# theshubh007/neural_rx

Measured on AMD Instinct MI355X. Metric: 5G NR slots/sec + p50 per-slot latency, nrx_rt config, higher is better.
Workload: dtype f16; 1 GPU; nrx_rt, 2 users, 4 PRB, 4 rx_ant, 16-QAM, batch=128 slots per GPU; global_batch=128, num_it=2, parallelism=dp1 (slot shards), streams=2

## Files before the change

### neural_rx_amd/build.py

```python
from __future__ import annotations

import hashlib
import os
import subprocess
import sys

HERE = os.path.dirname(os.path.abspath(__file__))
CSRC = os.path.join(HERE, "csrc")
LIB = os.path.join(HERE, "lib", "libnrx.so")
KERNEL_TUS = ["nrx_k_p16.hip", "nrx_k_p16m.hip", "nrx_k_p16s.hip", "nrx_k_p64.hip", "nrx_k_fwd0.hip",
              "nrx_k_fwd1.hip", "nrx_k_fwd2.hip", "nrx_k_rr.hip", "nrx_k_col.hip", "nrx_dispatch.hip"]
SOURCES = [os.path.join(CSRC, f) for f in KERNEL_TUS] + [
    os.path.join(CSRC, "nrx_aerial.hip"), os.path.join(CSRC, "nrx_synth.hip"), os.path.join(CSRC, "nrx_lmmse.hip"),
    os.path.join(CSRC, "nrx_kbest.hip"), os.path.join(CSRC, "nrx_chest.hip"),
    os.path.join(CSRC, "nrx_softmetrics.hip"), os.path.join(CSRC, "nrx_ldpc.hip"),
    os.path.join(CSRC, "nrx_cfo.hip"), os.path.join(CSRC, "nrx_ls.hip"), os.path.join(CSRC, "nrx_cir.hip"),
    os.path.join(CSRC, "nrx_ofdm.hip"), os.path.join(CSRC, "nrx_timechan.hip"), os.path.join(CSRC, "nrx_train.hip"),
    os.path.join(CSRC, "nrx_model.cpp"), os.path.join(CSRC, "nrx_api.cpp")]
HEADERS = [os.path.join(CSRC, "nrx_internal.h"), os.path.join(CSRC, "nrx_model.h"), os.path.join(CSRC, "nrx_rng.h"),
           os.path.join(HERE, "..", "include", "nrx.h")]
KERNEL_INCS = [os.path.join(CSRC, "nrx_device.inc"), os.path.join(CSRC, "nrx_launch.inc"),
               os.path.join(CSRC, "nrx_rr.inc"), os.path.join(CSRC, "nrx_col.inc"), os.path.join(CSRC, "nrx_geom.h")]
DEPS = SOURCES + HEADERS + KERNEL_INCS + [os.path.abspath(__file__)]
ARCH = os.environ.get("NRX_OFFLOAD_ARCH", "gfx950")


def hipcc() -> str:
    for c in (os.environ.get("HIPCC"), "/opt/rocm/bin/hipcc", "hipcc"):
        if c and (os.path.sep not in c or os.path.exists(c)):
            return c
    raise RuntimeError("hipcc not found")


def needs_build() -> bool:
    if not os.path.exists(LIB):
        return True
    t = os.path.getmtime(LIB)
    if any(os.path.getmtime(d) > t for d in DEPS if os.path.exists(d)):
        return True
    return any(_stale(os.path.join(OBJ_DIR, os.path.basename(s) + ".o"), s) for s in SOURCES)


OBJ_DIR = os.path.join(HERE, "lib", "obj")


def _includes(src: str) -> list:
    if os.path.basename(src) in KERNEL_TUS:
        return HEADERS + KERNEL_INCS
    return HEADERS


def _sig(src: str) -> str:
    return " ".join(repr(os.path.getmtime(d)) for d in [src] + _includes(src) if os.path.exists(d))


def _stale(obj: str, src: str) -> bool:
    sig = obj + ".sig"
    if not os.path.exists(obj) or not os.path.exists(sig):
        return True
    return open(sig).read() != _sig(src)


def strip_comments(text: str) -> str:
    out, i, n = [], 0, len(text)
    while i < n:
        c = text[i]
        if c == "/" and i + 1 < n and text[i + 1] == "/":
            j = text.find("\n", i)
            i = n if j < 0 else j
            out.append(" ")
        elif c == "/" and i + 1 < n and text[i + 1] == "*":
            j = text.find("*/", i + 2)
            i = n if j < 0 else j + 2
            out.append(" ")
        elif c in "\"'":
            j = i + 1
            while j < n and text[j] != c:
                j += 2 if text[j] == "\\" else 1
            out.append(text[i:j + 1])
            i = j + 1
        else:
            out.append(c)
            i += 1
    return " ".join("".join(out).split())


def hash_sources(texts: dict) -> str:
    h = hashlib.sha256()
    for name in sorted(texts):
        h.update(name.encode() + b"\0" + strip_comments(texts[name]).encode() + b"\0")
    return h.hexdigest()[:16]


def source_hash() -> str:
    texts = {}
    for p in sorted(set(SOURCES + HEADERS + KERNEL_INCS)):
        with open(p, encoding="utf-8") as f:
            texts[os.path.basename(p)] = f.read()
    return hash_sources(texts)


def _build_id_object(verbose: bool, obj_dir: str = OBJ_DIR, tag: str = "") -> str:
    src = os.path.join(obj_dir, "nrx_build_id.cpp")
    obj = src + ".o"
    with open(src, "w") as f:
        f.write('extern "C" const char* nrx_build_id(void) { return "%s%s"; }\n' % (source_hash(), tag))
    cmd = [hipcc(), "-O2", "-fPIC", "-c", src, "-o", obj]
    if verbose:
        print(" ".join(cmd), flush=True)
    subprocess.run(cmd, check=True)
    return obj


def build(force: bool = False, verbose: bool = True, lib: str = LIB, obj_dir: str = OBJ_DIR,
          extra_flags=()) -> str:
    if lib == LIB and not force and not needs_build():
        return LIB
    os.makedirs(obj_dir, exist_ok=True)
    tmp = lib + f".tmp{os.getpid()}"
    flags = [f"--offload-arch={ARCH}", "-O3", "-std=c++17", "-fPIC", "-Wall", "-Wno-unused-function",
             *extra_flags]
    objs, procs = [], []
    for src in SOURCES:
        obj = os.path.join(obj_dir, os.path.basename(src) + ".o")
        objs.append(obj)
        if not force and not _stale(obj, src):
            continue
        part = obj + f".{os.getpid()}.part"
        cmd = [hipcc(), *flags, "-c", src, "-o", part]
        if verbose:
            print(" ".join(cmd), flush=True)
        procs.append((subprocess.Popen(cmd), part, obj, _sig(src)))
    bad = 0
    for p, part, obj, sig in procs:
        rc = p.wait()
        if rc:
            bad = rc
            if os.path.exists(part):
                os.remove(part)
        else:
            os.replace(part, obj)
            with open(obj + ".sig", "w") as f:
                f.write(sig)
    if bad:
        raise subprocess.CalledProcessError(bad, "hipcc -c")
    objs.append(_build_id_object(verbose, obj_dir, "+" + "".join(extra_flags) if extra_flags else ""))
    cmd = [hipcc(), f"--offload-arch={ARCH}", "-shared", *objs, "-o", tmp]
    if verbose:
        print(" ".join(cmd), flush=True)
    subprocess.run(cmd, check=True)
    os.replace(tmp, lib)
    return lib


if __name__ == "__main__":
    build(force="--force" in sys.argv)
```

### neural_rx_amd/csrc/nrx_api.cpp

```cpp
#include <hip/hip_runtime.h>

#include <cmath>
#include <cstdio>
#include <cstdlib>
#include <cstring>
#include <string>
#include <type_traits>
#include <vector>

#include "../../include/nrx.h"
#include "nrx_internal.h"
#include "nrx_model.h"

namespace nrx {
hipError_t launch_forward_f16(const FwdArgs<_Float16, float, _Float16>& args, const ModelW<_Float16, float>& W,
                              const FwdPlan& pl, const FusedCtl& fc, hipStream_t st, Prof* prof);
void device_counts(int* cus, int* xccs);
size_t fused_sync_bytes();
hipError_t fused_sync_status(void* sync, int* st, bool reset, hipEvent_t last);
hipError_t run_tier_p64(const FwdArgs<double, double, float>& args, const ModelW<double, double>& W,
                        const FwdPlan& pl, hipStream_t st, Prof* prof);
hipError_t setup_kernels();
int strip_width(int precision);

static thread_local std::string g_err;

int fail(int code, const std::string& msg) {
  g_err = msg;
  return code;
}

int hip_fail(hipError_t e, const char* what) {
  return fail(NRX_ERR_HIP, std::string(what) + ": " + hipGetErrorString(e));
}
}

using namespace nrx;

namespace {

int check_range(const char* name, long v, long lo, long hi, int code = NRX_ERR_SHAPE) {
  if (v >= lo && v <= hi) return NRX_OK;
  return fail(code, std::string(name) + " must be " + std::to_string(lo) + ".." + std::to_string(hi));
}

template <class IO>
int check_grid(const IO* io, int tx_supported = kMaxUsers, int min_subcarriers = 1) {
  if (io->num_symbols != kT) return fail(NRX_ERR_SHAPE, "num_symbols must be 14");
  if (int rc = check_range("batch", io->batch, 1, 65535)) return rc;
  if (int rc = check_range("num_subcarriers", io->num_subcarriers, min_subcarriers, 12 * 275)) return rc;
  if (io->num_tx > tx_supported && tx_supported < kMaxUsers)
    return fail(NRX_ERR_UNSUPPORTED, "the kernels are built for num_tx <= " + std::to_string(tx_supported));
  return check_range("num_tx", io->num_tx, 1, kMaxUsers);
}
template <class IO>
int check_grid_ant(const IO* io, int tx_supported = kMaxUsers, int min_subcarriers = 1) {
  if (int rc = check_grid(io, tx_supported, min_subcarriers)) return rc;
  return check_range("num_rx_ant", io->num_rx_ant, 1, 16);
}

int check_mcs_bits(const int32_t* bits, int num_mcs, bool qam, int num_mcs_code = NRX_ERR_SHAPE) {
  if (int rc = check_range("num_mcs", num_mcs, 1, 8, num_mcs_code)) return rc;
  for (int m = 0; m < num_mcs; ++m)
    if (qam ? bits[m] != 2 && bits[m] != 4 && bits[m] != 6 : bits[m] < 1 || bits[m] > 8)
      return fail(NRX_ERR_INVALID_ARG, qam ? "mcs_bits must be 2, 4 or 6" : "mcs_bits must be 1..8");
  return NRX_OK;
}
int check_bits_stride(int bits_stride, const int32_t* bits, int num_mcs) {
  for (int m = 0; m < num_mcs; ++m)
    if (bits_stride < bits[m]) return fail(NRX_ERR_SHAPE, "bits_stride < max(mcs_bits)");
  return NRX_OK;
}

int check_dmrs_symbols(const int32_t* sym, int n, int* mask = nullptr) {
  if (int rc = check_range("num_dmrs_symbols", n, 1, 4)) return rc;
  int bits = 0;
  for (int k = 0; k < n; ++k) {
    if (sym[k] < 0 || sym[k] >= kT || (k && sym[k] <= sym[k - 1]))
      return fail(NRX_ERR_INVALID_ARG, "dmrs_symbols must be ascending symbol indices below 14");
    bits |= 1 << sym[k];
  }
  if (mask) *mask = bits;
  return NRX_OK;
}
int check_cdm_group(const int32_t* group, int num_tx) {
  for (int u = 0; u < num_tx; ++u)
    if (group[u] != 0 && group[u] != 1) return fail(NRX_ERR_INVALID_ARG, "cdm_group must be 0/1");
  return NRX_OK;
}
int check_dmrs_ports(int num_tx, const int32_t* group, const int32_t* focc, const int32_t* tocc, int despread_f,
                     int despread_t, int num_subcarriers, const int32_t* sym, int num_dmrs_symbols) {
  if (int rc = check_range("despread_f", despread_f, 0, 1, NRX_ERR_INVALID_ARG)) return rc;
  if (int rc = check_range("despread_t", despread_t, 0, 1, NRX_ERR_INVALID_ARG)) return rc;
  unsigned seen = 0;
  for (int u = 0; u < num_tx; ++u) {
    if ((focc[u] != 0 && focc[u] != 1) || (tocc[u] != 0 && tocc[u] != 1))
      return fail(NRX_ERR_INVALID_ARG, "focc and tocc must be 0/1");
    const unsigned bit = 1u << (group[u] + 2 * focc[u] + 4 * tocc[u]);
    if (seen & bit) return fail(NRX_ERR_INVALID_ARG, "two ports share one (cdm_group, focc, tocc)");
    seen |= bit;
    if (focc[u] && !despread_f) return fail(NRX_ERR_INVALID_ARG, "a port with focc = 1 needs despread_f");
    if (tocc[u] && !despread_t) return fail(NRX_ERR_INVALID_ARG, "a port with tocc = 1 needs despread_t");
  }
  if (despread_f && num_subcarriers % 4)
    return fail(NRX_ERR_SHAPE, "despread_f needs num_subcarriers % 4 == 0 (pairs of comb positions)");
  if (despread_t) {
    bool ok = num_dmrs_symbols % 2 == 0;
    for (int k = 0; ok && k < num_dmrs_symbols; k += 2) ok = sym[k + 1] == sym[k] + 1;
    if (!ok) return fail(NRX_ERR_INVALID_ARG, "despread_t needs dmrs_symbols in pairs (t, t + 1)");
  }
  return NRX_OK;
}
int check_aerial_list(const void* re, const void* im, int num_subcarriers) {
  if ((re == nullptr) != (im == nullptr)) return fail(NRX_ERR_INVALID_ARG, "Aerial outputs come in (real, imag) pairs");
  if (re && num_subcarriers % 12) return fail(NRX_ERR_SHAPE, "Aerial pilot list needs num_subcarriers % 12 == 0");
  return NRX_OK;
}
int check_symbol_mask(const char* name, int v) {
  if (v >= 0 && v < (1 << kT)) return NRX_OK;
  return fail(NRX_ERR_INVALID_ARG, std::string(name) + " must be a mask of the 14 symbols");
}
int check_pos(const char* name, double v) {
  if (v > 0.0 && std::isfinite(v)) return NRX_OK;
  return fail(NRX_ERR_INVALID_ARG, std::string(name) + " must be finite and > 0");
}
int check_nonneg(const char* name, double v) {
  if (v >= 0.0 && std::isfinite(v)) return NRX_OK;
  return fail(NRX_ERR_INVALID_ARG, std::string(name) + " must be finite and >= 0");
}

int check_tap_span(long l_min, long l_max) {
  if (int rc = check_range("l_min", l_min, -255, 0)) return rc;
  if (int rc = check_range("l_max", l_max, 0, 255)) return rc;
  if (l_max - l_min + 1 > 256) return fail(NRX_ERR_SHAPE, "the tap span l_max - l_min + 1 must be <= 256");
  return NRX_OK;
}

int too_small(size_t need) {
  return fail(NRX_ERR_WORKSPACE, "workspace too small: need " + std::to_string(need) + " bytes");
}
int check_workspace(const void* ws, size_t bytes, size_t need, size_t align) {
  if (!ws) return fail(NRX_ERR_INVALID_ARG, "null workspace pointer");
  if ((uintptr_t)ws & (align - 1))
    return fail(NRX_ERR_INVALID_ARG, "workspace must be " + std::to_string(align) + "-byte aligned");
  return bytes < need ? too_small(need) : NRX_OK;
}
int store_size(size_t* bytes, size_t need) {
  if (!bytes) return fail(NRX_ERR_INVALID_ARG, "bytes is NULL");
  *bytes = need;
  return NRX_OK;
}
int launched(hipError_t e, const char* what) { return e == hipSuccess ? NRX_OK : hip_fail(e, what); }

}

struct EventProf : Prof {
  struct Rec { int kid; hipEvent_t a, b; };
  std::vector<Rec> recs;
  std::vector<hipEvent_t> pool;
  hipEvent_t get() {
    if (!pool.empty()) {
      hipEvent_t e = pool.back();
      pool.pop_back();
      return e;
    }
    hipEvent_t e = nullptr;
    (void)hipEventCreate(&e);
    return e;
  }
  void begin(int kid, void* st) override {
    Rec r{kid, get(), nullptr};
    (void)hipEventRecord(r.a, (hipStream_t)st);
    recs.push_back(r);
  }
  void end(int, void* st) override {
    hipEvent_t e = get();
    (void)hipEventRecord(e, (hipStream_t)st);
    recs.back().b = e;
  }
  int64_t launches[K_COUNT] = {0};
  double total_ms[K_COUNT] = {0};
  hipError_t collect() {
    for (auto& r : recs) {
      hipError_t e = hipEventSynchronize(r.b);
      if (e != hipSuccess) return e;
      float ms = 0.f;
      e = hipEventElapsedTime(&ms, r.a, r.b);
      if (e != hipSuccess) return e;
      launches[r.kid] += 1;
      total_ms[r.kid] += ms;
      pool.push_back(r.a);
      pool.push_back(r.b);
    }
    recs.clear();
    return hipSuccess;
  }
  void reset() {
    for (int k = 0; k < K_COUNT; ++k) {
      launches[k] = 0;
      total_ms[k] = 0;
    }
  }
  ~EventProf() override {
    for (auto& r : recs) {
      (void)hipEventDestroy(r.a);
      if (r.b) (void)hipEventDestroy(r.b);
    }
    for (auto e : pool) (void)hipEventDestroy(e);
  }
};

struct nrx_handle {
  nrx_desc desc;
  int device;
  DeviceModel<_Float16, float> m16;
  DeviceModel<double, double> m64;
  EventProf* prof = nullptr;
  void* fused_sync = nullptr;
  int fused_enabled = 1;
  int spin_limit = kFusedSpinLimit;
  int dbg_err = 0;
  int update_rr = kSchedDefault;
  hipEvent_t last_ev = nullptr;
  hipStream_t last_stream = nullptr;
  bool have_last = false;
  FusedCtl fused_ctl() const { return FusedCtl{fused_sync, spin_limit, dbg_err}; }
  int small_tiers = 1;
  Sched sched() const { return Sched{update_rr, fused_enabled, small_tiers}; }
};

struct FwdWs {
  double* norm;
  void *s_out, *s_in, *a_out, *a, *pe16;
  size_t total;
};
static FwdWs fwd_layout(const nrx_shape* s, int precision, void* ws) {
  const bool f16 = precision == NRX_PREC_F16;
  const size_t plane = (size_t)s->num_tx * s->num_subcarriers * kT * kDS * (f16 ? 2 : 4);
  Carver c(ws);
  FwdWs w{};
  w.norm = c.take<double>(s->batch);
  w.s_out = c.take<char>(s->batch * plane);
  w.s_in = c.take<char>(s->batch * plane);
  w.a_out = c.take<char>(s->batch * plane);
  w.a = c.take<char>(s->batch * plane);
  if (f16) w.pe16 = c.take<char>(plane);
  w.total = c.bytes();
  return w;
}
static size_t ws_bytes_of(const nrx_shape* s, int precision) { return fwd_layout(s, precision, nullptr).total; }

static int check_shape(const nrx_shape* s) {
  if (!s) return fail(NRX_ERR_INVALID_ARG, "shape is NULL");
  return check_grid(s);
}

template <class WT, class BT, class S>
static void fill_args(FwdArgs<WT, BT, S>& a, const nrx_desc* d, const nrx_io* io, void* ws, int init_cinp) {
  const nrx_shape* s = &io->shape;
  a.B = s->batch;
  a.llr_B = s->batch;
  a.U = s->num_tx;
  a.F = s->num_subcarriers;
  a.A = d->num_rx_ant;
  a.M = d->num_mcs;
  a.H = num_heads(d);
  a.init_cinp = init_cinp;
  a.num_init = num_heads(d);
  a.masking = d->var_mcs_masking;
  a.use_h = d->use_h_hat;
  a.bits_max = bits_max(d);
  for (int i = 0; i < kMaxHeads; ++i)
    a.head_bits[i] = i < a.H ? head_bits(d, i) : 0;
  a.y = io->y;
  a.pe = io->pe;
  a.h_hat = io->h_hat;
  a.active = io->active;
  a.mcs_mask = io->mcs_mask;
  a.llr = io->llr;
  a.h_ref = io->h_ref;
  const FwdWs w = fwd_layout(s, io->precision, ws);
  a.norm = w.norm;
  a.s_in = (S*)w.s_in;
  a.s_out = (S*)w.s_out;
  a.a = (S*)w.a;
  a.a_out = (S*)w.a_out;
  a.pe16 = (S*)w.pe16;
  a.ws_base = (const char*)ws;
  a.ws_bytes = w.total < 0xFFFFFFFFull ? (unsigned)w.total : 0xFFFFFFFFu;
}

static int forward_slots(nrx_handle* h, const nrx_io* io, int llr_B, void* workspace, hipStream_t st);
static int chunk_slots(const nrx_shape* s, int precision);

template <class F>
static int each_chunk(const nrx_shape* s, int precision, F f) {
  const int B = s->batch, bc = chunk_slots(s, precision);
  for (int b0 = 0; b0 < B; b0 += bc)
    if (int rc = f(b0, b0 + bc < B ? bc : B - b0)) return rc;
  return NRX_OK;
}

static FwdPlan plan_f16(FwdArgs<_Float16, float, _Float16>& a, const nrx_desc* d, const nrx_io* io, int n, void* ws,
                        int init_cinp, const Sched& sc, int cus, int xccs) {
  nrx_io c = *io;
  c.shape.batch = n;
  fill_args(a, d, &c, ws, init_cinp);
  return plan_forward(a, io->num_it, sc, cus, xccs);
}

static int busy(const nrx_handle* h, hipStream_t st) {
  if (h->have_last && h->last_stream != st && hipEventQuery(h->last_ev) == hipErrorNotReady)
    return fail(NRX_ERR_BUSY, "a one-launch forward of this handle is still running on another stream");
  return NRX_OK;
// ... 840 lines not shown
}

int nrx_chest_nmse(const nrx_nmse_io* io, void* workspace, size_t workspace_bytes, void* stream) {
  if (int rc = check_nmse(io)) return rc;
  if (int rc = check_workspace(workspace, workspace_bytes, nmse_workspace_bytes(*io), 8)) return rc;
  return launched(launch_chest_nmse(*io, workspace, (hipStream_t)stream), "channel nmse launch");
}

struct nrx_ldpc {
  LdpcDev d;
  int device;
  void* tables;
};

constexpr int kLdpcMaxN = 68 * 384;

int nrx_ldpc_create(const nrx_ldpc_code* code, int32_t device, nrx_ldpc** out) {
  if (!code || !code->shifts || !out) return fail(NRX_ERR_INVALID_ARG, "null argument");
  *out = nullptr;
  const int mb = code->mb, nb = code->nb, z = code->z;
  if (mb < 1 || mb > 46) return fail(NRX_ERR_SHAPE, "mb must be 1..46");
  if (nb < 2 || nb > 68) return fail(NRX_ERR_SHAPE, "nb must be 2..68");
  if (nb <= mb) return fail(NRX_ERR_SHAPE, "nb must be > mb");
  if (z < 2 || z > 384) return fail(NRX_ERR_SHAPE, "z must be 2..384");
  if (code->kb < 1 || code->kb >= nb) return fail(NRX_ERR_SHAPE, "kb must be 1..nb-1");
  if (device < -1) return fail(NRX_ERR_INVALID_ARG, "device must be >= 0, or -1 for a handle without device tables");
  std::vector<int> row_ptr(mb + 1, 0), edges, colw(nb, 0);
  for (int i = 0; i < mb; ++i) {
    for (int j = 0; j < nb; ++j) {
      const int s = code->shifts[i * nb + j];
      if (s < -1 || s >= z) return fail(NRX_ERR_INVALID_ARG, "shifts must be -1..z-1");
      if (s < 0) continue;
      edges.push_back(j * z);
      edges.push_back(s);
      colw[j] += 1;
    }
    row_ptr[i + 1] = (int)edges.size() / 2;
    const int w = row_ptr[i + 1] - row_ptr[i];
    if (w < 2 || w > 32) return fail(NRX_ERR_INVALID_ARG, "row weight must be 2..32");
  }
  for (int j = 0; j < nb; ++j)
    if (!colw[j]) return fail(NRX_ERR_INVALID_ARG, "column weight must be >= 1");
  nrx_ldpc* h = new nrx_ldpc();
  h->d.mb = mb, h->d.nb = nb, h->d.z = z, h->d.kb = code->kb, h->d.num_edges = row_ptr[mb];
  h->d.plan = ldpc_plan(nb, z, h->d.num_edges);
  h->d.row_ptr = nullptr, h->d.edges = nullptr;
  h->device = device;
  h->tables = nullptr;
  if (device >= 0) {
    hipError_t e = hipSetDevice(device);
    if (e == hipSuccess) e = ldpc_setup();
    const size_t rp = (size_t)(mb + 1) * 4, rpa = (rp + 15) / 16 * 16, eb = edges.size() * 4;
    if (e == hipSuccess) e = hipMalloc(&h->tables, rpa + eb);
    if (e == hipSuccess) e = hipMemcpy(h->tables, row_ptr.data(), rp, hipMemcpyHostToDevice);
    if (e == hipSuccess) e = hipMemcpy((char*)h->tables + rpa, edges.data(), eb, hipMemcpyHostToDevice);
    if (e != hipSuccess) {
      if (h->tables) (void)hipFree(h->tables);
      delete h;
      return hip_fail(e, "ldpc tables");
    }
    h->d.row_ptr = (const int*)h->tables;
    h->d.edges = (const int*)((char*)h->tables + rpa);
  }
  *out = h;
  return NRX_OK;
}

void nrx_ldpc_destroy(nrx_ldpc* h) {
  if (!h) return;
  if (h->tables) (void)hipFree(h->tables);
  delete h;
}

static int check_ldpc_io(const nrx_ldpc_io* io) {
  if (!io) return fail(NRX_ERR_INVALID_ARG, "io is NULL");
  if (!io->llr_in || !io->hard || !io->iters || !io->parity_ok) return fail(NRX_ERR_INVALID_ARG, "null tensor pointer");
  if (int rc = check_range("num_iter", io->num_iter, 1, 100, NRX_ERR_INVALID_ARG)) return rc;
  if (io->cn_type != 0 && io->cn_type != 1) return fail(NRX_ERR_INVALID_ARG, "cn_type must be 0 (boxplus) or 1 (min-sum)");
  if (io->early_stop != 0 && io->early_stop != 1) return fail(NRX_ERR_INVALID_ARG, "early_stop must be 0 or 1");
  if (io->cn_type == 1 && !(io->ms_scale > 0.0f && io->ms_scale <= 1.0f))
    return fail(NRX_ERR_INVALID_ARG, "ms_scale must be in (0, 1]");
  if (int rc = check_pos("llr_clip", io->llr_clip)) return rc;
  return check_range("num_cw", io->num_cw, 1, 1 << 20);
}

static size_t ldpc_workspace_bytes(const nrx_ldpc* h, const nrx_ldpc_io* io) {
  const size_t msgs = h->d.plan.msg_lds ? 0 : (size_t)io->num_cw * h->d.num_edges * h->d.z * 4;
  return msgs > 256 ? msgs : 256;
}

int nrx_ldpc_workspace_size(const nrx_ldpc* h, const nrx_ldpc_io* io, size_t* bytes) {
  if (int rc = check_ldpc_io(io)) return rc;
  if (!h) return fail(NRX_ERR_INVALID_ARG, "null handle");
  return store_size(bytes, ldpc_workspace_bytes(h, io));
}

int nrx_ldpc_decode(nrx_ldpc* h, const nrx_ldpc_io* io, void* workspace, size_t workspace_bytes, void* stream) {
  if (int rc = check_ldpc_io(io)) return rc;
  if (!h) return fail(NRX_ERR_INVALID_ARG, "null handle");
  if (int rc = check_workspace(workspace, workspace_bytes, ldpc_workspace_bytes(h, io), 16)) return rc;
  if (h->device < 0) return fail(NRX_ERR_INVALID_ARG, "no device: the handle was created with device = -1");
  return launched(launch_ldpc_decode(h->d, *io, workspace, (hipStream_t)stream), "ldpc decode launch");
}

int nrx_ldpc_gather(const nrx_ldpc_gather_io* io, void* stream) {
  if (!io) return fail(NRX_ERR_INVALID_ARG, "io is NULL");
  if (!io->llr || !io->bits || !io->active || !io->llr_in || !io->skip)
    return fail(NRX_ERR_INVALID_ARG, "null tensor pointer");
  if (int rc = check_llr_grid(io)) return rc;
  if (int rc = check_range("num_cw_per_user", io->num_cw_per_user, 1, 64)) return rc;
  if (int rc = check_range("n", io->n, 4, kLdpcMaxN)) return rc;
  if ((int64_t)io->batch * io->num_tx * io->num_cw_per_user > (1 << 20))
    return fail(NRX_ERR_SHAPE, "batch * num_tx * num_cw_per_user must be <= 2^20");
  if (int rc = check_range("n_tx", io->n_tx, 1, 1 << 20)) return rc;
  if (!io->tx_col && io->n_tx > io->n) return fail(NRX_ERR_SHAPE, "n_tx > n needs a tx_col");
  return launched(launch_ldpc_gather(*io, (hipStream_t)stream), "ldpc gather launch");
}

int nrx_ldpc_count(const nrx_ldpc_count_io* io, void* stream) {
  if (!io) return fail(NRX_ERR_INVALID_ARG, "io is NULL");
  if (!io->hard || !io->skip || !io->counts) return fail(NRX_ERR_INVALID_ARG, "null tensor pointer");
  if (int rc = check_range("batch", io->batch, 1, 65535)) return rc;
  if (int rc = check_range("num_tx", io->num_tx, 1, kMaxUsers)) return rc;
  if (int rc = check_range("num_cw_per_user", io->num_cw_per_user, 1, 64)) return rc;
  if (int rc = check_range("n", io->n, 4, kLdpcMaxN)) return rc;
  if (io->num_info < 1 || io->num_info > io->n) return fail(NRX_ERR_SHAPE, "num_info must be 1..n");
  return launched(launch_ldpc_count(*io, (hipStream_t)stream), "ldpc count launch");
}

static int check_aligned(const char* name, const void* p, size_t align) {
  if (!((uintptr_t)p & (align - 1))) return NRX_OK;
  return fail(NRX_ERR_INVALID_ARG, std::string(name) + " must be " + std::to_string(align) + "-byte aligned");
}

static int check_train(const nrx_desc* d, const nrx_train_io* io) {
  if (int rc = check_desc(d)) return rc;
  if (!io) return fail(NRX_ERR_INVALID_ARG, "io is NULL");
  if (int rc = check_shape(&io->shape)) return rc;
  if ((int64_t)io->shape.batch * io->shape.num_tx * io->shape.num_subcarriers * kT > (1 << 24))
    return fail(NRX_ERR_SHAPE, "training takes at most 2^24 positions (batch x num_tx x num_subcarriers x 14)");
  if (io->num_it < 1 || io->num_it > d->num_it) return fail(NRX_ERR_INVALID_ARG, "Invalid number of iterations");
  if (int rc = check_symbol_mask("dmrs_symbol_mask", io->dmrs_symbol_mask)) return rc;
  if (io->dmrs_symbol_mask == (1 << kT) - 1)
    return fail(NRX_ERR_INVALID_ARG, "dmrs_symbol_mask must leave a data symbol");
  if (int rc = check_range("multiloss", io->multiloss, 0, 1, NRX_ERR_INVALID_ARG)) return rc;
  if (int rc = check_nonneg("w_chest", io->w_chest)) return rc;
  if (int rc = check_bits_stride(io->bits_stride, d->bits, d->num_mcs)) return rc;
  if (!io->y || !io->pe || !io->active || !io->bits || !io->weights || !io->grad || !io->loss)
    return fail(NRX_ERR_INVALID_ARG, "null tensor pointer");
  if (d->use_h_hat && !io->h_hat) return fail(NRX_ERR_INVALID_ARG, "h_hat is required by this model");
  if (io->w_chest > 0.0 && !io->h) return fail(NRX_ERR_INVALID_ARG, "h is required when w_chest > 0");
  const void* f32s[] = {io->y, io->pe, io->h_hat, io->active, io->mcs_mask, io->h, io->weights, io->grad, io->llr,
                        io->h_ref};
  for (const void* p : f32s)
    if (int rc = check_aligned("float tensors", p, 4)) return rc;
  return check_aligned("loss", io->loss, 8);
}

int nrx_train_workspace_size(const nrx_desc* desc, const nrx_train_io* io, size_t* bytes) {
  if (int rc = check_train(desc, io)) return rc;
  return store_size(bytes, train_workspace_bytes(*desc, *io));
}

int nrx_train_grad(const nrx_desc* desc, const nrx_train_io* io, void* workspace, size_t workspace_bytes,
                   void* stream) {
  return nrx_train_grad_acc(desc, io, nullptr, workspace, workspace_bytes, stream);
}

int nrx_train_grad_acc(const nrx_desc* desc, const nrx_train_io* io, const nrx_train_acc* acc, void* workspace,
                       size_t workspace_bytes, void* stream) {
  if (int rc = check_train(desc, io)) return rc;
  if (acc) {
    if (int rc = check_range("accumulate", acc->accumulate, 0, 1, NRX_ERR_INVALID_ARG)) return rc;
    if (acc->batch_total < io->shape.batch || acc->batch_total > 65535)
      return fail(NRX_ERR_SHAPE, "batch_total must be shape.batch..65535");
  }
  if (int rc = check_workspace(workspace, workspace_bytes, train_workspace_bytes(*desc, *io), 256)) return rc;
  return launched(launch_train_grad(*desc, *io, acc && acc->accumulate, acc ? acc->batch_total : io->shape.batch,
                                    workspace, (hipStream_t)stream),
                  "training launch");
}

int nrx_adam_step(const nrx_adam_io* io, void* stream) {
  if (!io) return fail(NRX_ERR_INVALID_ARG, "io is NULL");
  if (!io->w || !io->g || !io->m || !io->v) return fail(NRX_ERR_INVALID_ARG, "null tensor pointer");
  const void* f32s[] = {io->w, io->g, io->m, io->v};
  for (const void* p : f32s)
    if (int rc = check_aligned("float tensors", p, 4)) return rc;
  if (io->n < 0) return fail(NRX_ERR_INVALID_ARG, "n must be >= 0");
  if (io->step < 1) return fail(NRX_ERR_INVALID_ARG, "step must be >= 1");
  if (int rc = check_nonneg("lr", io->lr)) return rc;
  if (int rc = check_nonneg("eps", io->eps)) return rc;
  if (!(io->beta1 >= 0.0 && io->beta1 < 1.0) || !(io->beta2 >= 0.0 && io->beta2 < 1.0))
    return fail(NRX_ERR_INVALID_ARG, "beta1 and beta2 must be in [0, 1)");
  const double c1 = 1.0 - std::pow(io->beta1, (double)io->step), c2 = 1.0 - std::pow(io->beta2, (double)io->step);
  return launched(launch_adam(*io, c1, c2, (hipStream_t)stream), "adam launch");
}

int nrx_profile_enable(nrx_handle* h, int32_t enable) {
  if (!h) return fail(NRX_ERR_INVALID_ARG, "null handle");
  if (enable) {
    if (!h->prof) h->prof = new EventProf();
    hipError_t e = h->prof->collect();
    h->prof->reset();
    if (e != hipSuccess) return hip_fail(e, "profile reset");
  } else {
    delete h->prof;
    h->prof = nullptr;
  }
  return NRX_OK;
}

int nrx_fused_status(nrx_handle* h, int32_t* status, int32_t reset) {
  if (!h || !status) return fail(NRX_ERR_INVALID_ARG, "null argument");
  int st[3] = {0, 0, 0};
  hipError_t e = fused_sync_status(h->fused_sync, st, reset != 0, h->have_last ? h->last_ev : nullptr);
  if (e != hipSuccess) return hip_fail(e, "fused status");
  for (int i = 0; i < 3; ++i) status[i] = st[i];
  if (st[0])
    return fail(NRX_ERR_FUSED, "one-launch forward error bits " + std::to_string(st[0]) +
                                   " (1: dependency wait timed out, 2: items left undone): outputs invalid");
  return NRX_OK;
}

int nrx_fused_config(nrx_handle* h, int32_t enable, int32_t spin_limit, int32_t inject_err) {
  if (!h) return fail(NRX_ERR_INVALID_ARG, "null argument");
  if (enable > 2) return fail(NRX_ERR_INVALID_ARG, "enable must be 0 (off), 1 (default) or 2 (force)");
  if (enable >= 0) h->fused_enabled = enable;
  if (spin_limit >= 0) h->spin_limit = spin_limit > 0 ? spin_limit : kFusedSpinLimit;
  if (inject_err >= 0) h->dbg_err = inject_err;
  return NRX_OK;
}

int nrx_update_schedule(nrx_handle* h, int32_t update_rr) {
  if (!h) return fail(NRX_ERR_INVALID_ARG, "null argument");
  if (update_rr > kSchedMax) return fail(NRX_ERR_INVALID_ARG, "update_rr is a stage mask 0..127");
  if (update_rr >= 0) h->update_rr = update_rr;
  return NRX_OK;
}

int nrx_debug_small_tiers(nrx_handle* h, int32_t enable) {
  if (!h) return fail(NRX_ERR_INVALID_ARG, "null argument");
  if (enable >= 0) h->small_tiers = enable != 0;
  return NRX_OK;
}

static int debug_forward_plan(const nrx_desc* desc, const nrx_shape* shape, int32_t precision, int32_t num_it,
                              int32_t sched_mask, int32_t fused_mode, int32_t cus, int32_t xccs, int32_t io_flags,
                              int32_t* out, int32_t cap) {
  if (int rc = check_desc(desc)) return rc;
  if (int rc = check_shape(shape)) return rc;
  if (precision != NRX_PREC_F16 && precision != NRX_PREC_F32X) return fail(NRX_ERR_INVALID_ARG, "unknown precision");
  if (num_it < 1 || num_it > desc->num_it) return fail(NRX_ERR_INVALID_ARG, "Invalid number of iterations");
  if (sched_mask < 0 || sched_mask > kSchedMax || fused_mode < 0 || fused_mode > 2 || cus < 0 || (!out && cap > 0))
    return fail(NRX_ERR_INVALID_ARG, "bad schedule, device counts or output");
  if (cus == 0) device_counts(&cus, &xccs);
  nrx_io io{*shape, num_it, precision};
  void* ws = reinterpret_cast<void*>(uintptr_t(256));
  if (io_flags & 1) io.h_ref = reinterpret_cast<float*>(ws);
  if (io_flags & 2) io.mcs_mask = reinterpret_cast<const float*>(ws);
  int n_out = 0;
  auto put = [&](int b0, int n, int s, const void* plan, int x, int y) {
    int rec[16] = {b0, n, s};
    memcpy(rec + 3, plan, 11 * sizeof(int));
    rec[14] = x, rec[15] = y;
    for (int k = 0; k < 16; ++k, ++n_out)
      if (n_out < cap) out[n_out] = rec[k];
  };
  static_assert(offsetof(FwdPlan, st) == 11 * sizeof(int) && offsetof(StagePlan, variant) == 11 * sizeof(int) &&
                    sizeof(StagePlan) == 12 * sizeof(int),
                "record layout");
  (void)each_chunk(shape, precision, [&](int b0, int n) {
    FwdPlan pl;
    if (precision == NRX_PREC_F16) {
      FwdArgs<_Float16, float, _Float16> a{};
      pl = plan_f16(a, desc, &io, n, ws, init_padded_cin(desc, 32), Sched{sched_mask, fused_mode}, cus, xccs);
    } else {
      FwdArgs<double, double, float> a{};
      nrx_io c = io;
      c.shape.batch = n;
      fill_args(a, desc, &c, ws, init_padded_cin(desc, 16));
      pl = plan_forward(a, num_it);
    }
    put(b0, n, -1, &pl, pl.one_launch(), pl.combine_launches());
    for (int s = 0; s < pl.num_init + pl.num_it; ++s) put(b0, n, s, &pl.st[s], pl.st[s].variant, 0);
    return 0;
  });
  return n_out;
}

int nrx_debug_forward_plan(const nrx_desc* desc, const nrx_shape* shape, int32_t precision, int32_t num_it,
                           int32_t sched_mask, int32_t fused_mode, int32_t cus, int32_t xccs, int32_t* out,
                           int32_t cap) {
  return debug_forward_plan(desc, shape, precision, num_it, sched_mask, fused_mode, cus, xccs, 0, out, cap);
}

int nrx_debug_forward_plan_io(const nrx_desc* desc, const nrx_shape* shape, int32_t precision, int32_t num_it,
                              int32_t sched_mask, int32_t fused_mode, int32_t cus, int32_t xccs, int32_t io_flags,
                              int32_t* out, int32_t cap) {
  if (io_flags < 0 || io_flags > 3) return fail(NRX_ERR_INVALID_ARG, "io_flags: 1 h_ref, 2 mcs_mask");
  return debug_forward_plan(desc, shape, precision, num_it, sched_mask, fused_mode, cus, xccs, io_flags, out, cap);
}

int nrx_profile_read(nrx_handle* h, int32_t kernel, int64_t* launches, double* total_ms) {
  if (!h || !launches || !total_ms) return fail(NRX_ERR_INVALID_ARG, "null argument");
  if (kernel < 0 || kernel >= K_COUNT) return fail(NRX_ERR_INVALID_ARG, "bad kernel id");
  if (!h->prof) return fail(NRX_ERR_INVALID_ARG, "profiling is not enabled");
  hipError_t e = h->prof->collect();
  if (e != hipSuccess) return hip_fail(e, "profile collect");
  *launches = h->prof->launches[kernel];
  *total_ms = h->prof->total_ms[kernel];
  return NRX_OK;
}

int nrx_compute_pe(int32_t num_tx, int32_t F, int32_t T, const int32_t* dmrs_symbols, int32_t nsym,
                   const int32_t* cdm_group, float* pe) {
  if (num_tx < 1 || F < 1 || T < 1 || !dmrs_symbols || nsym < 1 || !cdm_group || !pe)
    return fail(NRX_ERR_INVALID_ARG, "bad argument");
  std::vector<double> dt(T), df(F);
  for (int u = 0; u < num_tx; ++u) {
    if (cdm_group[u] != 0 && cdm_group[u] != 1) return fail(NRX_ERR_INVALID_ARG, "cdm_group must be 0/1");
    bool any_f = false;
    for (int t = 0; t < T; ++t) {
      int best = 1 << 30;
      for (int k = 0; k < nsym; ++k) best = std::min(best, std::abs(dmrs_symbols[k] - t));
      dt[t] = best;
    }
    for (int f = 0; f < F; ++f) {
      int best = 1 << 30;
      for (int p = cdm_group[u]; p < F; p += 2) {
        best = std::min(best, std::abs(p - f));
        any_f = true;
      }
      df[f] = best;
    }
    if (!any_f) return fail(NRX_ERR_INVALID_ARG, "user has no pilots");
    auto norm = [](std::vector<double>& v) {
      double m = 0;
      for (double x : v) m += x;
      m /= v.size();
      double s2 = 0;
      for (double& x : v) {
        x -= m;
        s2 += x * x;
      }
      const double sd = std::sqrt(s2 / v.size());
      if (sd > 0)
        for (double& x : v) x /= sd;
    };
    norm(dt);
    norm(df);
    for (int f = 0; f < F; ++f)
      for (int t = 0; t < T; ++t) {
        pe[(((size_t)u * F + f) * T + t) * 2 + 0] = (float)dt[t];
        pe[(((size_t)u * F + f) * T + t) * 2 + 1] = (float)df[f];
      }
  }
  return NRX_OK;
}

double nrx_flops_per_re_user(const nrx_desc* d, int32_t num_it) {
  return check_desc(d) ? 0.0 : flops_per_re_user(d, num_it);
}

}
```

### neural_rx_amd/csrc/nrx_col.inc

```

#ifndef NRX_COL_PR3
#define NRX_COL_PR3 2
#endif
__device__ __forceinline__ int col_fstart(int strip, int strips) { return strips == 1 ? 0 : strip * kColFO - 2; }
__device__ __forceinline__ int col_pos_lo(int strips) { return strips == 1 ? 0 : 2; }
__device__ __forceinline__ int col_pos_hi(int strips) { return strips == 1 ? kColPos : kColPos - 2; }

template <int N, class F, int... I>
__device__ __forceinline__ void col_sfor_(F&& f, std::integer_sequence<int, I...>) {
  (f(std::integral_constant<int, I>{}), ...);
}
template <int N, class F>
__device__ __forceinline__ void col_sfor(F&& f) {
  col_sfor_<N>(f, std::make_integer_sequence<int, N>{});
}

template <int CINP, int COUTP>
struct WCol {
  WLds<P16, CINP, COUTP> w;
  unsigned boff;
  __device__ WCol(const char* base, const char* bias_row, int g) : w{base} {
    boff = rr_lds_addr(bias_row) + 16u * (unsigned)g;
    asm("" : "+v"(boff));
  }
  __device__ half8 afrag(int n, int kc, int lane, int g) const { return w.afrag(n, kc, lane, g); }
  __device__ void dw_taps(int kc, int g, half8 (&t)[9]) const { w.dw_taps(kc, g, t); }
  __device__ floatx4 bias_acc(int n, int) const { return *(rr_lds_cfloatx4*)((rr_lds_cchar*)(size_t)boff + 64 * n); }
};

template <int NKC, int RO, int A, int B, int COUTP, bool REGH, int NIN, class WS>
__device__ __forceinline__ void col_pass(const half8 (&in)[NIN][NKC], const RrNb& nb, const WS& ws, int lane, int g,
                                         floatx4 (&acc)[B - A][COUTP / 16]) {
  constexpr int NR = B - A;
  constexpr int NT = COUTP / 16;
  constexpr bool TOP = !REGH && A == 0, BOT = !REGH && B == RO;
  static_assert(NR >= 1 && A >= 0 && B <= RO && NIN == (REGH ? RO + 2 : RO), "rows");
  half8 w[9], xt{}, xb{};
  auto load = [&](int kc) {
    if constexpr (TOP) xt = rr_ld(nb.top, kc);
    if constexpr (BOT) xb = rr_ld(nb.bot, kc);
    ws.dw_taps(kc, g, w);
  };
  load(0);
#pragma unroll
  for (int kc = 0; kc < NKC; ++kc) {
    half8 a_cur = ws.afrag(0, kc, lane, g);
    half8 d[NR];
#pragma unroll
    for (int r = 0; r < NR; ++r) {
      const int i = A + r;
      if constexpr (REGH) {
        d[r] = P16::dw_row(in[i][kc], in[i + 1][kc], in[i + 2][kc], w);
      } else {
        const half8 x0 = i - 1 < 0 ? xt : in[i - 1 < 0 ? 0 : i - 1][kc];
        const half8 x2 = i + 1 >= RO ? xb : in[i + 1 >= RO ? RO - 1 : i + 1][kc];
        d[r] = P16::dw_row(x0, in[i][kc], x2, w);
      }
    }
    dw_fence<NR>(d);
    if (kc + 1 < NKC) load(kc + 1);
#pragma unroll
    for (int n = 0; n < NT; ++n) {
      half8 a_nxt = a_cur;
      if (n + 1 < NT) a_nxt = ws.afrag(n + 1, kc, lane, g);
      if (kc == 0) {
        const floatx4 bn = ws.bias_acc(n, g);
#pragma unroll
        for (int r = 0; r < NR; ++r) acc[r][n] = P16::mma_v(a_cur, d[r], bn);
      } else {
#pragma unroll
        for (int r = 0; r < NR; ++r) acc[r][n] = P16::mma_v(a_cur, d[r], acc[r][n]);
      }
      a_cur = a_nxt;
    }
  }
}

struct ColNoPost {
  __device__ void operator()() const {}
};
template <int NKC, int RO, int PR, bool REGH, int NIN, class WS, class Post = ColNoPost>
__device__ __forceinline__ void col_layer(const half8 (&in)[NIN][NKC], const RrNb& nb, const WS& ws, int lane, int g,
                                          half8 (&out)[RO][4], int f_own0, int F, Post post0 = Post{}) {
  static_assert(RO % PR == 0, "passes");
  col_sfor<RO / PR>([&](auto J) __attribute__((always_inline)) {
    constexpr int A = decltype(J)::value * PR;
    floatx4 acc[PR][8];
    col_pass<NKC, RO, A, A + PR, kHID, REGH>(in, nb, ws, lane, g, acc);
    rr_to_own<RO, A, A + PR>(acc, out, f_own0, F);
    if constexpr (A == 0) post0();
  });
}

#ifndef NRX_COL_ZD
#define NRX_COL_ZD 2
#endif
#if defined(NRX_STAMPS) && defined(NRX_PRO_STAMPS)
#define COL_PRO_TS(m) rr_ts(1, m)
#else
#define COL_PRO_TS(m)
#endif
template <int PR>
struct ColZ {
  static constexpr int D = NRX_COL_ZD;
  unsigned soff[kColRO + 2];
  half8 xb[D][PR + 2];
};
template <int PR>
__device__ __forceinline__ void col_gz_load_step(ColZ<PR>& z, const GZ& gz, int s) {
  const int j = s / 4, kc = s % 4;
#pragma unroll
  for (int i = 0; i < PR + 2; ++i) z.xb[s % ColZ<PR>::D][i] = gz.load(kc, z.soff[j * PR + i]);
}
template <int PR>
__device__ __forceinline__ void col_gz_first(ColZ<PR>& z, const GZ& gz, int p0) {
#pragma unroll
  for (int i = 0; i < kColRO + 2; ++i) z.soff[i] = gz.row_soff(p0 - 1 + i);
#pragma unroll
  for (int s = 0; s < ColZ<PR>::D; ++s) col_gz_load_step<PR>(z, gz, s);
}
template <int PR, class WS, class Post = ColNoPost>
__device__ __forceinline__ void col_conv1_gz(ColZ<PR>& z, const GZ& gz, const WS& ws, int lane, int g,
                                             half8 (&out)[kColRO][4], int f_own0, int F, Post post0 = Post{}) {
  constexpr int RO = kColRO, NP = RO / PR, NS = NP * 4, D = ColZ<PR>::D;
  half8 w[9];
  ws.dw_taps(0, g, w);
  col_sfor<NP>([&](auto J) __attribute__((always_inline)) {
    constexpr int j = decltype(J)::value;
    floatx4 acc[PR][8];
#pragma unroll
    for (int kc = 0; kc < 4; ++kc) {
      const int s = j * 4 + kc;
      half8 a_cur = ws.afrag(0, kc, lane, g);
      half8 d[PR];
#pragma unroll
      for (int r = 0; r < PR; ++r) d[r] = P16::dw_row(z.xb[s % D][r], z.xb[s % D][r + 1], z.xb[s % D][r + 2], w);
      dw_fence<PR>(d);
      if constexpr (!std::is_same_v<Post, ColNoPost>) {
        if (s == 0) COL_PRO_TS(3);
      }
      if (s + D < NS) col_gz_load_step<PR>(z, gz, s + D);
      if (s + 1 < NS) ws.dw_taps((kc + 1) % 4, g, w);
#pragma unroll
      for (int n = 0; n < 8; ++n) {
        half8 a_nxt = a_cur;
        if (n + 1 < 8) a_nxt = ws.afrag(n + 1, kc, lane, g);
        if (kc == 0) {
          const floatx4 bn = ws.bias_acc(n, g);
#pragma unroll
          for (int r = 0; r < PR; ++r) acc[r][n] = P16::mma_v(a_cur, d[r], bn);
        } else {
#pragma unroll
          for (int r = 0; r < PR; ++r) acc[r][n] = P16::mma_v(a_cur, d[r], acc[r][n]);
        }
        a_cur = a_nxt;
      }
    }
    rr_to_own<RO, j * PR, (j + 1) * PR>(acc, out, f_own0, F);
    if constexpr (j == 0 && !std::is_same_v<Post, ColNoPost>) {
      COL_PRO_TS(4);
      post0();
      COL_PRO_TS(5);
    }
  });
}

template <int PR, class Epi>
__device__ __forceinline__ void col_conv3(const half8 (&own)[kColRO][4], const RrNb& nb, Epi& epi, int lane, int t,
                                          int g, int p0) {
  col_sfor<kColRO / PR>([&](auto J) __attribute__((always_inline)) {
    constexpr int A = decltype(J)::value * PR;
    typename Epi::template PrefT<PR> pf;
    epi.template prefetch<PR>(pf, p0 + A, t, g);
    floatx4 acc[PR][4];
    col_pass<4, kColRO, A, A + PR, kDSP, false>(own, nb, epi.ws, lane, g, acc);
    epi.template settle<PR>(pf);
    epi.template run<PR>(acc, pf, p0 + A, t, g, 0, PR);
  });
}

#ifndef NRX_COL_RB
#define NRX_COL_RB 3
#endif
template <int PR, class Epi>
__device__ __forceinline__ void col_conv3_ro(const half8 (&own)[kColRO][4], const RrNb& nb, Epi& epi, int lane, int t,
                                             int g, int p0) {
  constexpr int RB = NRX_COL_RB;
  static_assert(kColRO % RB == 0, "readout row batches");
  CFrag<P16, kDSP / 16> sb[kColRO];
  bool ok[kColRO];
  col_sfor<kColRO / PR>([&](auto J) __attribute__((always_inline)) {
    constexpr int A = decltype(J)::value * PR;
    typename Epi::template PrefT<PR> pf;
    epi.template prefetch<PR>(pf, p0 + A, t, g);
    floatx4 acc[PR][4];
    col_pass<4, kColRO, A, A + PR, kDSP, false>(own, nb, epi.ws, lane, g, acc);
    epi.template settle<PR>(pf);
    CFrag<P16, kDSP / 16> sbp[PR];
    bool okp[PR];
    epi.template state_frags<PR>(acc, pf, p0 + A, t, g, sbp, okp);
#pragma unroll
    for (int r = 0; r < PR; ++r) {
      sb[A + r] = sbp[r];
      ok[A + r] = okp[r];
    }
  });
  col_sfor<kColRO / RB>([&](auto J) __attribute__((always_inline)) {
    constexpr int A = decltype(J)::value * RB;
    CFrag<P16, kDSP / 16> sbr[RB];
    bool okr[RB];
#pragma unroll
    for (int r = 0; r < RB; ++r) {
      sbr[r] = sb[A + r];
      okr[r] = ok[A + r];
    }
    epi.template readout_rows<RB>(sbr, okr, p0 + A, t, g);
  });
}

__device__ __forceinline__ void col_ts(int k, int m) { rr_ts(k, m); }

template <int CINP1, int TAILM>
struct ColStage {
  SepStage<CINP1, kHID> s1;
  SepStage<kHID, kHID> s2;
  SepStage<kHID, kDSP> s3;
  DenseStage<kDSP, kAGG> d1;
  DenseStage<kAGG, kDSP> d2;
  __device__ __forceinline__ void load_w1(const BlockParams<P16>& prm) { s1.load(prm.w[0]); }
  __device__ __forceinline__ void load_rest(const BlockParams<P16>& prm) {
    s2.load(prm.w[1]);
    s3.load(prm.w[2]);
    if constexpr (TAILM == TAIL_AGG) {
      d1.load(prm.agg[0]);
      d2.load(prm.agg[1]);
    }
  }
  __device__ __forceinline__ void load(const BlockParams<P16>& prm) {
    load_w1(prm);
    load_rest(prm);
  }
  __device__ __forceinline__ void store_w1(char* smem) const {
    s1.store(smem + kRrW1);
    for (int i = nrx_tid(); i < 768 / 4; i += 512) reinterpret_cast<float*>(smem + kRrNeg)[i] = -__builtin_inff();
    for (int i = nrx_tid(); i < kRrExChunk * 4 / 16; i += 512)
      reinterpret_cast<intx4*>(smem + kRrZero)[i] = intx4{0, 0, 0, 0};
  }
  __device__ __forceinline__ void store_rest(char* smem) const {
    s2.store(smem + kRrW2);
    s3.store(smem + kRrW3);
    if constexpr (TAILM == TAIL_AGG) {
      d1.store(smem + kRrW3 + 16 * 1024, reinterpret_cast<float*>(smem + kRrW3 + kWTailBias));
      d2.store(smem + kRrW3 + 24 * 1024, reinterpret_cast<float*>(smem + kRrW3 + kWTailBias + kAGG * 4));
    }
  }
  __device__ __forceinline__ void store(char* smem) const {
    store_w1(smem);
    store_rest(smem);
  }
};

template <int CHP, int TAILM, bool FIRST = false, class LT = ColGeneric>
__device__ __forceinline__ void col_upd_item(const BlockParams<P16>& prm, char* smem, int wave, int b, int u, int strip,
                                             int k, ColStage<kUPD_CINP, TAILM>* stage = nullptr) {
  constexpr int PR = 2;
  col_ts(k, 0);
  const int lane = nrx_tid() & 63, t = lane & 15, g = lane >> 4;
  const int p0 = kColRO * wave;
  const int strips = prm.strips;
  const int f_start = col_fstart(strip, strips);
  const int F = prm.a.F;
  const int f_own0 = f_start + p0;
  const RrNb nb = rr_nb(smem, wave, t, g);
  half8 own[kColRO][4];
  const GZ gz = gz_make(prm, b, u, f_start, t, g);
  ColZ<PR> z;
  col_gz_first<PR>(z, gz, p0);
  if constexpr (FIRST) {
    COL_PRO_TS(0);
    stage->load_rest(prm);
    COL_PRO_TS(1);
    stage->store_w1(smem);
    COL_PRO_TS(2);
    __syncthreads();
  }
  col_ts(k, 5);
  {
    const WRr<kHID> w1(smem + kRrW1, t < kT ? smem + kRrW1 + kWBias : smem + kRrNeg + kRrNegOff, g);
    if constexpr (FIRST) col_conv1_gz<PR>(z, gz, w1, lane, g, own, f_own0, F, [&]() { stage->store_rest(smem); });
    else col_conv1_gz<PR>(z, gz, w1, lane, g, own, f_own0, F);
  }
  col_ts(k, 1);
  __syncthreads();
  rr_write_exch<kColRO>(smem, wave, t, g, own);
  __syncthreads();
  col_ts(k, 2);
  {
    const WRr<kHID> w2(smem + kRrW2, t < kT ? smem + kRrW2 + kWBias : smem + kRrNeg + kRrNegOff, g);
    half8 nxt[kColRO][4];
    col_layer<4, kColRO, PR, false>(own, nb, w2, lane, g, nxt, f_own0, F);
#pragma unroll
    for (int r = 0; r < kColRO; ++r)
#pragma unroll
      for (int kc = 0; kc < 4; ++kc) own[r][kc] = nxt[r][kc];
  }
  col_ts(k, 3);
  using WS3 = WLds<P16, kHID, kDSP>;
  const WS3 w3{smem + kRrW3};
  char* WB = TAILM == TAIL_READOUT_WB ? smem + kRrW1 : smem + kRrW3;
  if constexpr (TAILM == TAIL_READOUT_WB) {
    RrHeads<CHP> hd;
    hd.load(prm);
    __syncthreads();
    rr_write_exch<kColRO>(smem, wave, t, g, own);
    hd.store(WB, prm);
  } else {
    __syncthreads();
    rr_write_exch<kColRO>(smem, wave, t, g, own);
  }
  __syncthreads();
  col_ts(k, 4);
  EpiConv3<P16, WS3, CHP, TAILM, LT> epi{&prm, nullptr, WB, w3, b, u, f_start, col_pos_hi(strips), 0, 1.f, false,
                                     (float)prm.a.active[(size_t)b * prm.a.U + u], -1, 0, 0};
  epi.pos_lo = col_pos_lo(strips);
  if constexpr (TAILM == TAIL_READOUT_WB) col_conv3_ro<NRX_COL_PR3>(own, nb, epi, lane, t, g, p0);
  else col_conv3<NRX_COL_PR3>(own, nb, epi, lane, t, g, p0);
  col_ts(k, 6);
}

template <int CHP, int TAILM, bool MULTI, class LT = ColGeneric>
__device__ __forceinline__ void col_update_stage(const BlockParams<P16>& prm, int items) {
  extern __shared__ __attribute__((aligned(16))) char smem[];
  rr_ts(0, 7);
  rr_ts_edge(0);
  const int wave = __builtin_amdgcn_readfirstlane(nrx_tid() >> 6);
  int k = 0;
  {
    ColStage<kUPD_CINP, TAILM> stage;
    stage.load_w1(prm);
    int b, u, strip;
    work_item(blockIdx.x, prm.a.B, prm.a.U, prm.strips, prm.order_rev, b, u, strip);
    col_upd_item<CHP, TAILM, true, LT>(prm, smem, wave, b, u, strip, k, &stage);
  }
  if constexpr (MULTI) {
    for (int i = blockIdx.x; i < items; i += gridDim.x, ++k) {
      int b, u, strip;
      if (k > 0) {
        work_item(i, prm.a.B, prm.a.U, prm.strips, prm.order_rev, b, u, strip);
        col_upd_item<CHP, TAILM>(prm, smem, wave, b, u, strip, k);
      }
      if constexpr (TAILM == TAIL_READOUT_WB) {
        if (i + (int)gridDim.x < items) {
          SepStage<kUPD_CINP, kHID> s1;
          SepStage<kHID, kHID> s2;
          s1.load(prm.w[0]);
          s2.load(prm.w[1]);
          __syncthreads();
          s1.store(smem + kRrW1);
          s2.store(smem + kRrW2);
          __syncthreads();
        }
      }
    }
  }
  rr_ts_edge(1);
}

template <int CHP, int TAILM, class LT = ColGeneric>
__global__ __launch_bounds__(512) void k_update_col(BlockParams<P16> prm, int items) {
  col_update_stage<CHP, TAILM, false, LT>(prm, items);
}
template <int CHP, int TAILM>
__global__ __launch_bounds__(512) void k_update_col_multi(BlockParams<P16> prm, int items) {
  col_update_stage<CHP, TAILM, true>(prm, items);
}

struct ColInitRow {
  floatx4 v0, v1;
  float2 pe;
};
__device__ __forceinline__ ColInitRow col_init_load(const FwdArgs<_Float16, float, _Float16>& a, int b, int u, int f,
                                                    int t, int g) {
  const bool ok = f >= 0 && f < a.F && t < kT;
  const size_t re = ((size_t)b * a.F + (ok ? f : 0)) * kT + (ok ? t : 0);
  const float* src = a.y + re * 8;
  if (g == 1 && a.use_h) src = a.h_hat + ((size_t)b * a.U * a.F * kT + (size_t)u * a.F * kT + (re - (size_t)b * a.F * kT)) * 8;
  ColInitRow r;
  r.v0 = reinterpret_cast<const floatx4*>(src)[0];
  r.v1 = reinterpret_cast<const floatx4*>(src)[1];
  r.pe = *reinterpret_cast<const float2*>(a.pe + (((size_t)u * a.F + (ok ? f : 0)) * kT + (ok ? t : 0)) * 2);
  return r;
}
__device__ __forceinline__ half8 col_init_z(const ColInitRow& r, float ns, bool ok, int g, bool use_h) {
  const float v[8] = {r.v0[0], r.v0[1], r.v0[2], r.v0[3], r.v1[0], r.v1[1], r.v1[2], r.v1[3]};
  half8 o;
#pragma unroll
  for (int e = 0; e < 8; ++e) {
    float x = f32_rounded(v[e] * ns);
    if (g == 2) x = e == 0 ? r.pe.x : (e == 1 ? r.pe.y : 0.f);
    if (!ok || g == 3 || (g == 1 && !use_h)) x = 0.f;
    o[e] = (_Float16)x;
  }
  return o;
}

struct ColInitLane {
  const char* src;
  const char* pe;
};
__device__ __forceinline__ ColInitLane col_init_lane(const FwdArgs<_Float16, float, _Float16>& a, int b, int u, int g) {
  const size_t plane = (size_t)a.F * kT * 8;
  const float* y = a.y + (size_t)b * plane;
  const float* h = a.h_hat + ((size_t)b * a.U + u) * plane;
  return ColInitLane{reinterpret_cast<const char*>(g == 1 ? h : y),
                     reinterpret_cast<const char*>(a.pe + (size_t)u * a.F * kT * 2)};
}
__device__ __forceinline__ ColInitRow col_init_load_lean(const ColInitLane& ln, int F, int f, int t) {
  const bool ok = f >= 0 && f < F && t < kT;
  const unsigned re = (unsigned)((ok ? f : 0) * kT + (ok ? t : 0));
  ColInitRow r;
  r.v0 = *reinterpret_cast<const floatx4*>(ln.src + re * 32u);
  r.v1 = *reinterpret_cast<const floatx4*>(ln.src + re * 32u + 16u);
  r.pe = *reinterpret_cast<const float2*>(ln.pe + re * 8u);
  return r;
}
__device__ __forceinline__ half8 col_init_z_lean(const ColInitRow& r, float sc, bool ok, int g) {
  float v[8] = {r.v0[0], r.v0[1], r.v0[2], r.v0[3], r.v1[0], r.v1[1], r.v1[2], r.v1[3]};
  if (g == 2) v[0] = r.pe.x, v[1] = r.pe.y;
  half8 o;
#pragma unroll
  for (int e = 0; e < 8; ++e) o[e] = (_Float16)f32_rounded(v[e] * sc);
  typedef unsigned u32x4 __attribute__((ext_vector_type(4)));
  u32x4 w = __builtin_bit_cast(u32x4, o);
  const bool k0 = ok && g < 3, k1 = ok && g < 2;
  w[0] = k0 ? w[0] : 0u;
#pragma unroll
  for (int i = 1; i < 4; ++i) w[i] = k1 ? w[i] : 0u;
  return __builtin_bit_cast(half8, w);
}

template <int TAILM, bool FIRST = false, class LT = ColGeneric>
__device__ __forceinline__ void col_init_item(const BlockParams<P16>& prm, char* smem, int wave, int b, int u,
                                              int strip, int k, ColStage<32, TAILM>* stage = nullptr) {
  constexpr int PR = 2;
  constexpr bool LEAN = LT::kLean;
  col_ts(k, 0);
  const auto& a = prm.a;
  const int lane = nrx_tid() & 63, t = lane & 15, g = lane >> 4;
  const int p0 = kColRO * wave;
  const int strips = LEAN ? 1 : prm.strips;
  const int f_start = col_fstart(strip, strips);
  const int F = a.F, A2 = LEAN ? 8 : 2 * a.A;
  const bool norm_pre = LEAN ? false : prm.norm_pre != 0;
  const int f_own0 = f_start + p0;
  const RrNb nb = rr_nb(smem, wave, t, g);
  const float* yslot = a.y + (size_t)b * F * kT * A2;
  const int nqs = F * kT * A2 / 4;
  NormPre npre;
  if (!norm_pre) npre = slot_norm_issue(yslot, nqs);
  ColInitRow zr[kColRO + 2];
  if constexpr (LEAN) {
    const ColInitLane ln = col_init_lane(a, b, u, g);
#pragma unroll
    for (int i = 0; i < kColRO + 2; ++i) zr[i] = col_init_load_lean(ln, F, f_own0 - 1 + i, t);
  } else {
#pragma unroll
    for (int i = 0; i < kColRO + 2; ++i) zr[i] = col_init_load(a, b, u, f_own0 - 1 + i, t, g);
  }
  if constexpr (FIRST) stage->load_rest(prm);
  const int m = LEAN ? 0 : prm.m;
  const float wm = a.masking ? 1.f : (a.mcs_mask ? a.mcs_mask[((size_t)b * a.U + u) * a.M + m] : (m == 0 ? 1.f : 0.f));
  if constexpr (FIRST) {
    stage->store_w1(smem);
    if (norm_pre) __syncthreads();
  }
  const float ns = norm_pre ? (float)a.norm[b]
                                : (float)slot_norm(npre, yslot, nqs, reinterpret_cast<double*>(smem + kColRed));
  col_ts(k, 5);
  half8 zin[kColRO + 2][1];
  const float zsc = g == 2 ? 1.f : ns;
#pragma unroll
  for (int i = 0; i < kColRO + 2; ++i) {
    const int f = f_own0 - 1 + i;
    if constexpr (LEAN) zin[i][0] = col_init_z_lean(zr[i], zsc, f >= 0 && f < F && t < kT, g);
    else zin[i][0] = col_init_z(zr[i], ns, f >= 0 && f < F && t < kT, g, a.use_h != 0);
  }
  dpp_in_fence(zin);
  if (a.pe16 && g == 2 && t < kT) {
#pragma unroll
    for (int i = 1; i <= kColRO; ++i) {
      const int p = p0 + i - 1, f = f_start + p;
      if (p >= col_pos_lo(strips) && p < col_pos_hi(strips) && f >= 0 && f < F) {
        const half8 h = zin[i][0];
        *reinterpret_cast<half8*>(a.pe16 + (((size_t)u * F + f) * kT + t) * kDS) = h;
      }
    }
  }
  half8 own[kColRO][4];
  {
    const WCol<32, kHID> w1(smem + kRrW1, t < kT ? smem + kRrW1 + kWBias : smem + kRrNeg + kRrNegOff, g);
    half8 o1[kColRO][4];
    if constexpr (FIRST) col_layer<1, kColRO, PR, true>(zin, nb, w1, lane, g, o1, f_own0, F, [&]() { stage->store_rest(smem); });
    else col_layer<1, kColRO, PR, true>(zin, nb, w1, lane, g, o1, f_own0, F);
#pragma unroll
    for (int r = 0; r < kColRO; ++r)
#pragma unroll
      for (int kc = 0; kc < 4; ++kc) own[r][kc] = o1[r][kc];
  }
  col_ts(k, 1);
  __syncthreads();
  rr_write_exch<kColRO>(smem, wave, t, g, own);
  __syncthreads();
  col_ts(k, 2);
  {
    const WRr<kHID> w2(smem + kRrW2, t < kT ? smem + kRrW2 + kWBias : smem + kRrNeg + kRrNegOff, g);
    half8 nxt[kColRO][4];
    col_layer<4, kColRO, PR, false>(own, nb, w2, lane, g, nxt, f_own0, F);
#pragma unroll
    for (int r = 0; r < kColRO; ++r)
#pragma unroll
      for (int kc = 0; kc < 4; ++kc) own[r][kc] = nxt[r][kc];
  }
  col_ts(k, 3);
  __syncthreads();
  rr_write_exch<kColRO>(smem, wave, t, g, own);
  __syncthreads();
  col_ts(k, 4);
  using WS3 = WLds<P16, kHID, kDSP>;
  const WS3 w3{smem + kRrW3};
  EpiConv3<P16, WS3, 16, TAILM, LT> epi{&prm, nullptr, smem + kRrW3, w3, b, u, f_start, col_pos_hi(strips), 1, wm, m == 0,
                                    (float)a.active[(size_t)b * a.U + u], -1, 0, 0};
  epi.pos_lo = col_pos_lo(strips);
  col_conv3<NRX_COL_PR3>(own, nb, epi, lane, t, g, p0);
  col_ts(k, 6);
}

template <int TAILM, bool MULTI, class LT = ColGeneric>
__device__ __forceinline__ void col_init_stage(const BlockParams<P16>& prm, int items) {
  extern __shared__ __attribute__((aligned(16))) char smem[];
  rr_ts(0, 7);
  rr_ts_edge(0);
  const int wave = __builtin_amdgcn_readfirstlane(nrx_tid() >> 6);
  {
    ColStage<32, TAILM> stage;
    stage.load_w1(prm);
    int b, u, strip;
    work_item(blockIdx.x, prm.a.B, prm.a.U, LT::kLean ? 1 : prm.strips, prm.order_rev, b, u, strip);
    col_init_item<TAILM, true, LT>(prm, smem, wave, b, u, strip, 0, &stage);
  }
  if constexpr (MULTI) {
    int k = 1;
    for (int i = blockIdx.x + gridDim.x; i < items; i += gridDim.x, ++k) {
      int b, u, strip;
      work_item(i, prm.a.B, prm.a.U, prm.strips, prm.order_rev, b, u, strip);
      col_init_item<TAILM>(prm, smem, wave, b, u, strip, k);
    }
  }
  rr_ts_edge(1);
}

template <int TAILM, class LT = ColGeneric>
__global__ __launch_bounds__(512) void k_init_col(BlockParams<P16> prm, int items) {
  col_init_stage<TAILM, false, LT>(prm, items);
}
template <int TAILM>
__global__ __launch_bounds__(512) void k_init_col_multi(BlockParams<P16> prm, int items) {
  col_init_stage<TAILM, true>(prm, items);
}

struct ColFwdParams {
  BlockParams<P16> st[kColMaxStages];
  FusedSync* sync;
  int nst;
  int nq;
  int spin_limit;
  int dbg_err;
};

template <int CHP, int KIND>
__device__ __forceinline__ void fwd_col_item(const BlockParams<P16>& prm, char* smem, int wave, int b, int u,
                                             int strip, int k) {
  if constexpr (KIND == 0) {
    ColStage<32, TAIL_AGG> st;
    st.load_w1(prm);
    col_init_item<TAIL_AGG, true>(prm, smem, wave, b, u, strip, k, &st);
  } else if constexpr (KIND == 1) {
    ColStage<kUPD_CINP, TAIL_AGG> st;
    st.load_w1(prm);
    col_upd_item<CHP, TAIL_AGG, true>(prm, smem, wave, b, u, strip, k, &st);
  } else {
    ColStage<kUPD_CINP, TAIL_READOUT_WB> st;
    st.load_w1(prm);
    col_upd_item<CHP, TAIL_READOUT_WB, true>(prm, smem, wave, b, u, strip, k, &st);
  }
}

__device__ __forceinline__ int fwd_col_done(int* cnt, int* head, int* sh) {
  asm volatile("s_waitcnt vmcnt(0)" ::: "memory");
  __syncthreads();
  if (nrx_tid() == 0) {
    __hip_atomic_fetch_add(cnt, 1, __ATOMIC_RELAXED, __HIP_MEMORY_SCOPE_AGENT);
    sh[0] = atomicAdd(head, 1);
  }
  __syncthreads();
  return sh[0];
}

#ifdef NRX_STAMPS
#define NRX_FC_WAIT_STAMP(k)                                                  \
  if (nrx_tid() == 0 && g_nrx_stamp_on && (k) < 4 && blockIdx.x < 4096) \
    g_nrx_rr_stamps[blockIdx.x][16 * (k) + 15] = __builtin_amdgcn_s_memtime();
#else
#define NRX_FC_WAIT_STAMP(k)
#endif

template <int CHP>
__global__ __launch_bounds__(512) void k_fwd_col(ColFwdParams fp_arg) {
  typedef const __attribute__((address_space(4))) ColFwdParams KFP;
  const ColFwdParams& fp = *(const ColFwdParams*)(KFP*)__builtin_amdgcn_kernarg_segment_ptr();
  extern __shared__ __attribute__((aligned(16))) char smem[];
  __shared__ int sh[2];
  rr_ts(0, 7);
  rr_ts_edge(0);
  FusedSync* sy = fp_arg.sync;
  int* done = reinterpret_cast<int*>(sy + 1);
  const int nst = fp_arg.nst, nqs = fp_arg.nq, spin_limit = fp_arg.spin_limit;
  const int B = fp.st[0].a.B, U = fp.st[0].a.U, strips = fp.st[0].strips;
  const int ips = U * strips;
  const int q = xcc_id() % nqs;
  const int nbq = (B - q + nqs - 1) / nqs;
  const int per_stage = nbq * ips;
  const int total = nst * per_stage;
  int* head = &sy->head[q];
  const int wave = __builtin_amdgcn_readfirstlane(nrx_tid() >> 6);
  if (nrx_tid() == 0) {
    sh[0] = atomicAdd(head, 1);
    if (fp_arg.dbg_err && blockIdx.x == 0)
      __hip_atomic_fetch_or(&sy->err, fp_arg.dbg_err, __ATOMIC_RELAXED, __HIP_MEMORY_SCOPE_AGENT);
  }
  __syncthreads();
  int j = sh[0], k = 0;
  auto decode = [&](int jj, int s, int& b, int& u, int& strip) {
    const int r = jj - s * per_stage;
    b = q + nqs * (r / ips);
    const int ru = r % ips;
    u = ru / strips;
    strip = ru % strips;
  };
  if (nst == 3 && j < per_stage) {
    int b, u, strip;
    decode(j, 0, b, u, strip);
    fwd_col_item<CHP, 0>(fp.st[0], smem, wave, b, u, strip, k++);
    j = fwd_col_done(done + b, head, sh);
    if (j >= per_stage && j < 2 * per_stage) {
      decode(j, 1, b, u, strip);
      fused_wait(done + b, ips, sy, spin_limit);
      NRX_FC_WAIT_STAMP(k);
      fwd_col_item<CHP, 1>(fp.st[1], smem, wave, b, u, strip, k++);
      j = fwd_col_done(done + B + b, head, sh);
      if (j >= 2 * per_stage && j < total) {
        decode(j, 2, b, u, strip);
        fused_wait(done + B + b, ips, sy, spin_limit);
        NRX_FC_WAIT_STAMP(k);
        fwd_col_item<CHP, 2>(fp.st[2], smem, wave, b, u, strip, k++);
        j = fwd_col_done(done + 2 * B + b, head, sh);
      }
    }
  }
  while (j < total) {
    const int s = j / per_stage;
    int b, u, strip;
    decode(j, s, b, u, strip);
    if (s >= 1) fused_wait(done + (s - 1) * B + b, ips, sy, spin_limit);
    NRX_FC_WAIT_STAMP(k);
    if (s == 0) fwd_col_item<CHP, 0>(fp.st[0], smem, wave, b, u, strip, k);
    else if (s < nst - 1) fwd_col_item<CHP, 1>(fp.st[s], smem, wave, b, u, strip, k);
    else fwd_col_item<CHP, 2>(fp.st[s], smem, wave, b, u, strip, k);
    j = fwd_col_done(done + s * B + b, head, sh);
    ++k;
  }
  rr_ts_edge(1);
  if (nrx_tid() == 0) {
    asm volatile("s_waitcnt vmcnt(0)" ::: "memory");
    sh[1] = atomicAdd(&sy->exits, 1) == (int)(gridDim.x * gridDim.y) - 1;
  }
  __syncthreads();
  if (sh[1]) {
    for (int i = nrx_tid(); i < nst * B; i += 512)
      if (__hip_atomic_load(done + i, __ATOMIC_RELAXED, __HIP_MEMORY_SCOPE_AGENT) != ips)
        __hip_atomic_fetch_or(&sy->err, 2, __ATOMIC_RELAXED, __HIP_MEMORY_SCOPE_AGENT);
    __syncthreads();
    for (int i = nrx_tid(); i < nst * B; i += 512) done[i] = 0;
    if (nrx_tid() < 8) sy->head[nrx_tid()] = 0;
    if (nrx_tid() == 0) sy->exits = 0;
  }
}
```

### neural_rx_amd/csrc/nrx_device.inc

```
#include <hip/hip_runtime.h>
#include <stdint.h>
#include <stdlib.h>

#include <type_traits>
#include <utility>

#include "nrx_internal.h"
#include "nrx_geom.h"

#ifndef NRX_ABLATE
#define NRX_ABLATE 0
#endif

namespace nrx {

#ifdef NRX_STAMPS
static __device__ unsigned long long g_nrx_stamps[4096][64];
static __constant__ int g_nrx_stamp_on;
static __device__ unsigned long long g_nrx_rr_stamps[4096][64];
static __device__ int g_fstamp_item[4096];
__device__ __forceinline__ void fstamp(int m) {
  if (threadIdx.x == 0 && g_nrx_stamp_on == 100) {
    const int wg = blockIdx.x, it = g_fstamp_item[wg];
    if (wg < 4096 && it < 8) g_nrx_rr_stamps[wg][8 * it + m] = __builtin_amdgcn_s_memtime();
// ... 508 lines not shown
    if (in_off == 0) stamp_w(56);
    __syncthreads();
  }
}

template <class P, int CINP, int COUTP, bool GZIN = false, class WS, class Epi, class Post>
__device__ __forceinline__ void conv_layer(const char* X, int nslots, int in_off, int pos_lo,
                                           int pos_hi, const WS& ws, Epi&& epi, Post&& post_math,
                                           const GZ* gz = nullptr, bool skip = false) {
  const int wave = __builtin_amdgcn_readfirstlane(nrx_tid() >> 6);
  if constexpr (P::WLDS) {
    static_assert(P::R == 4, "f16 row split assumes passes of 4 / 3 rows");
    const int nrows = pos_hi - pos_lo;
    int n4 = nrows - 24;
    n4 = n4 < 0 ? 0 : n4;
    const int p0 = pos_lo + 4 * (wave < n4 ? wave : n4) + 3 * (wave > n4 ? wave - n4 : 0);
    const bool act = p0 < pos_hi;
    if (wave < n4) layer_pass<P, CINP, COUTP, 4, GZIN>(X, nslots, in_off, p0, act, true, ws, epi, post_math, gz, skip);
    else layer_pass<P, CINP, COUTP, 3, GZIN>(X, nslots, in_off, p0, act, true, ws, epi, post_math, gz, skip);
  } else {
    for (int base = pos_lo; base < pos_hi; base += 8 * P::R) {
      const int p0 = base + wave * P::R;
      layer_pass<P, CINP, COUTP, P::R, false>(X, nslots, in_off, p0, p0 < pos_hi, base == pos_lo, ws, epi, post_math,
                                              nullptr, skip);
    }
  }
}

struct NoPref {};

template <class P, int COUTP, class WS, int ER = 2>
struct EpiInPlace {
  template <int R>
  using PrefT = NoPref;
  static constexpr bool kNoBarrier = false;
  static constexpr bool kNextHook = false;
  static constexpr bool kNextHookRO = false;
  static constexpr int kEarlyRow = ER;
  char* X;
  int in_off, pos_hi, f_start, F;
  WS ws;
  __device__ void pre() const {}
  template <int R>
  __device__ void prefetch(NoPref&, int, int, int) const {}
  template <int R>
  __device__ void run(const typename P::Acc (&acc)[R][COUTP / 16], const NoPref&, int p0, int t,
                      int g, int r_lo, int r_hi) const {
    using Real = typename P::Real;
    using S = typename P::S;
    constexpr int NQ = COUTP * (int)sizeof(S) / 16;
    if constexpr (sizeof(S) == 2) {
      typedef __attribute__((address_space(3))) half8 lds_half8;
      constexpr int NKC = COUTP / 32;
      unsigned lo[NKC];
#pragma unroll
      for (int kc = 0; kc < NKC; ++kc) {
        lo[kc] = (unsigned)(size_t)(__attribute__((address_space(3))) char*)X +
                 (unsigned)((p0 - in_off - 1) * slot_pitch<P>() + (t * NQ + ((4 * kc + g) ^ swz<NQ>(t))) * 16);
        asm("" : "+v"(lo[kc]));
      }
#pragma unroll
      for (int r = 0; r < R; ++r) {
        if (r < r_lo || r >= r_hi) continue;
        const int p = p0 + r;
        if (p >= pos_hi) continue;
        const int f = f_start + p;
        const bool z = f < 0 || f >= F;
        if (t < kT) {
          if (!z) {
#pragma unroll
            for (int kc = 0; kc < NKC; ++kc) {
              const auto& a0 = acc[r][2 * kc];
              const auto& a1 = acc[r][2 * kc + 1];
              half8 h = half8{(S)a0[0], (S)a0[1], (S)a0[2], (S)a0[3], (S)a1[0], (S)a1[1], (S)a1[2], (S)a1[3]};
              h = __builtin_elementwise_max(h, half8{});
              *(lds_half8*)(size_t)(lo[kc] + r * slot_pitch<P>()) = h;
            }
          } else {
#pragma unroll
            for (int kc = 0; kc < NKC; ++kc) *(lds_half8*)(size_t)(lo[kc] + r * slot_pitch<P>()) = half8{};
          }
        }
      }
    } else {
#pragma unroll
      for (int r = 0; r < R; ++r) {
        if (r < r_lo || r >= r_hi) continue;
        const int p = p0 + r;
        if (p >= pos_hi) continue;
        const int f = f_start + p;
        const bool z = f < 0 || f >= F;
        const int slot = p - in_off - 1;
#pragma unroll
        for (int n = 0; n < COUTP / 16; ++n) {
#pragma unroll
          for (int j = 0; j < 4; ++j) {
            const int co = 16 * n + P::co(g, j);
            Real v = (Real)acc[r][n][j];
            v = v > (Real)0 ? v : (Real)0;
            if (z || t >= kT) v = (Real)0;
            *reinterpret_cast<S*>(X + xoff<P, NQ>(slot, t, co / P::EPC) + (co % P::EPC) * (int)sizeof(S)) = (S)v;
          }
        }
      }
    }
  }
};

template <class P, int CINP, int COUTP, class Src>
__device__ __forceinline__ void dense_tile(Src src, int lane, int g,
                                           const DenseW<typename P::WT, typename P::BT>& w,
                                           typename P::Acc (&acc)[COUTP / 16]) {
  constexpr int NKC = CINP / P::KC;
#pragma unroll
  for (int n = 0; n < COUTP / 16; ++n) acc[n] = P::zero();
  const typename P::WT* wrow = w.w + (lane & 15) * CINP + g * P::CPL;
#pragma unroll
  for (int kc = 0; kc < NKC; ++kc) {
    const typename P::DV b = src(kc * 4 + g);
#pragma unroll
    for (int n = 0; n < COUTP / 16; ++n)
      acc[n] = P::mma(wrow + n * 16 * CINP + kc * P::KC, b, acc[n]);
  }
}

template <class P, int COUTP>
__device__ __forceinline__ void epi_lds(char* out, int row, int t, int g,
                                        const typename P::Acc (&acc)[COUTP / 16],
                                        const typename P::BT* bias, bool relu, bool zero) {
  using Real = typename P::Real;
  const bool z = zero || t >= kT;
#pragma unroll
  for (int n = 0; n < COUTP / 16; ++n) {
#pragma unroll
    for (int j = 0; j < 4; ++j) {
      const int co = 16 * n + P::co(g, j);
      Real v = (Real)acc[n][j] + (Real)bias[co];
      if (relu) v = v > (Real)0 ? v : (Real)0;
      if (z) v = (Real)0;
      lds_store<P>(out, lds_elem_off<P, COUTP>(row, t, co), v);
    }
  }
}

__device__ __forceinline__ void wave_lds_sync() {
  __builtin_amdgcn_fence(__ATOMIC_RELEASE, "wavefront");
  __builtin_amdgcn_wave_barrier();
  __builtin_amdgcn_fence(__ATOMIC_ACQUIRE, "wavefront");
}


template <class P>
struct BlockParams {
  FwdArgs<typename P::WT, typename P::BT, typename P::S> a;
  SepW<typename P::WT, typename P::BT> w[3];
  DenseW<typename P::WT, typename P::BT> agg[2];
  DenseW<typename P::WT, typename P::BT> llr[kMaxHeads][2];
  DenseW<typename P::WT, typename P::BT> chest[2];
  int tail;
  int m;
  int strips;
  int order_rev;
  int inline_combine;
  int norm_pre;
  int pair;
  int gz;
};

static_assert(strip_lds_bytes<P16>(true) == 160 * 1024, "P16 strip image + WB = LDS");
static_assert(P16::FO <= 8 * P16::R && P16M::FO <= 8 * P16M::R && P16S::FO <= 8 * P16S::R,
              "the conv3 of a strip must run in one round");

__device__ __forceinline__ int sre(int f, int t) { return (f * kT + t) * kDS; }
__device__ __forceinline__ size_t srow(int b, int u, int f, int t, int U, int F) {
  return ((((size_t)b * U + u) * F + f) * kT + t) * kDS;
}

template <class P, int CINP, int COUTP, bool GZIN = false, class Epi, class Post>
__device__ __forceinline__ void run_layer(char* X, char* WB, const SepW<typename P::WT, typename P::BT>& w,
                                          int in_off, int pos_lo, int pos_hi, Epi&& epi_of, Post&& post,
                                          const GZ* gz = nullptr, bool skip = false) {
  constexpr int R0 = strip_slots<P>();
  if constexpr (P::WLDS) {
    WLds<P, CINP, COUTP> ws{WB};
    conv_layer<P, CINP, COUTP, GZIN>(X, R0, in_off, pos_lo, pos_hi, ws, epi_of(ws), post, gz, skip);
  } else {
    WGlb<P, CINP, COUTP> ws{w};
    conv_layer<P, CINP, COUTP>(X, R0, in_off, pos_lo, pos_hi, ws, epi_of(ws), post, nullptr, skip);
  }
}

static_assert(P16::FO + 4 <= 8 * P16::R && P16M::FO + 4 <= 8 * P16M::R && P16S::FO + 4 <= 8 * P16S::R,
              "P16 layers must run in one round (weights are swapped after it)");

template <class P, int CINP>
struct DLds {
  const char* base;
  const float* bias_p;
  static constexpr int NQ = CINP * 2 / 16;
  __device__ typename P::DV afrag(int n, int kc, int lane, int g) const {
    typedef const __attribute__((address_space(3))) char lds_char;
    typedef const __attribute__((address_space(3))) half8 lds_half8;
    unsigned a = (unsigned)(size_t)(lds_char*)base + (unsigned)lds_off<NQ>(0, lane & 15, kc * 4 + g);
    asm("" : "+v"(a));
    return *reinterpret_cast<lds_half8*>((lds_char*)(size_t)a + n * (kTP * NQ * 16));
  }
  __device__ typename P::Acc bias_acc(int n, int g) const { return P::bias_acc(bias_p, n, g); }
};
template <class P, int CINP>
struct DGlb {
  DenseW<typename P::WT, typename P::BT> w;
  __device__ typename P::DV afrag(int n, int kc, int lane, int g) const {
    return P::ld_w(w.w + (16 * n + (lane & 15)) * CINP + kc * P::KC + g * P::CPL);
  }
  __device__ typename P::Acc bias_acc(int n, int g) const { return P::bias_acc(w.b, n, g); }
};

template <int CINP, int COUTP>
__device__ __forceinline__ void stage_dense(char* dst, float* bias_dst, const DenseW<_Float16, float>& w) {
  constexpr int NQ = CINP * 2 / 16;
  constexpr int NW = COUTP * NQ;
  for (int idx = nrx_tid(); idx < NW; idx += 512) {
    const int co = idx / NQ, q = idx % NQ;
    *reinterpret_cast<intx4*>(dst + lds_off<NQ>(co >> 4, co & 15, q)) =
        *reinterpret_cast<const intx4*>(w.w + co * CINP + q * 8);
  }
  for (int idx = nrx_tid(); idx < COUTP; idx += 512) bias_dst[idx] = w.b[idx];
}

template <class P, int NT>
struct CFrag {
  static constexpr int NKC = NT * 16 / P::KC;
  typename P::DV b[NKC];
  __device__ CFrag() {}
  __device__ CFrag(const typename P::Real (&v)[NT][4]) {
    if constexpr (P::KC == 32) {
#pragma unroll
      for (int kc = 0; kc < NKC; ++kc)
        b[kc] = typename P::DV{(_Float16)v[2 * kc][0], (_Float16)v[2 * kc][1], (_Float16)v[2 * kc][2],
                               (_Float16)v[2 * kc][3], (_Float16)v[2 * kc + 1][0], (_Float16)v[2 * kc + 1][1],
                               (_Float16)v[2 * kc + 1][2], (_Float16)v[2 * kc + 1][3]};
    } else {
#pragma unroll
      for (int kc = 0; kc < NKC; ++kc)
        b[kc] = typename P::DV{(double)v[kc][0], (double)v[kc][1], (double)v[kc][2], (double)v[kc][3]};
    }
  }
  static constexpr bool kPackedRelu = P::KC == 32;
  __device__ void relu() {
    if constexpr (kPackedRelu) {
#pragma unroll
      for (int kc = 0; kc < NKC; ++kc) b[kc] = __builtin_elementwise_max(b[kc], typename P::DV{});
    }
  }
};

template <class P, int NT, int COUTP, int NR, class WS>
__device__ __forceinline__ void dense_rows(const CFrag<P, NT> (&in)[NR], const WS& ws, int lane, int g,
                                           typename P::Real (&out)[NR][COUTP / 16][4], bool relu) {
  using Real = typename P::Real;
  constexpr int NKC = CFrag<P, NT>::NKC;
#pragma unroll
  for (int n = 0; n < COUTP / 16; ++n) {
    typename P::Acc acc[NR];
    const typename P::Acc bn = ws.bias_acc(n, g);
#pragma unroll
    for (int kc = 0; kc < NKC; ++kc) {
      const typename P::DV a = ws.afrag(n, kc, lane, g);
#pragma unroll
      for (int r = 0; r < NR; ++r) acc[r] = P::mma_v(a, in[r].b[kc], kc == 0 ? bn : acc[r]);
    }
#pragma unroll
    for (int r = 0; r < NR; ++r)
#pragma unroll
      for (int j = 0; j < 4; ++j) {
        const Real v = (Real)acc[r][j];
        out[r][n][j] = relu ? (v > (Real)0 ? v : (Real)0) : v;
      }
  }
}

__device__ __forceinline__ int head_w1(int h) { return h * (kHeadSlot + 1024); }
__device__ __forceinline__ int head_w2(int h) { return head_w1(h) + 16 * 1024; }
__device__ __forceinline__ int head_b1(int h) { return head_w1(h) + kHeadSlot; }
__device__ __forceinline__ int head_b2(int h) { return head_b1(h) + 512; }

#ifndef NRX_RO_STRAIGHT
#define NRX_RO_STRAIGHT 1
#endif

template <class P, class WS, int CHP, int TAILM, class LT = ColGeneric>
struct EpiConv3 {
  using S = typename P::S;
  using Real = typename P::Real;
  static constexpr int NTS = kDSP / 16;
  template <int R>
  struct PrefT {
    std::conditional_t<sizeof(S) == 2, half4, Real[4]> prev[R][NTS];
  };
  static constexpr bool kNoBarrier = !readout_tail(TAILM);
  static constexpr bool kNextHook = TAILM == TAIL_AGG && P::WLDS;
  static constexpr bool kNextHookRO = TAILM == TAIL_READOUT_WB && P::WLDS;
  static constexpr int kEarlyRow = 8;
  const BlockParams<P>* prm;
  char* X;
  char* WB;
  WS ws;
  int b, u, f_start, pos_hi, mode;
  Real wm;
  bool first;
  Real act_h;
  int nb, nu, nfs;
  int pos_lo = 0;
  const BlockParams<P>* nprm = nullptr;
  const int* ndone = nullptr;
  int* nflag = nullptr;

  __device__ bool next_ready() const { return nb >= 0 && (!ndone || *nflag); }

  template <int R>
  __device__ void settle(PrefT<R>& pf) {
    if constexpr (sizeof(S) == 2) {
#pragma unroll
      for (int r = 0; r < R; ++r)
#pragma unroll
        for (int n = 0; n < NTS; ++n) asm volatile("" : "+v"(pf.prev[r][n]));
    }
    asm volatile("" : "+v"(act_h));
  }
  __device__ void next_hook();

  __device__ bool row_ok(int p, int t) const {
    if constexpr (LT::kLean) return p < prm->a.F && t < kT;
    return p >= pos_lo && p < pos_hi && f_start + p < prm->a.F && t < kT;
  }

  template <int R>
  __device__ void prefetch(PrefT<R>& pf, int p0, int t, int g) const {
    const auto& a = prm->a;
    if constexpr (LT::kLean) {
      static_assert(sizeof(S) == 2, "lean variants are f16");
      if (mode != 0) {
#pragma unroll
        for (int r = 0; r < R; ++r)
#pragma unroll
          for (int n = 0; n < NTS; ++n) pf.prev[r][n] = half4{0, 0, 0, 0};
        return;
      }
      const char* plane = reinterpret_cast<const char*>(a.s_in + srow(b, u, 0, 0, a.U, a.F));
      __builtin_amdgcn_sched_barrier(0);
#pragma unroll
      for (int r = 0; r < R; ++r) {
        const bool ok = row_ok(p0 + r, t);
        const unsigned ro = (unsigned)sre(ok ? p0 + r : 0, ok ? t : 0) * 2u + 8u * (unsigned)g;
#pragma unroll
        for (int n = 0; n < NTS; ++n) {
          unsigned o = ro + 32u * n;
          if (n == NTS - 1) o = ro + (g >= 2 ? 32u * n - 8u * (unsigned)(g - 1) : 32u * n);
          pf.prev[r][n] = *reinterpret_cast<const half4*>(plane + o);
        }
      }
      __builtin_amdgcn_sched_barrier(0);
      return;
    }
    const bool need = mode == 0 || !first;
#pragma unroll
    for (int r = 0; r < R; ++r) {
      const bool ok = need && row_ok(p0 + r, t);
      const S* src = (mode == 0 ? a.s_in : a.s_out) + srow(b, u, 0, 0, a.U, a.F) +
                     sre(ok ? f_start + p0 + r : 0, ok ? t : 0);
#pragma unroll
      for (int n = 0; n < NTS; ++n) {
        if constexpr (sizeof(S) == 2) {
          const int c0 = 16 * n + 4 * g;
          half4 h4 = half4{0, 0, 0, 0};
          if (ok && c0 < kDS) h4 = *reinterpret_cast<const half4*>(src + c0);
          pf.prev[r][n] = h4;
        } else {
#pragma unroll
          for (int j = 0; j < 4; ++j) {
            const int co = 16 * n + P::co(g, j);
            pf.prev[r][n][j] = (ok && co < kDS) ? (Real)src[co] : (Real)0;
          }
        }
      }
    }
  }

  __device__ void pre() const {
    if constexpr (P::WLDS) {
      if constexpr (TAILM == TAIL_READOUT_WB) {
        __syncthreads();
      } else if constexpr (TAILM == TAIL_READOUT) {
        const auto& a = prm->a;
        for (int h = 1; h < a.H; ++h) {
          stage_dense<kDSP, kHID>(X + head_w1(h), reinterpret_cast<float*>(X + head_b1(h)), prm->llr[h][0]);
          stage_dense<kHID, 16>(X + head_w2(h), reinterpret_cast<float*>(X + head_b2(h)), prm->llr[h][1]);
        }
        __syncthreads();
      }
    }
  }

  __device__ static void store_row16(S* dst, const Real (&v)[NTS][4], bool ok, int g) {
    unsigned w[NTS][2];
#pragma unroll
    for (int n = 0; n < NTS; ++n) {
      const half2 lo = half2{(S)v[n][0], (S)v[n][1]}, hi = half2{(S)v[n][2], (S)v[n][3]};
      w[n][0] = __builtin_bit_cast(unsigned, lo);
      w[n][1] = __builtin_bit_cast(unsigned, hi);
    }
#pragma unroll
    for (int n = 0; n < NTS; n += 2)
#pragma unroll
      for (int d = 0; d < 2; ++d) {
        const auto x = __builtin_amdgcn_permlane16_swap(w[n][d], w[n + 1][d], false, false);
        w[n][d] = x[0];
        w[n + 1][d] = x[1];
      }
    if (!ok) return;
    const int ck = 2 * (g & 1) + (g >> 1);
#pragma unroll
    for (int n = 0; n < NTS; n += 2) {
      const int chunk = 2 * n + ck;
      if (chunk * 8 < kDS)
        *reinterpret_cast<intx4*>(dst + chunk * 8) = intx4{(int)w[n][0], (int)w[n][1], (int)w[n + 1][0], (int)w[n + 1][1]};
    }
  }

  template <int NT16>
  __device__ __forceinline__ void store_f32(float* dst, const Real (&o)[NT16][4], int g, int nvalid) const {
#pragma unroll
    for (int n = 0; n < NT16; ++n) {
      if constexpr (sizeof(S) == 2) {
        const int c0 = 16 * n + 4 * g;
        if (c0 + 3 < nvalid && (nvalid & 3) == 0) {
          *reinterpret_cast<floatx4*>(dst + c0) = floatx4{(float)o[n][0], (float)o[n][1], (float)o[n][2], (float)o[n][3]};
          continue;
        }
      }
#pragma unroll
      for (int j = 0; j < 4; ++j) {
        const int co = 16 * n + P::co(g, j);
        if (co < nvalid) dst[co] = (float)o[n][j];
      }
    }
  }

  __device__ void head_lds(int hh, bool ch, const char*& w1, const float*& b1, const char*& w2,
                           const float*& b2) const {
    if constexpr (TAILM == TAIL_READOUT_WB) {
      w1 = WB + (ch ? kHW1C : 0);
      b1 = reinterpret_cast<const float*>(WB + kHB1 + (ch ? kHID * 4 : 0));
      b2 = reinterpret_cast<const float*>(WB + kHB2 + (ch ? 16 * 4 : 0));
      w2 = WB + kHW2 + (ch ? (LT::kLean ? 4 : prm->a.bits_max) * 256 : 0);
    } else {
      w1 = X + head_w1(hh);
      b1 = reinterpret_cast<const float*>(X + head_b1(hh));
      w2 = X + head_w2(hh);
      b2 = reinterpret_cast<const float*>(X + head_b2(hh));
    }
  }

  template <int NO, int RB, class W1, class W2>
  __device__ __forceinline__ void head_rows(const CFrag<P, NTS> (&sb)[RB], const W1& w1, const W2& w2, int lane,
                                            int g, Real (&o)[RB][NO][4]) const {
    Real hdn[RB][kHID / 16][4];
    using HF = CFrag<P, kHID / 16>;
    dense_rows<P, NTS, kHID, RB>(sb, w1, lane, g, hdn, !HF::kPackedRelu);
    HF hb[RB];
#pragma unroll
    for (int r = 0; r < RB; ++r) {
      hb[r] = HF(hdn[r]);
      hb[r].relu();
    }
    dense_rows<P, kHID / 16, NO * 16, RB>(hb, w2, lane, g, o, false);
  }

  template <int R>
  __device__ void run(const typename P::Acc (&acc)[R][NTS], const PrefT<R>& pf, int p0, int t, int g,
                      int r_lo, int r_hi) const {
    if (r_lo >= r_hi) return;
    stamp(6);
    const auto& a = prm->a;
    const int F = a.F, U = a.U;
    const int lane = nrx_tid() & 63;
    typename P::Acc accw[R][NTS];
#pragma unroll
    for (int r = 0; r < R; ++r)
#pragma unroll
      for (int n = 0; n < NTS; ++n) accw[r][n] = acc[r][n];
    if constexpr (LT::kLean) {
      if (mode == 1 && wm != (Real)1) {
#pragma unroll
        for (int r = 0; r < R; ++r)
#pragma unroll
          for (int n = 0; n < NTS; ++n)
#pragma unroll
            for (int j = 0; j < 4; ++j) accw[r][n][j] *= wm;
      }
    }
    Real sv[R][NTS][4];
#pragma unroll
    for (int r = 0; r < R; ++r)
#pragma unroll
      for (int n = 0; n < NTS; ++n)
#pragma unroll
        for (int j = 0; j < 4; ++j) {
          const int co = 16 * n + P::co(g, j);
          Real v = (Real)accw[r][n][j];
          if (!LT::kLean && mode == 1) v *= wm;
          v += (Real)pf.prev[r][n][j];
          if (co >= kDS) v = 0;
          sv[r][n][j] = (Real)(S)v;
        }
    size_t off[R];
    bool ok[R];
#pragma unroll
    for (int r = 0; r < R; ++r) {
      ok[r] = row_ok(p0 + r, t) && !(NRX_ABLATE & 16);
      off[r] = srow(b, u, 0, 0, U, F) + (size_t)(unsigned)sre(ok[r] ? f_start + p0 + r : 0, ok[r] ? t : 0);
    }
    if constexpr (!readout_tail(TAILM)) {
#pragma unroll
      for (int r = 0; r < R; ++r) {
        S* dst = a.s_out + off[r];
        if constexpr (sizeof(S) == 2) {
          store_row16(dst, sv[r], ok[r] && !((NRX_ABLATE & 32) && a.B > 0), g);
        } else {
          if (!ok[r]) continue;
#pragma unroll
          for (int n = 0; n < NTS; ++n)
#pragma unroll
            for (int j = 0; j < 4; ++j) {
              const int co = 16 * n + P::co(g, j);
              if (co < kDS) dst[co] = (S)sv[r][n][j];
            }
        }
      }
    }
    if constexpr (TAILM == TAIL_NONE) return;
    CFrag<P, NTS> sb[R];
#pragma unroll
    for (int r = 0; r < R; ++r) sb[r] = CFrag<P, NTS>(sv[r]);
    if constexpr (TAILM == TAIL_AGG) {
      Real hdn[R][kAGG / 16][4], sp[R][NTS][4];
      const Real act = act_h;
      CFrag<P, kAGG / 16> hb[R];
      if constexpr ((NRX_ABLATE & 128) != 0 && P::WLDS) {
#pragma unroll
        for (int r = 0; r < R; ++r)
#pragma unroll
          for (int n = 0; n < NTS; ++n)
#pragma unroll
            for (int j = 0; j < 4; ++j) sp[r][n][j] = sv[r][n][j];
      } else if constexpr (P::WLDS) {
        DLds<P, kDSP> w1{WB + 16 * 1024, reinterpret_cast<const float*>(WB + kWTailBias)};
        DLds<P, kAGG> w2{WB + 24 * 1024, reinterpret_cast<const float*>(WB + kWTailBias + kAGG * 4)};
        dense_rows<P, NTS, kAGG, R>(sb, w1, lane, g, hdn, !CFrag<P, kAGG / 16>::kPackedRelu);
#pragma unroll
        for (int r = 0; r < R; ++r) {
          hb[r] = CFrag<P, kAGG / 16>(hdn[r]);
          hb[r].relu();
        }
        dense_rows<P, kAGG / 16, kDSP, R>(hb, w2, lane, g, sp, false);
      } else {
        dense_rows<P, NTS, kAGG, R>(sb, DGlb<P, kDSP>{prm->agg[0]}, lane, g, hdn, !CFrag<P, kAGG / 16>::kPackedRelu);
#pragma unroll
        for (int r = 0; r < R; ++r) {
          hb[r] = CFrag<P, kAGG / 16>(hdn[r]);
          hb[r].relu();
        }
        dense_rows<P, kAGG / 16, kDSP, R>(hb, DGlb<P, kAGG>{prm->agg[1]}, lane, g, sp, false);
      }
#pragma unroll
      for (int r = 0; r < R; ++r) {
        S* dst = a.a_out + off[r];
        if constexpr (sizeof(S) == 2) {
          Real spa[NTS][4];
#pragma unroll
          for (int n = 0; n < NTS; ++n)
#pragma unroll
            for (int j = 0; j < 4; ++j) spa[n][j] = sp[r][n][j] * act;
          store_row16(dst, spa, ok[r] && !((NRX_ABLATE & 64) && a.B > 0), g);
        } else {
          if (!ok[r]) continue;
#pragma unroll
          for (int n = 0; n < NTS; ++n)
#pragma unroll
            for (int j = 0; j < 4; ++j) {
              const int co = 16 * n + P::co(g, j);
              if (co < kDS) dst[co] = (S)(sp[r][n][j] * act);
            }
        }
      }
    } else {
      constexpr int RB = R % 2 == 0 ? 2 : (R == 3 ? 3 : 1);
#pragma unroll
      for (int r0 = 0; r0 < R; r0 += RB) {
        CFrag<P, NTS> sbr[RB];
        bool okr[RB];
#pragma unroll
        for (int r = 0; r < RB; ++r) {
          sbr[r] = sb[r0 + r];
          okr[r] = ok[r0 + r];
        }
        readout_rows<RB>(sbr, okr, p0 + r0, t, g);
      }
    }
  }

  template <int RB>
  __device__ void readout_rows(const CFrag<P, NTS> (&sbr)[RB], const bool (&okr)[RB], int p0r, int t, int g) const {
    const auto& a = prm->a;
    const int F = a.F, U = a.U;
    const int lane = nrx_tid() & 63;
    auto one_head = [&](int hh, bool ch) __attribute__((always_inline)) {
      if (!ch) {
        Real o[RB][1][4];
        if constexpr (P::WLDS) {
          const char *w1, *w2;
          const float *b1, *b2;
          head_lds(hh, false, w1, b1, w2, b2);
          head_rows<1, RB>(sbr, DLds<P, kDSP>{w1, b1}, DLds<P, kHID>{w2, b2}, lane, g, o);
        } else {
          head_rows<1, RB>(sbr, DGlb<P, kDSP>{prm->llr[hh][0]}, DGlb<P, kHID>{prm->llr[hh][1]}, lane, g, o);
        }
        if constexpr (LT::kLean) {
          char* plane = reinterpret_cast<char*>(a.llr + ((size_t)b * U + u) * F * kT * LT::kBits);
          const int nb = a.head_bits[0];
#pragma unroll
          for (int r = 0; r < RB; ++r) {
            if (okr[r] && g == 0)
              *reinterpret_cast<floatx4*>(plane + (unsigned)((p0r + r) * kT + t) * (unsigned)(LT::kBits * 4)) =
                  floatx4{nb > 0 ? (float)o[r][0][0] : 0.f, nb > 1 ? (float)o[r][0][1] : 0.f,
                          nb > 2 ? (float)o[r][0][2] : 0.f, nb > 3 ? (float)o[r][0][3] : 0.f};
          }
          return;
        }
#pragma unroll
        for (int r = 0; r < RB; ++r) {
          if (!okr[r]) continue;
          const int f = f_start + p0r + r;
          float* dst = a.llr + ((((size_t)hh * a.llr_B + b) * U + u) * F + f) * kT * a.bits_max + t * a.bits_max;
          if constexpr (sizeof(S) == 2) {
            if (a.bits_max == 4) {
              const int nb = a.head_bits[hh];
              if (g == 0)
                *reinterpret_cast<floatx4*>(dst) =
                    floatx4{nb > 0 ? (float)o[r][0][0] : 0.f, nb > 1 ? (float)o[r][0][1] : 0.f,
                            nb > 2 ? (float)o[r][0][2] : 0.f, nb > 3 ? (float)o[r][0][3] : 0.f};
              continue;
            }
          }
#pragma unroll
          for (int j = 0; j < 4; ++j) {
            const int co = P::co(g, j);
            if (co < a.bits_max) dst[co] = co < a.head_bits[hh] ? (float)o[r][0][j] : 0.f;
          }
        }
      } else {
        Real o[RB][CHP / 16][4];
        if constexpr (P::WLDS) {
          const char *w1, *w2;
          const float *b1, *b2;
          head_lds(hh, true, w1, b1, w2, b2);
          head_rows<CHP / 16, RB>(sbr, DLds<P, kDSP>{w1, b1}, DLds<P, kHID>{w2, b2}, lane, g, o);
        } else {
          head_rows<CHP / 16, RB>(sbr, DGlb<P, kDSP>{prm->chest[0]}, DGlb<P, kHID>{prm->chest[1]}, lane, g, o);
        }
        if constexpr (LT::kLean) {
          static_assert(CHP == 16 && LT::kA2 == 8, "lean ChEst store");
          char* plane = reinterpret_cast<char*>(a.h_ref + ((size_t)b * U + u) * F * kT * LT::kA2);
#pragma unroll
          for (int r = 0; r < RB; ++r) {
            if (okr[r] && g < 2)
              *reinterpret_cast<floatx4*>(plane + (unsigned)((p0r + r) * kT + t) * (unsigned)(LT::kA2 * 4) +
                                          16u * (unsigned)g) =
                  floatx4{(float)o[r][0][0], (float)o[r][0][1], (float)o[r][0][2], (float)o[r][0][3]};
          }
          return;
        }
        const int A2 = 2 * a.A;
#pragma unroll
        for (int r = 0; r < RB; ++r) {
          if (!okr[r]) continue;
          const int f = f_start + p0r + r;
          store_f32<CHP / 16>(a.h_ref + ((((size_t)b * U + u) * F + f) * kT + t) * A2, o[r], g, A2);
        }
      }
    };
    if constexpr (LT::kLean) {
      __builtin_amdgcn_sched_barrier(0);
      one_head(0, false);
      __builtin_amdgcn_sched_barrier(0);
      if constexpr (LT::kHref) one_head(1, true);
      __builtin_amdgcn_sched_barrier(0);
    } else if (NRX_RO_STRAIGHT && a.H == 1) {
      one_head(0, false);
      if (a.h_ref) one_head(1, true);
    } else {
      for (int hh = 0; hh <= a.H; ++hh) {
        const bool ch = hh == a.H;
        if (ch && !a.h_ref) break;
        one_head(hh, ch);
      }
    }
  }

  template <int R>
  __device__ void state_frags(const typename P::Acc (&acc)[R][NTS], const PrefT<R>& pf, int p0, int t, int g,
                              CFrag<P, NTS> (&sb)[R], bool (&ok)[R]) const {
#pragma unroll
    for (int r = 0; r < R; ++r) {
      Real sv[NTS][4];
#pragma unroll
      for (int n = 0; n < NTS; ++n)
#pragma unroll
        for (int j = 0; j < 4; ++j) {
          const int co = 16 * n + P::co(g, j);
          Real v = (Real)acc[r][n][j];
          if (mode == 1) v *= wm;
          v += (Real)pf.prev[r][n][j];
          if (co >= kDS) v = 0;
          sv[n][j] = (Real)(S)v;
        }
      sb[r] = CFrag<P, NTS>(sv);
      ok[r] = row_ok(p0 + r, t) && !(NRX_ABLATE & 16);
    }
  }
};

#ifndef NRX_PREFETCH_W
#define NRX_PREFETCH_W 1
#endif
constexpr bool kPrefetchW = NRX_PREFETCH_W != 0;

template <class P>
struct FusedNext {
  const BlockParams<P>* nprm;
  const int* ndone;
  int nneed;
  int* nflag;
  int* head;
  int jnn;
};


template <class P, int CINP, int CHP, int TAILM, bool GZIN = false>
__device__ __forceinline__ void strip_block(const BlockParams<P>& prm, char* X, char* WB, int b, int u,
                                            int f_start, int mode, typename P::Real wm, bool first, int nb = -1,
                                            int nu = 0, int nfs = 0, FusedNext<P>* fn = nullptr,
                                            const GZ* gz = nullptr, int* psig = nullptr, bool skip = false) {
  constexpr int R0 = strip_slots<P>();
  const int F = prm.a.F;
  if (fn && nrx_tid() == 0) fn->jnn = atomicAdd(fn->head, 1);
  const bool fast = P::WLDS && skip;
  if (!fast) {
    SepStage<kHID, kHID> nx;
    if constexpr (P::WLDS && kPrefetchW) nx.load(prm.w[1]);
    run_layer<P, CINP, kHID, GZIN>(X, WB, prm.w[0], 0, 1, R0 - 1, [&](auto ws) {
      return EpiInPlace<P, kHID, decltype(ws), GZIN ? 0 : 2>{X, 0, R0 - 1, f_start, F, ws};
    }, [&]() {
      if constexpr (P::WLDS) {
        if constexpr (!kPrefetchW) nx.load(prm.w[1]);
        nx.store(WB);
      }
      if (psig) asm volatile("s_waitcnt vmcnt(0)" ::: "memory");
    }, gz, skip);
  }
  if (psig && nrx_tid() == 0) __hip_atomic_fetch_add(psig, 1, __ATOMIC_RELAXED, __HIP_MEMORY_SCOPE_AGENT);
  stamp(2);
  if (fast) {
    if constexpr (P::WLDS) {
      SepStage<kHID, kDSP> nx;
      DenseStage<kDSP, kAGG> d1;
      DenseStage<kAGG, kDSP> d2;
      nx.load(prm.w[2]);
      if constexpr (TAILM == TAIL_AGG) {
        d1.load(prm.agg[0]);
        d2.load(prm.agg[1]);
      }
      int pv = 0;
      const bool poll = fn && fn->ndone && nrx_tid() == 0;
      if (poll) {
        pv = __hip_atomic_load(fn->ndone, __ATOMIC_RELAXED, __HIP_MEMORY_SCOPE_AGENT);
        asm volatile("buffer_inv sc1" ::: "memory");
      }
      nx.store(WB);
      if constexpr (TAILM == TAIL_AGG) {
        d1.store(WB + 16 * 1024, reinterpret_cast<float*>(WB + kWTailBias));
        d2.store(WB + 24 * 1024, reinterpret_cast<float*>(WB + kWTailBias + kAGG * 4));
      }
      if (poll) {
        asm volatile("s_waitcnt vmcnt(0)" ::: "memory");
        *fn->nflag = pv >= fn->nneed;
      }
      __syncthreads();
    }
  } else {
    SepStage<kHID, kDSP> nx;
    DenseStage<kDSP, kAGG> d1;
    DenseStage<kAGG, kDSP> d2;
    auto ld = [&]() {
      if constexpr (P::WLDS) {
        nx.load(prm.w[2]);
        if constexpr (TAILM == TAIL_AGG) {
          d1.load(prm.agg[0]);
          d2.load(prm.agg[1]);
        }
      }
    };
    if constexpr (P::WLDS && kPrefetchW) ld();
    int pv = 0;
    const bool poll = fn && fn->ndone && nrx_tid() == 0;
    if (poll) {
      pv = __hip_atomic_load(fn->ndone, __ATOMIC_RELAXED, __HIP_MEMORY_SCOPE_AGENT);
      asm volatile("buffer_inv sc1" ::: "memory");
    }
    run_layer<P, kHID, kHID>(X, WB, prm.w[1], 1, 2, R0 - 2, [&](auto ws) {
      return EpiInPlace<P, kHID, decltype(ws)>{X, 1, R0 - 2, f_start, F, ws};
    }, [&]() {
      if (poll) {
        asm volatile("s_waitcnt vmcnt(0)" ::: "memory");
        *fn->nflag = pv >= fn->nneed;
      }
      if constexpr (P::WLDS) {
        if constexpr (!kPrefetchW) ld();
        nx.store(WB);
        if constexpr (TAILM == TAIL_AGG) {
          d1.store(WB + 16 * 1024, reinterpret_cast<float*>(WB + kWTailBias));
          d2.store(WB + 24 * 1024, reinterpret_cast<float*>(WB + kWTailBias + kAGG * 4));
        }
      }
    }, nullptr, skip);
  }
  stamp(3);
  {
    DenseStage<kDSP, kHID> l1, c1;
    DenseStage<kHID, 16> l2;
    DenseStage<kHID, CHP> c2;
    auto ld = [&]() {
      if constexpr (P::WLDS) {
        l1.load(prm.llr[0][0]);
        l2.load(prm.llr[0][1]);
        c1.load(prm.chest[0]);
        c2.load(prm.chest[1]);
      }
    };
    if constexpr (P::WLDS && readout_tail(TAILM) && kPrefetchW) ld();
    run_layer<P, kHID, kDSP>(X, WB, prm.w[2], 2, kHalo, R0 - kHalo, [&](auto ws) {
      EpiConv3<P, decltype(ws), CHP, TAILM> e{&prm, X, WB, ws, b, u, f_start, R0 - kHalo, mode, wm, first,
                                             (typename P::Real)prm.a.active[(size_t)b * prm.a.U + u],
                                             nb, nu, nfs};
      if (fn && fn->ndone) {
        e.nprm = fn->nprm;
        e.ndone = fn->ndone;
        e.nflag = fn->nflag;
      }
      return e;
    }, [&]() {
      if constexpr (P::WLDS && TAILM == TAIL_READOUT_WB) {
        if constexpr (!kPrefetchW) ld();
        const int nb2 = prm.a.bits_max;
        l1.store(WB, reinterpret_cast<float*>(WB + kHB1));
        c1.store(WB + kHW1C, reinterpret_cast<float*>(WB + kHB1 + kHID * 4));
        l2.store(WB + kHW2, reinterpret_cast<float*>(WB + kHB2), nb2);
        c2.store(WB + kHW2 + nb2 * 256, reinterpret_cast<float*>(WB + kHB2 + 16 * 4), 2 * prm.a.A);
      } else if constexpr (P::WLDS && TAILM == TAIL_READOUT) {
        if constexpr (!kPrefetchW) ld();
        const int H = prm.a.H;
        l1.store(X + head_w1(0), reinterpret_cast<float*>(X + head_b1(0)));
        l2.store(X + head_w2(0), reinterpret_cast<float*>(X + head_b2(0)));
        c1.store(X + head_w1(H), reinterpret_cast<float*>(X + head_b1(H)));
        c2.store(X + head_w2(H), reinterpret_cast<float*>(X + head_b2(H)));
      }
    }, nullptr, skip);
  }
}

template <int A2P>
constexpr int init_cinp(int kc) {
  int c = (2 * A2P + 2 + kc - 1) / kc * kc;
  int p = 32;
  while (p < c) p *= 2;
  return p;
}

__device__ __forceinline__ double sq4(double acc, floatx4 v) {
  acc = __builtin_fma((double)v[0], (double)v[0], acc);
  acc = __builtin_fma((double)v[1], (double)v[1], acc);
  acc = __builtin_fma((double)v[2], (double)v[2], acc);
  return __builtin_fma((double)v[3], (double)v[3], acc);
}

constexpr int kNormPre = 4;
struct NormPre {
  floatx4 v[kNormPre];
};
__device__ __forceinline__ NormPre slot_norm_issue(const float* y, int nq) {
  const floatx4* yq = reinterpret_cast<const floatx4*>(y);
  NormPre p;
#pragma unroll
  for (int k = 0; k < kNormPre; ++k) {
    const int i = nrx_tid() + 512 * k;
    p.v[k] = yq[i < nq ? i : nq - 1];
  }
  return p;
}
__device__ __forceinline__ double slot_norm(const NormPre& pre, const float* y, int nq, double* red) {
  const floatx4* yq = reinterpret_cast<const floatx4*>(y);
  double acc = 0.0;
#pragma unroll
  for (int k = 0; k < kNormPre; ++k)
    if (nrx_tid() + 512 * k < nq) acc = sq4(acc, pre.v[k]);
  for (int i = nrx_tid() + 512 * kNormPre; i < nq; i += 512) {
    const floatx4 v = yq[i];
    acc = sq4(acc, v);
  }
#pragma unroll
  for (int m = 32; m >= 1; m >>= 1) acc += __shfl_xor(acc, m);
  if ((nrx_tid() & 63) == 0) red[nrx_tid() >> 6] = acc;
  __syncthreads();
  double tot = 0.0;
#pragma unroll
  for (int w = 0; w < 8; ++w) tot += red[w];
  const double ms = tot / (double)(4 * nq);
  return ms > 0.0 ? 1.0 / sqrt(ms) : 0.0;
}

static __global__ __launch_bounds__(1024) void k_norm(const float* __restrict__ y, int nq, double* __restrict__ norm) {
  __shared__ double red[16];
  const floatx4* yq = reinterpret_cast<const floatx4*>(y) + (size_t)blockIdx.x * nq;
  double acc = 0.0;
  for (int i = nrx_tid(); i < nq; i += 1024) {
    const floatx4 v = yq[i];
    acc = sq4(acc, v);
  }
#pragma unroll
  for (int m = 32; m >= 1; m >>= 1) acc += __shfl_xor(acc, m);
  if ((nrx_tid() & 63) == 0) red[nrx_tid() >> 6] = acc;
  __syncthreads();
  if (nrx_tid() == 0) {
    double tot = 0.0;
    for (int w = 0; w < 16; ++w) tot += red[w];
    const double ms = tot / (double)(4 * nq);
    norm[blockIdx.x] = ms > 0.0 ? 1.0 / sqrt(ms) : 0.0;
  }
}

#ifndef NRX_INIT_ORDER
#define NRX_INIT_ORDER 1
#endif

template <class P, int A2P, int CHP, int TAILM>
__device__ __forceinline__ void init_user(const BlockParams<P>& prm, char* smem, int b, int u,
                                          int strip, typename P::Real wm, bool first, int nb = -1, int nu = 0,
                                          int nfs = 0, FusedNext<P>* fn = nullptr) {
  __shared__ double red[8];
  using S = typename P::S;
  using Real = typename P::Real;
  constexpr int CINP = init_cinp<A2P>(P::KC);
  constexpr int R0 = strip_slots<P>();
  constexpr int NQZ = CINP * (int)sizeof(S) / 16;
  const auto& a = prm.a;
  const int F = a.F, U = a.U, A2 = 2 * a.A;
  const int f0 = strip * P::FO;
  const int f_start = f0 - kHalo;
  char* X = smem;
  char* WB = smem + R0 * slot_pitch<P>();
  auto pad_zero = [&]() __attribute__((always_inline)) {
    if constexpr (sizeof(S) == 2 && CINP < kHID) {
      constexpr int NQ = kHID * (int)sizeof(S) / 16;
      for (int idx = nrx_tid(); idx < R0 * 2 * NQ; idx += 512) {
        const int q = idx % NQ, tt = kT + (idx / NQ) % 2, lf = idx / (2 * NQ);
        *reinterpret_cast<intx4*>(X + xoff<P, NQ>(lf, tt, q)) = intx4{0, 0, 0, 0};
      }
    }
  };
  if (!a.masking && wm == (Real)0) {
    if constexpr (sizeof(S) == 2) {
      constexpr int NQ = kHID * (int)sizeof(S) / 16;
      for (int idx = nrx_tid(); idx < R0 * 2 * NQ; idx += 512) {
        const int q = idx % NQ, tt = kT + (idx / NQ) % 2, lf = idx / (2 * NQ);
        *reinterpret_cast<intx4*>(X + xoff<P, NQ>(lf, tt, q)) = intx4{0, 0, 0, 0};
      }
    }
    if constexpr (sizeof(S) == 2) {
      const int lf = nrx_tid() / kTP, tt = nrx_tid() % kTP, f = f_start + lf;
      if (a.pe16 && lf >= kHalo && lf < kHalo + P::FO && lf < R0 && tt < kT && f >= 0 && f < F) {
        const float2 pv = *reinterpret_cast<const float2*>(a.pe + (((size_t)u * F + f) * kT + tt) * 2);
// ... 796 lines not shown
```

### neural_rx_amd/csrc/nrx_geom.h

```cpp
#pragma once
#include "nrx_internal.h"

namespace nrx {

enum Tail { TAIL_NONE = -1, TAIL_AGG = 0, TAIL_READOUT = 1, TAIL_READOUT_WB = 2 };
constexpr bool readout_tail(int t) { return t == TAIL_READOUT || t == TAIL_READOUT_WB; }

constexpr unsigned kGzOob = kGzRange;
template <class P>
constexpr int slot_pitch() { return kTP * kHID * (int)sizeof(typename P::S); }

constexpr int kWAlloc = 160 * 1024 - 30 * kTP * kHID * 2;
static_assert(kWBytes <= kWAlloc, "layer weight image exceeds the LDS left by the strip image");
__host__ __device__ constexpr bool heads_fit_wb(int bits_max, int chp, int a2 = 0) {
  return bits_max <= 16 && a2 <= chp && chp <= 32 && kHW2 + 256 * (bits_max + chp) <= kWAlloc;
}

template <class P>
constexpr int strip_slots() { return P::FO + 2 * kHalo; }
template <class P>
constexpr int strip_lds_bytes(bool heads_wb = false) {
  return strip_slots<P>() * slot_pitch<P>() + (P::WLDS ? (heads_wb ? kWAlloc : kWBytes) : 0);
}
constexpr int kHeadSlot = 24 * 1024;
constexpr int kNormFusedMaxQ = 8192;

constexpr int kFusedMaxStages = 12;
constexpr int kFusedLds = 160 * 1024 - 256;
template <class P>
constexpr int fused_lds() {
  return strip_lds_bytes<P>(true) > kFusedLds ? kFusedLds : strip_lds_bytes<P>(true);
}
constexpr int kFusedMaxB = 65536;
constexpr int kFusedMaxLS = 20;
constexpr int kFusedMaxUsers = 8;

constexpr int kRrFO = 16;
constexpr int kRrSlots = kRrFO + 2 * kHalo;
constexpr int kRrExRow = 4 * kT * 4 * 16;
constexpr int kRrExChunk = kT * 4 * 16;
constexpr int kRrExRows = 14;
constexpr int kRrW1 = 0;
constexpr int kRrW2 = kRrW1 + kWTailBias;
constexpr int kRrW3 = kRrW2 + kWTailBias;
constexpr int kRrNeg = kRrW3 + kWBytes;
constexpr int kRrNegOff = 128;
constexpr int kRrZero = kRrNeg + 768;
constexpr int kRrX = kRrZero + kRrExChunk * 4;
constexpr int kRrLds = kRrX + kRrExRows * kRrExRow;
static_assert(kRrLds <= 160 * 1024, "RR LDS plan exceeds the CU's LDS");
__host__ __device__ constexpr bool rr_heads_fit(int bits_max, int chp, int a2) {
  return bits_max <= 16 && a2 <= chp && chp <= 32 && kHW2 + 256 * (bits_max + chp) <= kRrExRows * kRrExRow;
}

constexpr int kColRO = 6;
constexpr int kColPos = 8 * kColRO;
constexpr int kColFO = kColPos - 4;
constexpr int kColRed = kRrLds;
constexpr int kColLds = kColRed + 64;
static_assert(kColLds <= 160 * 1024, "column LDS plan exceeds the CU's LDS");
__host__ __device__ constexpr int col_strips(int F) { return F <= kColPos ? 1 : (F + kColFO - 1) / kColFO; }
constexpr int kColMaxStages = 1 + kMaxIt;
enum ColVariant { COL_GENERIC = 0, COL_LEAN = 1, COL_LEAN_NO_HREF = 2 };
struct ColGeneric {
  static constexpr bool kLean = false, kHref = true;
};
template <bool HREF>
struct ColLean {
  static constexpr bool kLean = true, kHref = HREF;
  static constexpr int kBits = 4, kA2 = 8;
};
#ifndef NRX_COL_LEAN
#define NRX_COL_LEAN 1
#endif

}
```

### neural_rx_amd/csrc/nrx_internal.h

```cpp
#pragma once
#include <stddef.h>
#include <stdint.h>

#include "../../include/nrx.h"

namespace nrx {

constexpr int kT = 14;
constexpr int kTP = 16;
constexpr int kDS = 56;
constexpr int kDSP = 64;
constexpr int kHID = 128;
constexpr int kAGG = 64;
constexpr int kUPD_CINP = 128;
constexpr int kMaxInit = 8;
constexpr int kMaxIt = 8;
constexpr int kInlineUsers = 2;
constexpr int kMaxHeads = 8;
constexpr int kMaxUsers = 16;
constexpr int kHalo = 3;
constexpr unsigned kGzRange = 0x40000000u;
constexpr int init_a2p(int num_rx_ant) { return 2 * num_rx_ant <= 8 ? 8 : (2 * num_rx_ant <= 16 ? 16 : 32); }

inline size_t align256(size_t x) { return (x + 255) & ~size_t(255); }
struct Carver {
  char* base;
  size_t off = 0;
  explicit Carver(void* ws) : base((char*)ws) {}
  template <class T>
  T* take(size_t count) {
    T* p = base ? reinterpret_cast<T*>(base + off) : nullptr;
    off += align256(count * sizeof(T));
    return p;
  }
  size_t bytes() const { return off; }
};

constexpr int kTPImg = 16;
__host__ __device__ constexpr int swz_q(int nq, int t) {
  return nq >= 16 ? (t & 15) : (nq == 8 ? ((t >> 1) & 7) : (nq == 4 ? ((t >> 2) & 3) : 0));
}
__host__ __device__ constexpr int lds_img_off(int nq, int row, int t, int q) {
  return ((row * kTPImg + t) * nq + (q ^ swz_q(nq, t))) * 16;
}
constexpr int kWPw = kHID * kHID * 2;
constexpr int kWDw = 9 * kHID * 2;
constexpr int kWBias = kWPw + kWDw;
constexpr int kWTailBias = kWBias + kHID * 4;
constexpr int kWBytes = kWTailBias + 2 * kAGG * 4;
constexpr int kHW1C = 16 * 1024;
constexpr int kHB1 = 32 * 1024;
constexpr int kHB2 = kHB1 + 2 * kHID * 4;
constexpr int kHW2 = kHB2 + (16 + 32) * 4;

template <class WT, class BT>
struct SepW {
  const WT* dw;
  const WT* pw;
  const BT* b;
};

template <class WT, class BT>
struct DenseW {
  const WT* w;
  const BT* b;
};

template <class WT, class BT>
struct ModelW {
  SepW<WT, BT> init[kMaxInit][3];
  DenseW<WT, BT> agg[kMaxIt][2];
  SepW<WT, BT> upd[kMaxIt][3];
  DenseW<WT, BT> llr[kMaxHeads][2];
  DenseW<WT, BT> chest[2];
};

template <class WT, class BT, class S>
struct FwdArgs {
  int B, U, F, A, M, H;
  int llr_B;
  int init_cinp;
  int num_init;
  int masking;
  int use_h;
  int bits_max;
  int head_bits[kMaxHeads];
  const float* y;
  const float* pe;
  const float* h_hat;
  const float* active;
  const float* mcs_mask;
  float* llr;
  float* h_ref;
  double* norm;
  S* s_in;
  S* s_out;
  S* a;
  S* a_out;
  const char* ws_base;
  unsigned ws_bytes;
  S* pe16;
};

struct FusedCtl {
  void* sync;
  int spin_limit;
  int dbg_err;
};
struct Sched {
  int mask;
  int fused;
  int small = 1;
};
constexpr int kSchedRrAgg = 1, kSchedRrRo = 2, kSchedColAgg = 4, kSchedColRo = 8, kSchedColInit = 16;
constexpr int kSchedColFwd = 32;
constexpr int kSchedColWide = 64;
constexpr int kSchedMax = 127;
constexpr int kSchedDefault = kSchedColInit | kSchedColAgg | kSchedColRo | kSchedRrAgg;
constexpr int kFusedSpinLimit = 1 << 21;

enum KernelId {
  K_NORM = 0, K_INIT = 1, K_UPDATE = 2, K_FUSED = 3, K_UPDATE_RR = 4, K_COMBINE = 5, K_UPDATE_COL = 6, K_INIT_COL = 7,
  K_FWD_COL = 8, K_COUNT = 9
};

struct Prof {
  virtual void begin(int kid, void* stream) = 0;
  virtual void end(int kid, void* stream) = 0;
  virtual ~Prof() {}
};

enum FwdPath { PATH_P16S, PATH_P16M, PATH_P16, PATH_FWD_COL, PATH_KFWD0, PATH_KFWD1, PATH_KFWD2, PATH_P64 };
enum StageKind { STAGE_STRIP, STAGE_RR, STAGE_COL };
struct StagePlan {
  int kind;
  int kid;
  int tail;
  int chp;
  int one;
  int pair;
  int items, strips;
  int grid, lds;
  int order_rev;
  int variant;
};
struct FwdPlan {
  int path;
  int num_init, num_it;
  int norm_pre, gz, inline_combine;
  int grid, lds, a2p, heads_x, nq;
  StagePlan st[kMaxInit + kMaxIt];
  bool one_launch() const { return path >= PATH_FWD_COL && path <= PATH_KFWD2; }
  bool combine_launches() const { return !inline_combine && !one_launch(); }
};
FwdPlan plan_forward(const FwdArgs<_Float16, float, _Float16>& a, int num_it, const Sched& sc, int cus, int xccs);
FwdPlan plan_forward(const FwdArgs<double, double, float>& a, int num_it);

hipError_t launch_aerial_tables(const int32_t* ofdm_pos, const int32_t* sc_pos, int U, int nsym, int npil, int T,
                                int F, int32_t* nn, float* pe, hipStream_t st);
hipError_t launch_aerial_inputs(const float* y_re, const float* y_im, const float* h_re, const float* h_im,
                                const int32_t* nn, int B, int U, int F, int T, int A, int nsym, int npil, float* y,
                                float* h, hipStream_t st);
hipError_t launch_y_layout(const float* y0, const float* y1, int layout, int B, int F, int T, int A, float* y,
                           hipStream_t st);
hipError_t launch_aerial_llr(const float* llr, int B, int U, int F, int T, int bits_max, int bits, float* out,
                             hipStream_t st);

inline size_t gen_grid_elems(const nrx_gen_desc& d) {
  return (size_t)d.batch * d.num_tx * d.num_subcarriers * kT;
}
struct GenCfo {
  double eps_max[16];
  int constant;
  int fft_size;
  int h_with_phase;
  double* eps_out;
};
struct GenPlan {
  nrx_gen_desc d;
  nrx_gen_chan c;
  GenCfo cfo;
  bool cfo_on;
  const nrx_gen_dmrs* dmrs;
  const nrx_gen_cir* cir;
  const nrx_gen_td* td;
  const nrx_gen_tc* tc;
  const double* no_slot;
  size_t stage, pilots, cir_ws, total;
};
void gen_layout(GenPlan& p);
hipError_t launch_generate(const GenPlan& p, const nrx_gen_out& o, void* ws, hipStream_t st);
struct GenWs;
size_t gen_workspace_bytes(const nrx_gen_desc& d, GenWs* w, void* base);
size_t dmrs_workspace_bytes(const nrx_gen_desc& d);
hipError_t launch_export_taps(const nrx_gen_desc& d, const nrx_gen_chan& c, float* a_out, float* tau_out, void* ws,
                              hipStream_t st);

size_t cir_workspace_bytes(const nrx_gen_desc& d);
hipError_t launch_cir_rx(const nrx_gen_desc& d, const nrx_gen_cir& c, const double* x, void* ws,
                         const double* no_slot, float* y, float* h, float* y_re, float* y_im, hipStream_t st);

hipError_t launch_ls_estimate(const nrx_ls_io& io, hipStream_t st);
hipError_t launch_count_errors(const nrx_count_io& c, hipStream_t st);

size_t cfo_workspace_bytes(const nrx_gen_desc& d);
hipError_t launch_cfo_apply(const nrx_gen_desc& d, const GenCfo& c, const double* x, const float* active, double* xp,
                            hipStream_t st);
hipError_t launch_cfo_h_phase(const nrx_gen_desc& d, const GenCfo& c, float* h, hipStream_t st);
hipError_t launch_cfo_estimate(const nrx_cfo_io& io, hipStream_t st);
hipError_t launch_cfo_rotate(const nrx_cfo_io& io, hipStream_t st);

hipError_t launch_ofdm(const nrx_ofdm_io& io, bool modulate, hipStream_t st);
inline int64_t slot_samples(const int32_t* cp_length, int fft_size, int num_symbols) {
  int64_t n = 0;
  for (int t = 0; t < num_symbols; ++t) n += cp_length[t] + fft_size;
  return n;
}
template <class Stage>
nrx_ofdm_io stage_ofdm(const nrx_gen_desc& d, const Stage& s, int streams, void* grid, void* samples) {
  nrx_ofdm_io io{};
  io.batch = d.batch, io.num_streams = streams, io.grid_subcarriers = d.num_subcarriers, io.num_symbols = kT;
  io.fft_size = s.fft_size, io.first_bin = s.first_bin;
  for (int t = 0; t < kT; ++t) io.cp_length[t] = s.cp_length[t];
  io.precision = NRX_OFDM_F64, io.grid_layout = NRX_OFDM_GRID_PLANAR;
  io.num_samples = slot_samples(s.cp_length, s.fft_size, kT);
  io.grid = grid, io.samples = samples;
  return io;
}
size_t td_workspace_bytes(const nrx_gen_desc& d, const nrx_gen_td& td);
hipError_t launch_td_apply(const nrx_gen_desc& d, const nrx_gen_td& td, const double* x, void* ws, hipStream_t st);
hipError_t launch_td_h_phase(const nrx_gen_desc& d, const nrx_gen_td& td, float* h, hipStream_t st);

hipError_t launch_time_channel(const nrx_tc_io& io, hipStream_t st);
int tc_resolve_l_max(const nrx_gen_desc& d, const nrx_gen_chan& c, const nrx_gen_tc& tc);
size_t tc_workspace_bytes(const nrx_gen_desc& d, const nrx_gen_tc& tc);
hipError_t launch_tc_taps(const nrx_gen_desc& d, const nrx_gen_chan& c, const nrx_gen_tc& tc, const double* tau,
                          const double* spdp, double* gt, void* ws, hipStream_t st);
hipError_t launch_tc_rx(const nrx_gen_desc& d, const nrx_gen_chan& c, const nrx_gen_tc& tc, const double* x,
                        const double* tau, const double* gt, void* ws, const double* no_slot, float* y, float* h,
                        float* y_re, float* y_im, hipStream_t st);

hipError_t launch_lmmse(const nrx_lmmse_io& io, hipStream_t st);

size_t kbest_workspace_bytes(const nrx_kbest_io& io);
hipError_t launch_kbest(const nrx_kbest_io& io, void* ws, hipStream_t st);

size_t cov_workspace_bytes(const nrx_cov_io& io);
hipError_t launch_cov_accumulate(const nrx_cov_io& io, void* ws, hipStream_t st);
size_t cov_space_workspace_bytes(const nrx_cov_space_io& io);
hipError_t launch_cov_space(const nrx_cov_space_io& io, void* ws, hipStream_t st);
hipError_t launch_chest_lmmse(const nrx_chest_io& io, hipStream_t st);
hipError_t launch_chest_lin(const nrx_chest_io& io, hipStream_t st);
size_t chest3_workspace_bytes(const nrx_chest3_io& io);
hipError_t launch_chest_lmmse3(const nrx_chest3_io& io, void* ws, hipStream_t st);

constexpr int kSoftFS = NRX_SOFT_STRIP;
size_t llr_stats_workspace_bytes(const nrx_llr_stats_io& io);
hipError_t launch_llr_stats(const nrx_llr_stats_io& io, void* ws, hipStream_t st);
size_t nmse_workspace_bytes(const nrx_nmse_io& io);
hipError_t launch_chest_nmse(const nrx_nmse_io& io, void* ws, hipStream_t st);

struct LdpcPlan {
  int G;
  int threads;
  int lds_bytes;
  bool msg_lds;
};
struct LdpcDev {
  int mb, nb, z, kb, num_edges;
  LdpcPlan plan;
  const int* row_ptr;
  const int* edges;
};
LdpcPlan ldpc_plan(int nb, int z, int num_edges);
hipError_t ldpc_setup();
hipError_t launch_ldpc_decode(const LdpcDev& d, const nrx_ldpc_io& io, void* ws, hipStream_t st);
hipError_t launch_ldpc_gather(const nrx_ldpc_gather_io& io, hipStream_t st);
hipError_t launch_ldpc_count(const nrx_ldpc_count_io& io, hipStream_t st);

size_t train_workspace_bytes(const nrx_desc& d, const nrx_train_io& io);
hipError_t launch_train_grad(const nrx_desc& d, const nrx_train_io& io, bool accumulate, int batch_total, void* ws,
                             hipStream_t st);
hipError_t launch_adam(const nrx_adam_io& io, double c1, double c2, hipStream_t st);

hipError_t launch_llr_demap(const float* llr, int B, int U, int F, int T, int bits_stride, int bits,
                            const int32_t* data_re, int n_data, float* out, hipStream_t st);

}
```

### neural_rx_amd/csrc/nrx_k_col.hip

```cpp
#include "nrx_device.inc"
#include "nrx_launch.inc"

namespace nrx {

#include "nrx_rr.inc"
#include "nrx_col.inc"

#ifdef NRX_STAMPS
static void col_stamp_select(hipStream_t st) {
  static int launch_no = 0;
  static const int sel = getenv("NRX_STAMP_COL") ? atoi(getenv("NRX_STAMP_COL")) : -1;
  const int on = launch_no++ == sel;
  (void)hipMemcpyToSymbolAsync(HIP_SYMBOL(g_nrx_stamp_on), &on, sizeof(int), 0, hipMemcpyHostToDevice, st);
}
#else
static void col_stamp_select(hipStream_t) {}
#endif

hipError_t launch_init_col(const BlockParams<P16>& bp, const StagePlan& sp, hipStream_t st) {
  const int items = sp.items, grid = sp.grid;
  col_stamp_select(st);
  const bool agg = sp.tail == TAIL_AGG;
  if (sp.variant != COL_GENERIC) {
    if (!sp.one || !agg) return hipErrorInvalidValue;
    k_init_col<TAIL_AGG, ColLean<true>><<<grid, 512, sp.lds, st>>>(bp, items);
  } else if (sp.one) {
    if (agg) k_init_col<TAIL_AGG><<<grid, 512, sp.lds, st>>>(bp, items);
    else k_init_col<TAIL_NONE><<<grid, 512, sp.lds, st>>>(bp, items);
  } else {
    if (agg) k_init_col_multi<TAIL_AGG><<<grid, 512, sp.lds, st>>>(bp, items);
    else k_init_col_multi<TAIL_NONE><<<grid, 512, sp.lds, st>>>(bp, items);
  }
  return hipGetLastError();
}

hipError_t launch_update_col(const BlockParams<P16>& bp, const StagePlan& sp, hipStream_t st) {
  const int items = sp.items, grid = sp.grid, L = sp.lds;
  const bool ch32 = sp.chp == 32, one = sp.one;
  col_stamp_select(st);
  if (sp.variant != COL_GENERIC) {
    if (!one || ch32) return hipErrorInvalidValue;
    if (sp.tail != TAIL_READOUT_WB) k_update_col<16, TAIL_AGG, ColLean<true>><<<grid, 512, L, st>>>(bp, items);
    else if (sp.variant == COL_LEAN) k_update_col<16, TAIL_READOUT_WB, ColLean<true>><<<grid, 512, L, st>>>(bp, items);
    else k_update_col<16, TAIL_READOUT_WB, ColLean<false>><<<grid, 512, L, st>>>(bp, items);
  } else if (sp.tail == TAIL_READOUT_WB) {
    if (ch32) {
      if (one) k_update_col<32, TAIL_READOUT_WB><<<grid, 512, L, st>>>(bp, items);
      else k_update_col_multi<32, TAIL_READOUT_WB><<<grid, 512, L, st>>>(bp, items);
    } else {
      if (one) k_update_col<16, TAIL_READOUT_WB><<<grid, 512, L, st>>>(bp, items);
      else k_update_col_multi<16, TAIL_READOUT_WB><<<grid, 512, L, st>>>(bp, items);
    }
  } else {
    if (ch32) {
      if (one) k_update_col<32, TAIL_AGG><<<grid, 512, L, st>>>(bp, items);
      else k_update_col_multi<32, TAIL_AGG><<<grid, 512, L, st>>>(bp, items);
    } else {
      if (one) k_update_col<16, TAIL_AGG><<<grid, 512, L, st>>>(bp, items);
      else k_update_col_multi<16, TAIL_AGG><<<grid, 512, L, st>>>(bp, items);
    }
  }
  return hipGetLastError();
}

hipError_t launch_fwd_col(const Args16& args, const Model16& W, const FwdPlan& pl, const FusedCtl& fc, hipStream_t st,
                          Prof* prof) {
  ColFwdParams fp{};
  fp.sync = reinterpret_cast<FusedSync*>(fc.sync);
  fp.nst = pl.num_init + pl.num_it;
  fp.nq = pl.nq;
  fp.spin_limit = fc.spin_limit;
  fp.dbg_err = fc.dbg_err;
  norm_prepass(args, pl, st, prof);
  for (int s = 0; s < fp.nst; ++s) {
    BlockParams<P16>& bp = fp.st[s];
    plan_stage(bp, args, W, pl.num_it, s, TAIL_READOUT_WB);
    bp.inline_combine = pl.inline_combine;
    bp.norm_pre = pl.norm_pre;
    bp.strips = pl.st[s].strips;
    bp.gz = pl.gz;
  }
  col_stamp_select(st);
  if (prof) prof->begin(K_FWD_COL, st);
  k_fwd_col<16><<<pl.grid, 512, pl.lds, st>>>(fp);
  if (prof) prof->end(K_FWD_COL, st);
  return hipGetLastError();
}

hipError_t setup_col() {
  hipError_t e = hipSuccess;
  auto set = [&](const void* f) {
    const hipError_t r = hipFuncSetAttribute(f, hipFuncAttributeMaxDynamicSharedMemorySize, kColLds);
    if (r != hipSuccess) e = r;
  };
  set((const void*)k_init_col<TAIL_AGG>);
  set((const void*)k_init_col<TAIL_NONE>);
  set((const void*)k_init_col_multi<TAIL_AGG>);
  set((const void*)k_init_col_multi<TAIL_NONE>);
  set((const void*)k_update_col<16, TAIL_AGG>);
  set((const void*)k_update_col<32, TAIL_AGG>);
  set((const void*)k_update_col<16, TAIL_READOUT_WB>);
  set((const void*)k_update_col<32, TAIL_READOUT_WB>);
  set((const void*)k_update_col_multi<16, TAIL_AGG>);
  set((const void*)k_update_col_multi<32, TAIL_AGG>);
  set((const void*)k_update_col_multi<16, TAIL_READOUT_WB>);
  set((const void*)k_update_col_multi<32, TAIL_READOUT_WB>);
  set((const void*)k_fwd_col<16>);
  set((const void*)k_init_col<TAIL_AGG, ColLean<true>>);
  set((const void*)k_update_col<16, TAIL_AGG, ColLean<true>>);
  set((const void*)k_update_col<16, TAIL_READOUT_WB, ColLean<true>>);
  set((const void*)k_update_col<16, TAIL_READOUT_WB, ColLean<false>>);
  return e;
}

}

#ifdef NRX_STAMPS
extern "C" int nrx_debug_col_stamps(void* out, int n) {
  return (int)hipMemcpyFromSymbol(out, HIP_SYMBOL(nrx::g_nrx_rr_stamps), (size_t)n * 64 * 8, 0, hipMemcpyDeviceToHost);
}
#endif
```

### neural_rx_amd/csrc/nrx_launch.inc

```
#pragma once
namespace nrx {

using Args16 = FwdArgs<_Float16, float, _Float16>;
using Model16 = ModelW<_Float16, float>;
hipError_t run_tier_p16(const Args16& a, const Model16& W, const FwdPlan& pl, hipStream_t st, Prof* prof);
hipError_t run_tier_p16m(const Args16& a, const Model16& W, const FwdPlan& pl, hipStream_t st, Prof* prof);
hipError_t run_tier_p16s(const Args16& a, const Model16& W, const FwdPlan& pl, hipStream_t st, Prof* prof);
hipError_t run_tier_p64(const FwdArgs<double, double, float>& a, const ModelW<double, double>& W, const FwdPlan& pl,
                        hipStream_t st, Prof* prof);
hipError_t setup_tier_p16(), setup_tier_p16m(), setup_tier_p16s(), setup_tier_p64();
hipError_t launch_kforward_m0(int a2p, const FusedParams<P16>& fp, int grid, hipStream_t st);
hipError_t launch_kforward_m1(int a2p, const FusedParams<P16>& fp, int grid, hipStream_t st);
hipError_t launch_kforward_m2(int a2p, const FusedParams<P16>& fp, int grid, hipStream_t st);
hipError_t setup_kforward_m0(), setup_kforward_m1(), setup_kforward_m2();
hipError_t launch_update_rr(const BlockParams<P16>& bp, const StagePlan& sp, hipStream_t st);
hipError_t setup_update_rr();
hipError_t launch_init_col(const BlockParams<P16>& bp, const StagePlan& sp, hipStream_t st);
hipError_t launch_update_col(const BlockParams<P16>& bp, const StagePlan& sp, hipStream_t st);
hipError_t launch_fwd_col(const Args16& args, const Model16& W, const FwdPlan& pl, const FusedCtl& fc, hipStream_t st,
                          Prof* prof);
hipError_t setup_col();

template <class P>
static void plan_stage(BlockParams<P>& bp, const FwdArgs<typename P::WT, typename P::BT, typename P::S>& args,
                       const ModelW<typename P::WT, typename P::BT>& W, int num_it, int s, int ro_tail) {
  const int i = s - args.num_init;
  const bool last = i == num_it - 1;
  bp.a = args;
  if (i >= 0 && i % 2 == 0) {
    std::swap(bp.a.s_in, bp.a.s_out);
    std::swap(bp.a.a, bp.a.a_out);
  }
  for (int l = 0; l < 3; ++l) bp.w[l] = i < 0 ? W.init[s][l] : W.upd[i][l];
  bp.m = i < 0 ? s : 0;
  bp.tail = i < 0 ? (s == args.num_init - 1 ? TAIL_AGG : TAIL_NONE) : (last ? ro_tail : TAIL_AGG);
  for (int k = 0; k < 2; ++k)
    bp.agg[k] = last ? DenseW<typename P::WT, typename P::BT>{} : W.agg[i < 0 ? 0 : i + 1][k];
  for (int h = 0; h < args.H; ++h) {
    bp.llr[h][0] = W.llr[h][0];
    bp.llr[h][1] = W.llr[h][1];
  }
  bp.chest[0] = W.chest[0];
  bp.chest[1] = W.chest[1];
}

template <class A>
static void norm_prepass(const A& args, const FwdPlan& pl, hipStream_t st, Prof* prof) {
  if (!pl.norm_pre) return;
  if (prof) prof->begin(K_NORM, st);
  k_norm<<<args.B, 1024, 0, st>>>(args.y, args.F * kT * 2 * args.A / 4, args.norm);
  if (prof) prof->end(K_NORM, st);
}

#ifdef NRX_STAMPS
static void stamp_select(int launch, hipStream_t st) {
  static const int sel = getenv("NRX_STAMP_LAUNCH") ? atoi(getenv("NRX_STAMP_LAUNCH")) : 0;
  const int on = launch == sel;
  (void)hipMemcpyToSymbolAsync(HIP_SYMBOL(g_nrx_stamp_on), &on, sizeof(int), 0, hipMemcpyHostToDevice, st);
  (void)hipStreamSynchronize(st);
}
#else
static void stamp_select(int, hipStream_t) {}
#endif

template <class P>
struct Launch {
  using A = FwdArgs<typename P::WT, typename P::BT, typename P::S>;
  using MW = ModelW<typename P::WT, typename P::BT>;

  static hipError_t setup() {
    hipError_t e = hipSuccess;
    auto set = [&](const void* f, bool heads_wb = false) {
      hipError_t r = hipFuncSetAttribute(f, hipFuncAttributeMaxDynamicSharedMemorySize, strip_lds_bytes<P>(heads_wb));
      if (r != hipSuccess) e = r;
    };
#define NRX_SET_INIT(A2P)                                     \
    set((const void*)k_init<P, A2P, TAIL_NONE>);              \
    set((const void*)k_init<P, A2P, TAIL_AGG>);
    NRX_SET_INIT(8) NRX_SET_INIT(16) NRX_SET_INIT(32)
#undef NRX_SET_INIT
    set((const void*)k_update<P, 16, TAIL_AGG>);
    set((const void*)k_update<P, 16, TAIL_READOUT>);
    set((const void*)k_update<P, 32, TAIL_AGG>);
    set((const void*)k_update<P, 32, TAIL_READOUT>);
    if constexpr (P::WLDS) {
      set((const void*)k_update<P, 16, TAIL_READOUT_WB>, true);
      set((const void*)k_update<P, 32, TAIL_READOUT_WB>, true);
    }
    return e;
  }

  template <int A2P>
  static void launch_init(dim3 grid, int L, hipStream_t st, const BlockParams<P>& bp, bool tail) {
    static_assert(init_cinp<A2P>(P::KC) <= kHID, "StateInit input wider than the strip image");
    if (tail) k_init<P, A2P, TAIL_AGG><<<grid, 512, L, st>>>(bp);
    else k_init<P, A2P, TAIL_NONE><<<grid, 512, L, st>>>(bp);
  }

  static hipError_t launch_stage(const BlockParams<P>& bp, const StagePlan& sp, bool init, hipStream_t st) {
    const dim3 grid(sp.grid);
    const bool ch32 = sp.chp == 32;
    if constexpr (std::is_same<P, P16>::value) {
      if (sp.kind == STAGE_COL) return init ? launch_init_col(bp, sp, st) : launch_update_col(bp, sp, st);
      if (sp.kind == STAGE_RR) return launch_update_rr(bp, sp, st);
    }
    if (init) {
      if (sp.chp == 8) launch_init<8>(grid, sp.lds, st, bp, sp.tail == TAIL_AGG);
      else if (sp.chp == 16) launch_init<16>(grid, sp.lds, st, bp, sp.tail == TAIL_AGG);
      else launch_init<32>(grid, sp.lds, st, bp, sp.tail == TAIL_AGG);
    } else if (sp.tail == TAIL_READOUT_WB) {
      if constexpr (P::WLDS) {
        if (ch32) k_update<P, 32, TAIL_READOUT_WB><<<grid, 512, sp.lds, st>>>(bp);
        else k_update<P, 16, TAIL_READOUT_WB><<<grid, 512, sp.lds, st>>>(bp);
      }
    } else if (sp.tail == TAIL_READOUT) {
      if (ch32) k_update<P, 32, TAIL_READOUT><<<grid, 512, sp.lds, st>>>(bp);
      else k_update<P, 16, TAIL_READOUT><<<grid, 512, sp.lds, st>>>(bp);
    } else {
      if (ch32) k_update<P, 32, TAIL_AGG><<<grid, 512, sp.lds, st>>>(bp);
      else k_update<P, 16, TAIL_AGG><<<grid, 512, sp.lds, st>>>(bp);
    }
    return hipSuccess;
  }

  static hipError_t run(const A& args, const MW& W, const FwdPlan& pl, hipStream_t st, Prof* prof) {
    auto B_ = [&](int k) { if (prof) prof->begin(k, st); };
    auto E_ = [&](int k) { if (prof) prof->end(k, st); };
    BlockParams<P> bp{};
    bp.inline_combine = pl.inline_combine;
    bp.gz = pl.gz;
    norm_prepass(args, pl, st, prof);
    bp.norm_pre = pl.norm_pre;
    auto combine = [&](typename P::S* sp) {
      if (!pl.combine_launches()) return;
      dim3 g((args.F * kT * (kDS / P::EPC) + 255) / 256, args.B);
      B_(K_COMBINE);
      k_combine<P><<<g, 256, 0, st>>>(sp, args.active, args.U, args.F);
      E_(K_COMBINE);
    };
    auto stage = [&](int s) {
      const StagePlan& sp = pl.st[s];
      plan_stage(bp, args, W, pl.num_it, s, TAIL_READOUT);
      bp.strips = sp.strips;
      bp.pair = sp.pair;
      bp.order_rev = sp.order_rev;
      return launch_stage(bp, sp, s < pl.num_init, st);
    };
    B_(pl.st[0].kid);
    for (int m = 0; m < pl.num_init; ++m) {
      if (pl.st[m].kind == STAGE_STRIP) stamp_select(-1 - m, st);
      if (const hipError_t e = stage(m); e != hipSuccess) return e;
    }
    E_(pl.st[0].kid);
    combine(bp.a.a_out);
    for (int i = 0; i < pl.num_it; ++i) {
      const int s = pl.num_init + i;
      B_(pl.st[s].kid);
      stamp_select(i, st);
      if (const hipError_t e = stage(s); e != hipSuccess) return e;
      E_(pl.st[s].kid);
      if (i < pl.num_it - 1) combine(bp.a.a_out);
    }
    return hipGetLastError();
  }
};

template <class P>
static hipError_t run_fused(const Args16& args, const Model16& W, const FwdPlan& pl, const FusedCtl& fc, hipStream_t st,
                            Prof* prof) {
  FusedParams<P> fp{};
  fp.sync = reinterpret_cast<FusedSync*>(fc.sync);
  fp.ninit = pl.num_init;
  fp.nst = pl.num_init + pl.num_it;
  fp.heads_x = pl.heads_x;
  fp.gz = pl.gz;
  fp.nls = 0;
  for (int s = 0; s < fp.ninit; ++s) {
    fp.kind[fp.nls] = 0;
    fp.pidx[fp.nls++] = s;
  }
  for (int i = 0; i < pl.num_it; ++i) {
    if (!pl.inline_combine) {
      fp.kind[fp.nls] = 2;
      fp.pidx[fp.nls++] = fp.ninit + i;
    }
    fp.kind[fp.nls] = 1;
    fp.pidx[fp.nls++] = fp.ninit + i;
  }
  fp.nq = pl.nq;
  fp.spin_limit = fc.spin_limit;
  fp.dbg_err = fc.dbg_err;
  norm_prepass(args, pl, st, prof);
  for (int s = 0; s < fp.nst; ++s) {
    BlockParams<P>& bp = fp.st[s];
    plan_stage(bp, args, W, pl.num_it, s, pl.heads_x ? TAIL_READOUT : TAIL_READOUT_WB);
    bp.inline_combine = pl.inline_combine;
    bp.norm_pre = pl.norm_pre;
    bp.strips = pl.st[s].strips;
  }
#ifdef NRX_STAMPS
  {
    const int on = getenv("NRX_STAMP_FUSED") ? 100 : 0;
    (void)hipMemcpyToSymbolAsync(HIP_SYMBOL(g_nrx_stamp_on), &on, sizeof(int), 0, hipMemcpyHostToDevice, st);
    (void)hipStreamSynchronize(st);
  }
#endif
  if (prof) prof->begin(K_FUSED, st);
  hipError_t e = pl.path == PATH_KFWD0   ? launch_kforward_m0(pl.a2p, fp, pl.grid, st)
                 : pl.path == PATH_KFWD1 ? launch_kforward_m1(pl.a2p, fp, pl.grid, st)
                                         : launch_kforward_m2(pl.a2p, fp, pl.grid, st);
  if (e != hipSuccess) return e;
  if (prof) prof->end(K_FUSED, st);
  return hipGetLastError();
}

}
```

### neural_rx_amd/csrc/nrx_rr.inc

```

#ifndef NRX_RR_ZBRANCH
#define NRX_RR_ZBRANCH 1
#endif


#ifdef NRX_STAMPS
__device__ __forceinline__ void rr_ts(int k, int m) {
  if ((nrx_tid() & 255) == 0 && g_nrx_stamp_on && k < 4 && blockIdx.x < 4096)
    g_nrx_rr_stamps[blockIdx.x][16 * k + 2 * m + (nrx_tid() >> 8)] = __builtin_amdgcn_s_memtime();
}
__device__ __forceinline__ void rr_ts_edge(int e) {
  if (nrx_tid() == 0 && g_nrx_stamp_on && blockIdx.x < 4096) {
    g_nrx_rr_stamps[blockIdx.x][16 * (1 + e) + 14] = __builtin_amdgcn_s_memrealtime();
    if (e) g_nrx_rr_stamps[blockIdx.x][16 * 3 + 14] = __builtin_amdgcn_s_memtime();
  }
}
#else
__device__ __forceinline__ void rr_ts(int, int) {}
__device__ __forceinline__ void rr_ts_edge(int) {}
#endif

__device__ __forceinline__ int rr_r0(int w) { return w < 4 ? 1 + 3 * w : 13 + 2 * (w - 4); }
__device__ __forceinline__ int rr_slot(int w, int side) { return 2 * w + side - 1; }

typedef const __attribute__((address_space(3))) char rr_lds_cchar;
typedef __attribute__((address_space(3))) char rr_lds_char;
typedef const __attribute__((address_space(3))) half8 rr_lds_chalf8;
typedef __attribute__((address_space(3))) half8 rr_lds_half8;
typedef const __attribute__((address_space(3))) floatx4 rr_lds_cfloatx4;
__device__ __forceinline__ unsigned rr_lds_addr(const char* p) { return (unsigned)(size_t)(rr_lds_cchar*)p; }

template <int COUTP>
struct WRr {
  WLds<P16, kHID, COUTP> w;
  unsigned boff;
  __device__ WRr(const char* base, const char* bias_row, int g) : w{base} {
    boff = rr_lds_addr(bias_row) + 16u * (unsigned)g;
    asm("" : "+v"(boff));
  }
  __device__ half8 afrag(int n, int kc, int lane, int g) const { return w.afrag(n, kc, lane, g); }
  __device__ void dw_taps(int kc, int g, half8 (&t)[9]) const { w.dw_taps(kc, g, t); }
  __device__ floatx4 bias_acc(int n, int) const { return *(rr_lds_cfloatx4*)((rr_lds_cchar*)(size_t)boff + 64 * n); }
};

__device__ __forceinline__ unsigned rr_exch_lo(int g, int t) {
  int s = t + 2 * g;
  s = s >= kT ? s - kT : s;
  return (unsigned)((g * kT + s) * 16);
}
__device__ __forceinline__ unsigned rr_zero_lo(int g) {
  return (unsigned)(16 * (g == 0 ? 14 : g == 1 ? 12 : g == 2 ? 8 : 10));
}
static_assert((kRrX - kRrZero) % 256 == 0 && 16 * 15 + 3 * kRrExChunk + 16 <= kRrX - kRrZero,
              "zero slots must share the exchange rows' bank phase and stay inside the zero block");

struct RrNb {
  unsigned top, bot;
};
__device__ __forceinline__ RrNb rr_nb(const char* smem, int wave, int t, int g) {
  const unsigned zero = rr_lds_addr(smem + kRrZero) + rr_zero_lo(g);
  const unsigned lo = rr_exch_lo(g, t);
  RrNb nb;
  nb.top = (t < kT && wave > 0) ? rr_lds_addr(smem + kRrX + rr_slot(wave - 1, 1) * kRrExRow) + lo : zero;
  nb.bot = (t < kT && wave < 7) ? rr_lds_addr(smem + kRrX + rr_slot(wave + 1, 0) * kRrExRow) + lo : zero;
  asm("" : "+v"(nb.top), "+v"(nb.bot));
  return nb;
}
__device__ __forceinline__ half8 rr_ld(unsigned a, int kc) {
  return *(rr_lds_chalf8*)((rr_lds_cchar*)(size_t)a + kc * kRrExChunk);
}

template <int RO, int A, int B, int COUTP, class WS>
__device__ __forceinline__ void rr_pass(const half8 (&in)[RO][4], const RrNb& nb, const WS& ws, int lane, int g,
                                        floatx4 (&acc)[B - A][COUTP / 16]) {
  constexpr int NR = B - A;
  constexpr int NT = COUTP / 16;
  constexpr bool TOP = A == 0, BOT = B == RO;
  static_assert(NR >= 1 && A >= 0 && B <= RO, "rows");
  half8 w[9], xt{}, xb{};
  auto load = [&](int kc) {
    if constexpr (TOP) xt = rr_ld(nb.top, kc);
    if constexpr (BOT) xb = rr_ld(nb.bot, kc);
    ws.dw_taps(kc, g, w);
  };
  load(0);
#pragma unroll
  for (int kc = 0; kc < 4; ++kc) {
    half8 a_cur = ws.afrag(0, kc, lane, g);
    half8 d[NR];
#pragma unroll
    for (int r = 0; r < NR; ++r) {
      const int i = A + r;
      const half8 x0 = i - 1 < 0 ? xt : in[i - 1 < 0 ? 0 : i - 1][kc];
      const half8 x2 = i + 1 >= RO ? xb : in[i + 1 >= RO ? RO - 1 : i + 1][kc];
      d[r] = P16::dw_row(x0, in[i][kc], x2, w);
    }
    dw_fence<NR>(d);
    if (kc + 1 < 4) load(kc + 1);
#pragma unroll
    for (int n = 0; n < NT; ++n) {
      half8 a_nxt = a_cur;
      if (n + 1 < NT) a_nxt = ws.afrag(n + 1, kc, lane, g);
      if (kc == 0) {
        const floatx4 bn = ws.bias_acc(n, g);
#pragma unroll
        for (int r = 0; r < NR; ++r) acc[r][n] = P16::mma_v(a_cur, d[r], bn);
      } else {
#pragma unroll
        for (int r = 0; r < NR; ++r) acc[r][n] = P16::mma_v(a_cur, d[r], acc[r][n]);
      }
      a_cur = a_nxt;
    }
  }
}

template <int RO, int A, int B>
__device__ __forceinline__ void rr_to_own(const floatx4 (&acc)[B - A][8], half8 (&own)[RO][4], int f_own0, int F) {
#pragma unroll
  for (int r = 0; r < B - A; ++r) {
#pragma unroll
    for (int kc = 0; kc < 4; ++kc) {
      const floatx4& a0 = acc[r][2 * kc];
      const floatx4& a1 = acc[r][2 * kc + 1];
      half8 h = half8{(_Float16)a0[0], (_Float16)a0[1], (_Float16)a0[2], (_Float16)a0[3],
                      (_Float16)a1[0], (_Float16)a1[1], (_Float16)a1[2], (_Float16)a1[3]};
      h = __builtin_elementwise_max(h, half8{});
      if constexpr (!NRX_RR_ZBRANCH) {
        const int f = f_own0 + A + r;
        if (f < 0 || f >= F) h = half8{};
      }
      own[A + r][kc] = h;
    }
  }
  if constexpr (!NRX_RR_ZBRANCH) return;
  const int fa = f_own0 + A, fb = f_own0 + B - 1;
  if (__builtin_expect(fa < 0 || fb >= F, 0)) {
#pragma unroll
    for (int r = 0; r < B - A; ++r) {
      const int f = f_own0 + A + r;
      if (f < 0 || f >= F) {
#pragma unroll
        for (int kc = 0; kc < 4; ++kc) own[A + r][kc] = half8{};
      }
    }
  }
}

template <int RO>
__device__ __forceinline__ void rr_write_exch(char* smem, int wave, int t, int g, const half8 (&own)[RO][4]) {
  if (t >= kT) return;
  const unsigned lo = rr_exch_lo(g, t);
  if (wave > 0) {
    const unsigned a = rr_lds_addr(smem + kRrX + rr_slot(wave, 0) * kRrExRow) + lo;
#pragma unroll
    for (int kc = 0; kc < 4; ++kc) *(rr_lds_half8*)((rr_lds_char*)(size_t)a + kc * kRrExChunk) = own[0][kc];
  }
  if (wave < 7) {
    const unsigned a = rr_lds_addr(smem + kRrX + rr_slot(wave, 1) * kRrExRow) + lo;
#pragma unroll
    for (int kc = 0; kc < 4; ++kc) *(rr_lds_half8*)((rr_lds_char*)(size_t)a + kc * kRrExChunk) = own[RO - 1][kc];
  }
}

template <int RO, int A, int B>
__device__ __forceinline__ void rr_layer_own(half8 (&own)[RO][4], const RrNb& nb, const WRr<kHID>& ws, int lane, int g,
                                             int f_own0, int F) {
  floatx4 acc[B - A][8];
  rr_pass<RO, A, B, kHID>(own, nb, ws, lane, g, acc);
  rr_to_own<RO, A, B>(acc, own, f_own0, F);
}

template <int RO, int A, int B, class Epi>
__device__ __forceinline__ void rr_conv3(const half8 (&own)[RO][4], const RrNb& nb, Epi& epi, int lane, int t, int g,
                                         int p0, int kst = 0) {
  typename Epi::template PrefT<B - A> pf;
  epi.template prefetch<B - A>(pf, p0, t, g);
  floatx4 acc[B - A][4];
  rr_pass<RO, A, B, kDSP>(own, nb, epi.ws, lane, g, acc);
  rr_ts(kst, 5);
  epi.template settle<B - A>(pf);
  epi.template run<B - A>(acc, pf, p0, t, g, 0, B - A);
}

template <int CHP>
struct RrHeads {
  DenseStage<kDSP, kHID> l1, c1;
  DenseStage<kHID, 16> l2;
  DenseStage<kHID, CHP> c2;
  __device__ __forceinline__ void load(const BlockParams<P16>& prm) {
    l1.load(prm.llr[0][0]);
    l2.load(prm.llr[0][1]);
    c1.load(prm.chest[0]);
    c2.load(prm.chest[1]);
  }
  __device__ __forceinline__ void store(char* WB, const BlockParams<P16>& prm) const {
    const int nb2 = prm.a.bits_max;
    l1.store(WB, reinterpret_cast<float*>(WB + kHB1));
    c1.store(WB + kHW1C, reinterpret_cast<float*>(WB + kHB1 + kHID * 4));
    l2.store(WB + kHW2, reinterpret_cast<float*>(WB + kHB2), nb2);
    c2.store(WB + kHW2 + nb2 * 256, reinterpret_cast<float*>(WB + kHB2 + 16 * 4), 2 * prm.a.A);
  }
};

template <int RO, int A, int B, class Epi, class Hd>
__device__ __forceinline__ void rr_conv3_ro(const half8 (&own)[RO][4], const RrNb& nb, Epi& epi, const Hd& hd,
                                            const BlockParams<P16>& prm, char* X, int lane, int t, int g, int p0,
                                            int kst = 0) {
  constexpr int NR = B - A;
  constexpr int NRA = NR > 0 ? NR : 1;
  typename Epi::template PrefT<NRA> pf;
  floatx4 acc[NRA][4];
  if constexpr (NR > 0) {
    epi.template prefetch<NR>(pf, p0, t, g);
    rr_pass<RO, A, B, kDSP>(own, nb, epi.ws, lane, g, acc);
  }
  rr_ts(kst, 5);
  __syncthreads();
  hd.store(X, prm);
  __syncthreads();
  if constexpr (NR > 0) {
    epi.template settle<NR>(pf);
    epi.template run<NR>(acc, pf, p0, t, g, 0, NR);
  }
}

template <int RO>
__device__ __forceinline__ void rr_gz_first(GZ& gz, const BlockParams<P16>& prm, int wave, int b, int u, int strip) {
  const int lane = nrx_tid() & 63, t = lane & 15, g = lane >> 4;
  const int r0 = rr_r0(wave);
  gz = gz_make(prm, b, u, strip * kRrFO - kHalo, t, g);
#pragma unroll
  for (int i = 0; i < RO + 2; ++i) gz.x0[i] = gz.load(0, gz.row_soff(r0 - 1 + i));
}

template <int RO, int CHP, int TAILM>
__device__ __forceinline__ void rr_item(const BlockParams<P16>& prm, char* smem, int wave, int b, int u, int strip,
                                        int k) {
  rr_ts(k, 0);
  constexpr bool RO3 = RO == 3;
  const int lane = nrx_tid() & 63, t = lane & 15, g = lane >> 4;
  const int r0 = rr_r0(wave);
  const int f_start = strip * kRrFO - kHalo;
  const int F = prm.a.F;
  const int f_own0 = f_start + r0;
  char* X = smem + kRrX;
  const RrNb nb = rr_nb(smem, wave, t, g);
  half8 own[RO][4];
  GZ gz;
  rr_gz_first<RO>(gz, prm, wave, b, u, strip);
  {
    const WRr<kHID> w1(smem + kRrW1, t < kT ? smem + kRrW1 + kWBias : smem + kRrNeg + kRrNegOff, g);
    floatx4 acc[RO][8];
    conv_rows<P16, kUPD_CINP, kHID, RO, WRr<kHID>, true, true>(nullptr, r0, kRrSlots, t, g, lane, w1, acc, &gz);
    rr_to_own<RO, 0, RO>(acc, own, f_own0, F);
  }
  rr_ts(k, 1);
  __syncthreads();
  rr_write_exch<RO>(smem, wave, t, g, own);
  __syncthreads();
  rr_ts(k, 2);
  {
    const WRr<kHID> w2(smem + kRrW2, t < kT ? smem + kRrW2 + kWBias : smem + kRrNeg + kRrNegOff, g);
    if constexpr (RO3) {
      if (wave == 0) rr_layer_own<3, 1, 3>(own, nb, w2, lane, g, f_own0, F);
      else rr_layer_own<3, 0, 3>(own, nb, w2, lane, g, f_own0, F);
    } else {
      if (wave == 7) rr_layer_own<2, 0, 1>(own, nb, w2, lane, g, f_own0, F);
      else rr_layer_own<2, 0, 2>(own, nb, w2, lane, g, f_own0, F);
    }
  }
  rr_ts(k, 3);
  __syncthreads();
  rr_write_exch<RO>(smem, wave, t, g, own);
  __syncthreads();
  rr_ts(k, 4);
  using WS3 = WLds<P16, kHID, kDSP>;
  const WS3 w3{smem + kRrW3};
  char* WB = TAILM == TAIL_READOUT_WB ? X : smem + kRrW3;
  EpiConv3<P16, WS3, CHP, TAILM> epi{&prm, nullptr, WB, w3, b, u, f_start, kRrSlots - kHalo, 0, 1.f, false,
                                     (float)prm.a.active[(size_t)b * prm.a.U + u], -1, 0, 0};
  epi.pos_lo = kHalo;
  if constexpr (TAILM == TAIL_READOUT_WB) {
    RrHeads<CHP> hd;
    hd.load(prm);
    if constexpr (RO3) {
      if (wave == 0) rr_conv3_ro<3, 2, 3>(own, nb, epi, hd, prm, X, lane, t, g, r0 + 2, k);
      else rr_conv3_ro<3, 0, 3>(own, nb, epi, hd, prm, X, lane, t, g, r0, k);
    } else {
      if (wave == 7) rr_conv3_ro<2, 0, 0>(own, nb, epi, hd, prm, X, lane, t, g, r0, k);
      else rr_conv3_ro<2, 0, 2>(own, nb, epi, hd, prm, X, lane, t, g, r0, k);
    }
  } else {
    if constexpr (RO3) {
      if (wave == 0) rr_conv3<3, 2, 3>(own, nb, epi, lane, t, g, r0 + 2, k);
      else rr_conv3<3, 0, 3>(own, nb, epi, lane, t, g, r0, k);
    } else {
      if (wave != 7) rr_conv3<2, 0, 2>(own, nb, epi, lane, t, g, r0, k);
    }
  }
  rr_ts(k, 6);
}

template <int TAILM>
__device__ __forceinline__ void rr_stage_weights(const BlockParams<P16>& prm, char* smem) {
  SepStage<kUPD_CINP, kHID> s1;
  SepStage<kHID, kHID> s2;
  SepStage<kHID, kDSP> s3;
  DenseStage<kDSP, kAGG> d1;
  DenseStage<kAGG, kDSP> d2;
  s1.load(prm.w[0]);
  s2.load(prm.w[1]);
  s3.load(prm.w[2]);
  if constexpr (TAILM == TAIL_AGG) {
    d1.load(prm.agg[0]);
    d2.load(prm.agg[1]);
  }
  s1.store(smem + kRrW1);
  s2.store(smem + kRrW2);
  s3.store(smem + kRrW3);
  if constexpr (TAILM == TAIL_AGG) {
    d1.store(smem + kRrW3 + 16 * 1024, reinterpret_cast<float*>(smem + kRrW3 + kWTailBias));
    d2.store(smem + kRrW3 + 24 * 1024, reinterpret_cast<float*>(smem + kRrW3 + kWTailBias + kAGG * 4));
  }
  for (int i = nrx_tid(); i < 768 / 4; i += 512) reinterpret_cast<float*>(smem + kRrNeg)[i] = -__builtin_inff();
  for (int i = nrx_tid(); i < kRrExChunk * 4 / 16; i += 512) reinterpret_cast<intx4*>(smem + kRrZero)[i] = intx4{0, 0, 0, 0};
}

template <int CHP, int TAILM>
__global__ __launch_bounds__(512) void k_update_rr(BlockParams<P16> prm, int items) {
  extern __shared__ __attribute__((aligned(16))) char smem[];
  rr_ts(0, 7);
  rr_ts_edge(0);
  const int wave = __builtin_amdgcn_readfirstlane(nrx_tid() >> 6);
  rr_stage_weights<TAILM>(prm, smem);
  __syncthreads();
  int k = 0;
  for (int i = blockIdx.x; i < items; i += gridDim.x, ++k) {
    int b, u, strip;
    work_item(i, prm.a.B, prm.a.U, prm.strips, prm.order_rev, b, u, strip);
    if (wave < 4) rr_item<3, CHP, TAILM>(prm, smem, wave, b, u, strip, k);
    else rr_item<2, CHP, TAILM>(prm, smem, wave, b, u, strip, k);
  }
  rr_ts_edge(1);
}
```

Baseline: 1.278 million slots/s.

## Give lean column kernels a compact launch block with precomputed buffer offsets

Moves the lean column init and update kernels into their own translation unit. They now take a compact ColLaunch struct instead of the full BlockParams. The struct carries a precomputed buffer resource, per-slot strides and the weight pointers, so the kernel can build global-load offsets directly, with cheaper item decode for U=1 or 2. This aims to cut kernel-argument size and in-kernel address arithmetic, at the cost of a parallel code path that must stay in sync with the generic one.

```diff
diff --git a/neural_rx_amd/build.py b/neural_rx_amd/build.py
--- a/neural_rx_amd/build.py
+++ b/neural_rx_amd/build.py
@@ -9,7 +9,8 @@
 CSRC = os.path.join(HERE, "csrc")
 LIB = os.path.join(HERE, "lib", "libnrx.so")
 KERNEL_TUS = ["nrx_k_p16.hip", "nrx_k_p16m.hip", "nrx_k_p16s.hip", "nrx_k_p64.hip", "nrx_k_fwd0.hip",
-              "nrx_k_fwd1.hip", "nrx_k_fwd2.hip", "nrx_k_rr.hip", "nrx_k_col.hip", "nrx_dispatch.hip"]
+              "nrx_k_fwd1.hip", "nrx_k_fwd2.hip", "nrx_k_rr.hip", "nrx_k_col.hip", "nrx_k_col_lean.hip",
+              "nrx_dispatch.hip"]
 SOURCES = [os.path.join(CSRC, f) for f in KERNEL_TUS] + [
     os.path.join(CSRC, "nrx_aerial.hip"), os.path.join(CSRC, "nrx_synth.hip"), os.path.join(CSRC, "nrx_lmmse.hip"),
     os.path.join(CSRC, "nrx_kbest.hip"), os.path.join(CSRC, "nrx_chest.hip"),
diff --git a/neural_rx_amd/csrc/nrx_api.cpp b/neural_rx_amd/csrc/nrx_api.cpp
--- a/neural_rx_amd/csrc/nrx_api.cpp
+++ b/neural_rx_amd/csrc/nrx_api.cpp
@@ -10,6 +10,7 @@
 
 #include "../../include/nrx.h"
 #include "nrx_internal.h"
+#include "nrx_geom.h"
 #include "nrx_model.h"
 
 namespace nrx {
@@ -1456,6 +1457,27 @@
   return debug_forward_plan(desc, shape, precision, num_it, sched_mask, fused_mode, cus, xccs, io_flags, out, cap);
 }
 
+int nrx_debug_col_launch_block(const nrx_desc* desc, const nrx_io* io, void* ws, int32_t stage, void* out,
+                               int32_t bytes) {
+  if (!io || !ws || (!out && bytes > 0) || bytes < 0) return fail(NRX_ERR_INVALID_ARG, "null argument");
+  if (int rc = check_desc(desc)) return rc;
+  if (int rc = check_shape(&io->shape)) return rc;
+  if (io->precision != NRX_PREC_F16) return fail(NRX_ERR_INVALID_ARG, "the column launches are f16");
+  if (io->num_it < 1 || io->num_it > desc->num_it) return fail(NRX_ERR_INVALID_ARG, "Invalid number of iterations");
+  if (chunk_slots(&io->shape, io->precision) < io->shape.batch) return fail(NRX_ERR_INVALID_ARG, "a chunked forward");
+  FwdArgs<_Float16, float, _Float16> a{};
+  Sched sc{kSchedDefault, 0};
+  sc.small = 0;
+  const FwdPlan pl = plan_f16(a, desc, io, io->shape.batch, ws, init_padded_cin(desc, 32), sc, 256, 8);
+  if (stage < 0 || stage >= pl.num_init + pl.num_it || pl.one_launch() || pl.st[stage].kind != STAGE_COL ||
+      pl.st[stage].variant == COL_GENERIC)
+    return fail(NRX_ERR_INVALID_ARG, "not a lean column stage");
+  stage_planes(a, stage);
+  const ColLaunch cl = col_launch_block(a, pl.inline_combine, pl.st[stage].order_rev);
+  memcpy(out, &cl, (size_t)bytes < sizeof(cl) ? (size_t)bytes : sizeof(cl));
+  return (int)sizeof(cl);
+}
+
 int nrx_profile_read(nrx_handle* h, int32_t kernel, int64_t* launches, double* total_ms) {
   if (!h || !launches || !total_ms) return fail(NRX_ERR_INVALID_ARG, "null argument");
   if (kernel < 0 || kernel >= K_COUNT) return fail(NRX_ERR_INVALID_ARG, "bad kernel id");
diff --git a/neural_rx_amd/csrc/nrx_col.inc b/neural_rx_amd/csrc/nrx_col.inc
--- a/neural_rx_amd/csrc/nrx_col.inc
+++ b/neural_rx_amd/csrc/nrx_col.inc
@@ -165,15 +165,16 @@
   });
 }
 
-template <int PR, class Epi>
+template <int PR, bool GP = false, class Epi>
 __device__ __forceinline__ void col_conv3(const half8 (&own)[kColRO][4], const RrNb& nb, Epi& epi, int lane, int t,
-                                          int g, int p0) {
+                                          int g, int p0, int gp = 0) {
+  const int gm = GP ? gp : g;
   col_sfor<kColRO / PR>([&](auto J) __attribute__((always_inline)) {
     constexpr int A = decltype(J)::value * PR;
     typename Epi::template PrefT<PR> pf;
     epi.template prefetch<PR>(pf, p0 + A, t, g);
     floatx4 acc[PR][4];
-    col_pass<4, kColRO, A, A + PR, kDSP, false>(own, nb, epi.ws, lane, g, acc);
+    col_pass<4, kColRO, A, A + PR, kDSP, false>(own, nb, epi.ws, lane, gm, acc);
     epi.template settle<PR>(pf);
     epi.template run<PR>(acc, pf, p0 + A, t, g, 0, PR);
   });
@@ -182,9 +183,10 @@
 #ifndef NRX_COL_RB
 #define NRX_COL_RB 3
 #endif
-template <int PR, class Epi>
+template <int PR, bool GP = false, class Epi>
 __device__ __forceinline__ void col_conv3_ro(const half8 (&own)[kColRO][4], const RrNb& nb, Epi& epi, int lane, int t,
-                                             int g, int p0) {
+                                             int g, int p0, int gp = 0) {
+  const int gm = GP ? gp : g;
   constexpr int RB = NRX_COL_RB;
   static_assert(kColRO % RB == 0, "readout row batches");
   CFrag<P16, kDSP / 16> sb[kColRO];
@@ -194,7 +196,7 @@
     typename Epi::template PrefT<PR> pf;
     epi.template prefetch<PR>(pf, p0 + A, t, g);
     floatx4 acc[PR][4];
-    col_pass<4, kColRO, A, A + PR, kDSP, false>(own, nb, epi.ws, lane, g, acc);
+    col_pass<4, kColRO, A, A + PR, kDSP, false>(own, nb, epi.ws, lane, gm, acc);
     epi.template settle<PR>(pf);
     CFrag<P16, kDSP / 16> sbp[PR];
     bool okp[PR];
@@ -214,7 +216,7 @@
       sbr[r] = sb[A + r];
       okr[r] = ok[A + r];
     }
-    epi.template readout_rows<RB>(sbr, okr, p0 + A, t, g);
+    epi.template readout_rows<RB>(sbr, okr, p0 + A, t, gm);
   });
 }
 
@@ -240,6 +242,15 @@
     load_w1(prm);
     load_rest(prm);
   }
+  __device__ __forceinline__ void load_w1(const ColLaunch& cl) { s1.load(cl.w[0]); }
+  __device__ __forceinline__ void load_rest(const ColLaunch& cl) {
+    s2.load(cl.w[1]);
+    s3.load(cl.w[2]);
+    if constexpr (TAILM == TAIL_AGG) {
+      d1.load(cl.tail[0]);
+      d2.load(cl.tail[1]);
+    }
+  }
   __device__ __forceinline__ void store_w1(char* smem) const {
     s1.store(smem + kRrW1);
     for (int i = nrx_tid(); i < 768 / 4; i += 512) reinterpret_cast<float*>(smem + kRrNeg)[i] = -__builtin_inff();
@@ -260,7 +271,7 @@
   }
 };
 
-template <int CHP, int TAILM, bool FIRST = false, class LT = ColGeneric>
+template <int CHP, int TAILM, bool FIRST = false>
 __device__ __forceinline__ void col_upd_item(const BlockParams<P16>& prm, char* smem, int wave, int b, int u, int strip,
                                              int k, ColStage<kUPD_CINP, TAILM>* stage = nullptr) {
   constexpr int PR = 2;
@@ -320,7 +331,7 @@
   }
   __syncthreads();
   col_ts(k, 4);
-  EpiConv3<P16, WS3, CHP, TAILM, LT> epi{&prm, nullptr, WB, w3, b, u, f_start, col_pos_hi(strips), 0, 1.f, false,
+  EpiConv3<P16, WS3, CHP, TAILM> epi{&prm, nullptr, WB, w3, b, u, f_start, col_pos_hi(strips), 0, 1.f, false,
                                      (float)prm.a.active[(size_t)b * prm.a.U + u], -1, 0, 0};
   epi.pos_lo = col_pos_lo(strips);
   if constexpr (TAILM == TAIL_READOUT_WB) col_conv3_ro<NRX_COL_PR3>(own, nb, epi, lane, t, g, p0);
@@ -328,7 +339,7 @@
   col_ts(k, 6);
 }
 
-template <int CHP, int TAILM, bool MULTI, class LT = ColGeneric>
+template <int CHP, int TAILM, bool MULTI>
 __device__ __forceinline__ void col_update_stage(const BlockParams<P16>& prm, int items) {
   extern __shared__ __attribute__((aligned(16))) char smem[];
   rr_ts(0, 7);
@@ -340,7 +351,7 @@
     stage.load_w1(prm);
     int b, u, strip;
     work_item(blockIdx.x, prm.a.B, prm.a.U, prm.strips, prm.order_rev, b, u, strip);
-    col_upd_item<CHP, TAILM, true, LT>(prm, smem, wave, b, u, strip, k, &stage);
+    col_upd_item<CHP, TAILM, true>(prm, smem, wave, b, u, strip, k, &stage);
   }
   if constexpr (MULTI) {
     for (int i = blockIdx.x; i < items; i += gridDim.x, ++k) {
@@ -366,9 +377,9 @@
   rr_ts_edge(1);
 }
 
-template <int CHP, int TAILM, class LT = ColGeneric>
+template <int CHP, int TAILM>
 __global__ __launch_bounds__(512) void k_update_col(BlockParams<P16> prm, int items) {
-  col_update_stage<CHP, TAILM, false, LT>(prm, items);
+  col_update_stage<CHP, TAILM, false>(prm, items);
 }
 template <int CHP, int TAILM>
 __global__ __launch_bounds__(512) void k_update_col_multi(BlockParams<P16> prm, int items) {
@@ -408,13 +419,6 @@
   const char* src;
   const char* pe;
 };
-__device__ __forceinline__ ColInitLane col_init_lane(const FwdArgs<_Float16, float, _Float16>& a, int b, int u, int g) {
-  const size_t plane = (size_t)a.F * kT * 8;
-  const float* y = a.y + (size_t)b * plane;
-  const float* h = a.h_hat + ((size_t)b * a.U + u) * plane;
-  return ColInitLane{reinterpret_cast<const char*>(g == 1 ? h : y),
-                     reinterpret_cast<const char*>(a.pe + (size_t)u * a.F * kT * 2)};
-}
 __device__ __forceinline__ ColInitRow col_init_load_lean(const ColInitLane& ln, int F, int f, int t) {
   const bool ok = f >= 0 && f < F && t < kT;
   const unsigned re = (unsigned)((ok ? f : 0) * kT + (ok ? t : 0));
@@ -439,19 +443,18 @@
   return __builtin_bit_cast(half8, w);
 }
 
-template <int TAILM, bool FIRST = false, class LT = ColGeneric>
+template <int TAILM, bool FIRST = false>
 __device__ __forceinline__ void col_init_item(const BlockParams<P16>& prm, char* smem, int wave, int b, int u,
                                               int strip, int k, ColStage<32, TAILM>* stage = nullptr) {
   constexpr int PR = 2;
-  constexpr bool LEAN = LT::kLean;
   col_ts(k, 0);
   const auto& a = prm.a;
   const int lane = nrx_tid() & 63, t = lane & 15, g = lane >> 4;
   const int p0 = kColRO * wave;
-  const int strips = LEAN ? 1 : prm.strips;
+  const int strips = prm.strips;
   const int f_start = col_fstart(strip, strips);
-  const int F = a.F, A2 = LEAN ? 8 : 2 * a.A;
-  const bool norm_pre = LEAN ? false : prm.norm_pre != 0;
+  const int F = a.F, A2 = 2 * a.A;
+  const bool norm_pre = prm.norm_pre != 0;
   const int f_own0 = f_start + p0;
   const RrNb nb = rr_nb(smem, wave, t, g);
   const float* yslot = a.y + (size_t)b * F * kT * A2;
@@ -459,16 +462,10 @@
   NormPre npre;
   if (!norm_pre) npre = slot_norm_issue(yslot, nqs);
   ColInitRow zr[kColRO + 2];
-  if constexpr (LEAN) {
-    const ColInitLane ln = col_init_lane(a, b, u, g);
-#pragma unroll
-    for (int i = 0; i < kColRO + 2; ++i) zr[i] = col_init_load_lean(ln, F, f_own0 - 1 + i, t);
-  } else {
-#pragma unroll
-    for (int i = 0; i < kColRO + 2; ++i) zr[i] = col_init_load(a, b, u, f_own0 - 1 + i, t, g);
-  }
+#pragma unroll
+  for (int i = 0; i < kColRO + 2; ++i) zr[i] = col_init_load(a, b, u, f_own0 - 1 + i, t, g);
   if constexpr (FIRST) stage->load_rest(prm);
-  const int m = LEAN ? 0 : prm.m;
+  const int m = prm.m;
   const float wm = a.masking ? 1.f : (a.mcs_mask ? a.mcs_mask[((size_t)b * a.U + u) * a.M + m] : (m == 0 ? 1.f : 0.f));
   if constexpr (FIRST) {
     stage->store_w1(smem);
@@ -478,12 +475,10 @@
                                 : (float)slot_norm(npre, yslot, nqs, reinterpret_cast<double*>(smem + kColRed));
   col_ts(k, 5);
   half8 zin[kColRO + 2][1];
-  const float zsc = g == 2 ? 1.f : ns;
 #pragma unroll
   for (int i = 0; i < kColRO + 2; ++i) {
     const int f = f_own0 - 1 + i;
-    if constexpr (LEAN) zin[i][0] = col_init_z_lean(zr[i], zsc, f >= 0 && f < F && t < kT, g);
-    else zin[i][0] = col_init_z(zr[i], ns, f >= 0 && f < F && t < kT, g, a.use_h != 0);
+    zin[i][0] = col_init_z(zr[i], ns, f >= 0 && f < F && t < kT, g, a.use_h != 0);
   }
   dpp_in_fence(zin);
   if (a.pe16 && g == 2 && t < kT) {
@@ -528,14 +523,14 @@
   col_ts(k, 4);
   using WS3 = WLds<P16, kHID, kDSP>;
   const WS3 w3{smem + kRrW3};
-  EpiConv3<P16, WS3, 16, TAILM, LT> epi{&prm, nullptr, smem + kRrW3, w3, b, u, f_start, col_pos_hi(strips), 1, wm, m == 0,
+  EpiConv3<P16, WS3, 16, TAILM> epi{&prm, nullptr, smem + kRrW3, w3, b, u, f_start, col_pos_hi(strips), 1, wm, m == 0,
                                     (float)a.active[(size_t)b * a.U + u], -1, 0, 0};
   epi.pos_lo = col_pos_lo(strips);
   col_conv3<NRX_COL_PR3>(own, nb, epi, lane, t, g, p0);
   col_ts(k, 6);
 }
 
-template <int TAILM, bool MULTI, class LT = ColGeneric>
+template <int TAILM, bool MULTI>
 __device__ __forceinline__ void col_init_stage(const BlockParams<P16>& prm, int items) {
   extern __shared__ __attribute__((aligned(16))) char smem[];
   rr_ts(0, 7);
@@ -545,8 +540,8 @@
     ColStage<32, TAILM> stage;
     stage.load_w1(prm);
     int b, u, strip;
-    work_item(blockIdx.x, prm.a.B, prm.a.U, LT::kLean ? 1 : prm.strips, prm.order_rev, b, u, strip);
-    col_init_item<TAILM, true, LT>(prm, smem, wave, b, u, strip, 0, &stage);
+    work_item(blockIdx.x, prm.a.B, prm.a.U, prm.strips, prm.order_rev, b, u, strip);
+    col_init_item<TAILM, true>(prm, smem, wave, b, u, strip, 0, &stage);
   }
   if constexpr (MULTI) {
     int k = 1;
@@ -559,13 +554,232 @@
   rr_ts_edge(1);
 }
 
-template <int TAILM, class LT = ColGeneric>
+template <int TAILM>
 __global__ __launch_bounds__(512) void k_init_col(BlockParams<P16> prm, int items) {
-  col_init_stage<TAILM, false, LT>(prm, items);
+  col_init_stage<TAILM, false>(prm, items);
 }
 template <int TAILM>
 __global__ __launch_bounds__(512) void k_init_col_multi(BlockParams<P16> prm, int items) {
   col_init_stage<TAILM, true>(prm, items);
+}
+
+#ifndef NRX_COL_ROWS_FIRST
+#define NRX_COL_ROWS_FIRST 1
+#endif
+
+__device__ __forceinline__ void col_item(const ColLaunch& cl, int& b, int& u, int& bu) {
+  const int i = blockIdx.x, U = cl.U;
+  auto divu = [&](int v, int& q, int& r) __attribute__((always_inline)) {
+    if (U == 1) q = v, r = 0;
+    else if (U == 2) q = v >> 1, r = v & 1;
+    else q = v / U, r = v % U;
+  };
+  if (cl.wi_full < 0) {
+    int j = i >> 3;
+    if (cl.order_rev) j = cl.wi_per - 1 - j;
+    bu = (i & 7) * cl.wi_per + j;
+    divu(bu, b, u);
+  } else if (i < cl.wi_full) {
+    int j = i >> 3, q;
+    if (cl.order_rev) j = cl.wi_per - 1 - j;
+    divu(j, q, u);
+    b = 8 * q + (i & 7);
+    bu = b * U + u;
+  } else {
+    bu = i;
+    divu(i, b, u);
+  }
+}
+
+__device__ __forceinline__ GZ col_gz_block(const ColLaunch& cl, int bu, int u, int t, int g) {
+  GZ gz;
+  char* base = reinterpret_cast<char*>(((unsigned long long)(cl.rsrc[1] & 0xffffu) << 32) | cl.rsrc[0]);
+  gz.rsrc = __builtin_amdgcn_make_buffer_rsrc(base, (short)(cl.rsrc[1] >> 16), (int)cl.rsrc[2], (int)cl.rsrc[3]);
+  gz.f_start = 0;
+  gz.F = cl.F;
+  const unsigned tb = (unsigned)(t * kDS * 2);
+  const unsigned so = cl.s_in0 + (unsigned)bu * cl.st_bu + tb;
+  const unsigned ao = cl.a0 + (unsigned)bu * cl.a_bu + (unsigned)(u * cl.a_u) + tb;
+  const unsigned po = cl.pe0 + (unsigned)u * cl.st_bu + tb;
+#pragma unroll
+  for (int kc = 0; kc < 4; ++kc) {
+    const int q = 4 * kc + g;
+    unsigned off = kGzOob;
+    if (t < kT) {
+      if (q < 7) off = ao + 16u * q;
+      else if (q < 14) off = so + 16u * (q - 7);
+      else if (q == 14) off = po;
+    }
+    gz.off[kc] = off;
+  }
+  return gz;
+}
+
+template <int TAILM, class LT>
+__device__ __forceinline__ void col_update_lean(const ColLaunch& cl) {
+  extern __shared__ __attribute__((aligned(16))) char smem[];
+  constexpr int PR = 2, CHP = 16, k = 0;
+  rr_ts(0, 7);
+  rr_ts_edge(0);
+  const int wave = __builtin_amdgcn_readfirstlane(nrx_tid() >> 6);
+  ColStage<kUPD_CINP, TAILM> stage;
+  if constexpr (!NRX_COL_ROWS_FIRST) stage.load_w1(cl);
+  int b, u, bu;
+  col_item(cl, b, u, bu);
+  col_ts(k, 0);
+  const int lane = nrx_tid() & 63, t = lane & 15, g = lane >> 4;
+  const int p0 = kColRO * wave, f_own0 = p0;
+  const int F = cl.F;
+  const GZ gz = col_gz_block(cl, bu, u, t, g);
+  ColZ<PR> z;
+  col_gz_first<PR>(z, gz, p0);
+  if constexpr (NRX_COL_ROWS_FIRST) stage.load_w1(cl);
+  COL_PRO_TS(0);
+  stage.load_rest(cl);
+  COL_PRO_TS(1);
+  half8 own[kColRO][4];
+  stage.store_w1(smem);
+  COL_PRO_TS(2);
+  __syncthreads();
+  col_ts(k, 5);
+  {
+    const WRr<kHID> w1(smem + kRrW1, t < kT ? smem + kRrW1 + kWBias : smem + kRrNeg + kRrNegOff, g);
+    col_conv1_gz<PR>(z, gz, w1, lane, g, own, f_own0, F, [&]() { stage.store_rest(smem); });
+  }
+  col_ts(k, 1);
+  __syncthreads();
+  int te = t, ge = g;
+  asm volatile("" : "+v"(te), "+v"(ge));
+  rr_write_exch<kColRO>(smem, wave, te, ge, own);
+  const RrNb nb = rr_nb(smem, wave, te, ge);
+  __syncthreads();
+  col_ts(k, 2);
+  {
+    const WRr<kHID> w2(smem + kRrW2, te < kT ? smem + kRrW2 + kWBias : smem + kRrNeg + kRrNegOff, ge);
+    half8 nxt[kColRO][4];
+    col_layer<4, kColRO, PR, false>(own, nb, w2, lane, ge, nxt, f_own0, F);
+#pragma unroll
+    for (int r = 0; r < kColRO; ++r)
+#pragma unroll
+      for (int kc = 0; kc < 4; ++kc) own[r][kc] = nxt[r][kc];
+  }
+  col_ts(k, 3);
+  int t3 = t, g3 = g;
+  asm volatile("" : "+v"(t3), "+v"(g3));
+  using WS3 = WLds<P16, kHID, kDSP>;
+  const WS3 w3{smem + kRrW3};
+  char* WB = TAILM == TAIL_READOUT_WB ? smem + kRrW1 : smem + kRrW3;
+  if constexpr (TAILM == TAIL_READOUT_WB) {
+    RrHeads<CHP> hd;
+    hd.load(cl.tail);
+    __syncthreads();
+    rr_write_exch<kColRO>(smem, wave, t3, g3, own);
+    hd.store(WB, LT::kBits, LT::kA2);
+  } else {
+    __syncthreads();
+    rr_write_exch<kColRO>(smem, wave, t3, g3, own);
+  }
+  __syncthreads();
+  col_ts(k, 4);
+  EpiConv3<P16, WS3, CHP, TAILM, LT> epi{&cl, nullptr, WB, w3, b, u, 0, kColPos, 0, 1.f, false, (float)cl.active[bu], -1, 0, 0};
+  epi.bu = bu;
+  if constexpr (TAILM == TAIL_READOUT_WB) col_conv3_ro<NRX_COL_PR3, true>(own, nb, epi, lane, t, g, p0, g3);
+  else col_conv3<NRX_COL_PR3, true>(own, nb, epi, lane, t, g, p0, g3);
+  col_ts(k, 6);
+  rr_ts_edge(1);
+}
+
+template <class LT>
+__device__ __forceinline__ void col_init_lean(const ColLaunch& cl) {
+  extern __shared__ __attribute__((aligned(16))) char smem[];
+  constexpr int PR = 2, k = 0;
+  rr_ts(0, 7);
+  rr_ts_edge(0);
+  const int wave = __builtin_amdgcn_readfirstlane(nrx_tid() >> 6);
+  ColStage<32, TAIL_AGG> stage;
+  if constexpr (!NRX_COL_ROWS_FIRST) stage.load_w1(cl);
+  int b, u, bu;
+  col_item(cl, b, u, bu);
+  col_ts(k, 0);
+  const int lane = nrx_tid() & 63, t = lane & 15, g = lane >> 4;
+  const int p0 = kColRO * wave, f_own0 = p0;
+  const int F = cl.F;
+  const char* yb = cl.y + (size_t)((unsigned)b * cl.y_b);
+  const float* yslot = reinterpret_cast<const float*>(yb);
+  const int nqs = cl.nq;
+  const NormPre npre = slot_norm_issue(yslot, nqs);
+  ColInitRow zr[kColRO + 2];
+  const ColInitLane ln{g == 1 ? cl.h_hat + (size_t)((unsigned)bu * cl.y_b) : yb, cl.pe + (size_t)((unsigned)u * cl.pe_u)};
+#pragma unroll
+  for (int i = 0; i < kColRO + 2; ++i) zr[i] = col_init_load_lean(ln, F, f_own0 - 1 + i, t);
+  if constexpr (NRX_COL_ROWS_FIRST) stage.load_w1(cl);
+  stage.load_rest(cl);
+  const RrNb nb = rr_nb(smem, wave, t, g);
+  const float wm = cl.mcs_mask ? cl.mcs_mask[(size_t)bu * cl.M] : 1.f;
+  stage.store_w1(smem);
+  const float ns = (float)slot_norm(npre, yslot, nqs, reinterpret_cast<double*>(smem + kColRed));
+  col_ts(k, 5);
+  half8 zin[kColRO + 2][1];
+  const float zsc = g == 2 ? 1.f : ns;
+#pragma unroll
+  for (int i = 0; i < kColRO + 2; ++i) {
+    const int f = f_own0 - 1 + i;
+    zin[i][0] = col_init_z_lean(zr[i], zsc, f >= 0 && f < F && t < kT, g);
+  }
+  dpp_in_fence(zin);
+  if (cl.pe16 && g == 2 && t < kT) {
+    char* pe16 = cl.pe16 + (size_t)((unsigned)u * cl.st_bu);
+#pragma unroll
+    for (int i = 1; i <= kColRO; ++i) {
+      const int f = p0 + i - 1;
+      if (f < F) *reinterpret_cast<half8*>(pe16 + (unsigned)sre(f, t) * 2u) = zin[i][0];
+    }
+  }
+  half8 own[kColRO][4];
+  {
+    const WCol<32, kHID> w1(smem + kRrW1, t < kT ? smem + kRrW1 + kWBias : smem + kRrNeg + kRrNegOff, g);
+    half8 o1[kColRO][4];
+    col_layer<1, kColRO, PR, true>(zin, nb, w1, lane, g, o1, f_own0, F, [&]() { stage.store_rest(smem); });
+#pragma unroll
+    for (int r = 0; r < kColRO; ++r)
+#pragma unroll
+      for (int kc = 0; kc < 4; ++kc) own[r][kc] = o1[r][kc];
+  }
+  col_ts(k, 1);
+  __syncthreads();
+  rr_write_exch<kColRO>(smem, wave, t, g, own);
+  __syncthreads();
+  col_ts(k, 2);
+  {
+    const WRr<kHID> w2(smem + kRrW2, t < kT ? smem + kRrW2 + kWBias : smem + kRrNeg + kRrNegOff, g);
+    half8 nxt[kColRO][4];
+    col_layer<4, kColRO, PR, false>(own, nb, w2, lane, g, nxt, f_own0, F);
+#pragma unroll
+    for (int r = 0; r < kColRO; ++r)
+#pragma unroll
+      for (int kc = 0; kc < 4; ++kc) own[r][kc] = nxt[r][kc];
+  }
+  col_ts(k, 3);
+  __syncthreads();
+  rr_write_exch<kColRO>(smem, wave, t, g, own);
+  __syncthreads();
+  col_ts(k, 4);
+  using WS3 = WLds<P16, kHID, kDSP>;
+  const WS3 w3{smem + kRrW3};
+  EpiConv3<P16, WS3, 16, TAIL_AGG, LT> epi{&cl, nullptr, smem + kRrW3, w3, b, u, 0, kColPos, 1, wm, true, (float)cl.active[bu], -1, 0, 0};
+  epi.bu = bu;
+  col_conv3<NRX_COL_PR3>(own, nb, epi, lane, t, g, p0);
+  col_ts(k, 6);
+  rr_ts_edge(1);
+}
+
+template <int TAILM, class LT>
+__global__ __launch_bounds__(512) void k_update_col_lean(ColLaunch cl) {
+  col_update_lean<TAILM, LT>(cl);
+}
+template <class LT>
+__global__ __launch_bounds__(512) void k_init_col_lean(ColLaunch cl) {
+  col_init_lean<LT>(cl);
 }
 
 struct ColFwdParams {
diff --git a/neural_rx_amd/csrc/nrx_device.inc b/neural_rx_amd/csrc/nrx_device.inc
--- a/neural_rx_amd/csrc/nrx_device.inc
+++ b/neural_rx_amd/csrc/nrx_device.inc
@@ -834,7 +834,8 @@
   static constexpr bool kNextHook = TAILM == TAIL_AGG && P::WLDS;
   static constexpr bool kNextHookRO = TAILM == TAIL_READOUT_WB && P::WLDS;
   static constexpr int kEarlyRow = 8;
-  const BlockParams<P>* prm;
+  using Prm = std::conditional_t<LT::kLean, ColLaunch, BlockParams<P>>;
+  const Prm* prm;
   char* X;
   char* WB;
   WS ws;
@@ -847,7 +848,12 @@
   const BlockParams<P>* nprm = nullptr;
   const int* ndone = nullptr;
   int* nflag = nullptr;
-
+  int bu = 0;
+
+  __device__ const auto& args() const {
+    if constexpr (LT::kLean) return *prm;
+    else return prm->a;
+  }
   __device__ bool next_ready() const { return nb >= 0 && (!ndone || *nflag); }
 
   template <int R>
@@ -863,13 +869,12 @@
   __device__ void next_hook();
 
   __device__ bool row_ok(int p, int t) const {
-    if constexpr (LT::kLean) return p < prm->a.F && t < kT;
-    return p >= pos_lo && p < pos_hi && f_start + p < prm->a.F && t < kT;
+    if constexpr (LT::kLean) return p < prm->F && t < kT;
+    else return p >= pos_lo && p < pos_hi && f_start + p < prm->a.F && t < kT;
   }
 
   template <int R>
   __device__ void prefetch(PrefT<R>& pf, int p0, int t, int g) const {
-    const auto& a = prm->a;
     if constexpr (LT::kLean) {
       static_assert(sizeof(S) == 2, "lean variants are f16");
       if (mode != 0) {
@@ -879,7 +884,7 @@
           for (int n = 0; n < NTS; ++n) pf.prev[r][n] = half4{0, 0, 0, 0};
         return;
       }
-      const char* plane = reinterpret_cast<const char*>(a.s_in + srow(b, u, 0, 0, a.U, a.F));
+      const char* plane = prm->s_in + (size_t)((unsigned)bu * prm->st_bu);
       __builtin_amdgcn_sched_barrier(0);
 #pragma unroll
       for (int r = 0; r < R; ++r) {
@@ -893,8 +898,8 @@
         }
       }
       __builtin_amdgcn_sched_barrier(0);
-      return;
-    }
+    } else {
+    const auto& a = prm->a;
     const bool need = mode == 0 || !first;
 #pragma unroll
     for (int r = 0; r < R; ++r) {
@@ -916,6 +921,7 @@
           }
         }
       }
+    }
     }
   }
 
@@ -985,7 +991,8 @@
       w1 = WB + (ch ? kHW1C : 0);
       b1 = reinterpret_cast<const float*>(WB + kHB1 + (ch ? kHID * 4 : 0));
       b2 = reinterpret_cast<const float*>(WB + kHB2 + (ch ? 16 * 4 : 0));
-      w2 = WB + kHW2 + (ch ? (LT::kLean ? 4 : prm->a.bits_max) * 256 : 0);
+      if constexpr (LT::kLean) w2 = WB + kHW2 + (ch ? 4 * 256 : 0);
+      else w2 = WB + kHW2 + (ch ? prm->a.bits_max * 256 : 0);
     } else {
       w1 = X + head_w1(hh);
       b1 = reinterpret_cast<const float*>(X + head_b1(hh));
@@ -1014,8 +1021,6 @@
                       int r_lo, int r_hi) const {
     if (r_lo >= r_hi) return;
     stamp(6);
-    const auto& a = prm->a;
-    const int F = a.F, U = a.U;
     const int lane = nrx_tid() & 63;
     typename P::Acc accw[R][NTS];
 #pragma unroll
@@ -1046,19 +1051,32 @@
           if (co >= kDS) v = 0;
           sv[r][n][j] = (Real)(S)v;
         }
-    size_t off[R];
+    std::conditional_t<LT::kLean, unsigned, size_t> off[R];
     bool ok[R];
 #pragma unroll
     for (int r = 0; r < R; ++r) {
       ok[r] = row_ok(p0 + r, t) && !(NRX_ABLATE & 16);
-      off[r] = srow(b, u, 0, 0, U, F) + (size_t)(unsigned)sre(ok[r] ? f_start + p0 + r : 0, ok[r] ? t : 0);
-    }
+      if constexpr (LT::kLean) off[r] = (unsigned)sre(ok[r] ? p0 + r : 0, ok[r] ? t : 0);
+      else off[r] = srow(b, u, 0, 0, prm->a.U, prm->a.F) + (size_t)(unsigned)sre(ok[r] ? f_start + p0 + r : 0, ok[r] ? t : 0);
+    }
+    auto row_dst = [&](bool agg, int r) __attribute__((always_inline)) -> S* {
+      if constexpr (LT::kLean) {
+        char* plane = (agg ? prm->a_out : prm->s_out) + (size_t)((unsigned)bu * prm->st_bu);
+        return reinterpret_cast<S*>(plane) + off[r];
+      } else {
+        return (agg ? prm->a.a_out : prm->a.s_out) + off[r];
+      }
+    };
+    auto slots = [&]() __attribute__((always_inline)) {
+      if constexpr (LT::kLean) return prm->B;
+      else return prm->a.B;
+    };
     if constexpr (!readout_tail(TAILM)) {
 #pragma unroll
       for (int r = 0; r < R; ++r) {
-        S* dst = a.s_out + off[r];
+        S* dst = row_dst(false, r);
         if constexpr (sizeof(S) == 2) {
-          store_row16(dst, sv[r], ok[r] && !((NRX_ABLATE & 32) && a.B > 0), g);
+          store_row16(dst, sv[r], ok[r] && !((NRX_ABLATE & 32) && slots() > 0), g);
         } else {
           if (!ok[r]) continue;
 #pragma unroll
@@ -1105,16 +1123,26 @@
         }
         dense_rows<P, kAGG / 16, kDSP, R>(hb, DGlb<P, kAGG>{prm->agg[1]}, lane, g, sp, false);
       }
+      if constexpr (LT::kLean) {
+        if (act != (Real)1) {
+#pragma unroll
+          for (int r = 0; r < R; ++r)
+#pragma unroll
+            for (int n = 0; n < NTS; ++n)
+#pragma unroll
+              for (int j = 0; j < 4; ++j) sp[r][n][j] *= act;
+        }
+      }
 #pragma unroll
       for (int r = 0; r < R; ++r) {
-        S* dst = a.a_out + off[r];
+        S* dst = row_dst(true, r);
         if constexpr (sizeof(S) == 2) {
           Real spa[NTS][4];
 #pragma unroll
           for (int n = 0; n < NTS; ++n)
 #pragma unroll
-            for (int j = 0; j < 4; ++j) spa[n][j] = sp[r][n][j] * act;
-          store_row16(dst, spa, ok[r] && !((NRX_ABLATE & 64) && a.B > 0), g);
+            for (int j = 0; j < 4; ++j) spa[n][j] = LT::kLean ? sp[r][n][j] : sp[r][n][j] * act;
+          store_row16(dst, spa, ok[r] && !((NRX_ABLATE & 64) && slots() > 0), g);
         } else {
           if (!ok[r]) continue;
 #pragma unroll
@@ -1144,7 +1172,7 @@
 
   template <int RB>
   __device__ void readout_rows(const CFrag<P, NTS> (&sbr)[RB], const bool (&okr)[RB], int p0r, int t, int g) const {
-    const auto& a = prm->a;
+    const auto& a = args();
     const int F = a.F, U = a.U;
     const int lane = nrx_tid() & 63;
     auto one_head = [&](int hh, bool ch) __attribute__((always_inline)) {
@@ -1159,8 +1187,8 @@
           head_rows<1, RB>(sbr, DGlb<P, kDSP>{prm->llr[hh][0]}, DGlb<P, kHID>{prm->llr[hh][1]}, lane, g, o);
         }
         if constexpr (LT::kLean) {
-          char* plane = reinterpret_cast<char*>(a.llr + ((size_t)b * U + u) * F * kT * LT::kBits);
-          const int nb = a.head_bits[0];
+          char* plane = prm->llr + (size_t)((unsigned)bu * prm->llr_bu);
+          const int nb = prm->head_bits;
 #pragma unroll
           for (int r = 0; r < RB; ++r) {
             if (okr[r] && g == 0)
@@ -1168,8 +1196,7 @@
                   floatx4{nb > 0 ? (float)o[r][0][0] : 0.f, nb > 1 ? (float)o[r][0][1] : 0.f,
                           nb > 2 ? (float)o[r][0][2] : 0.f, nb > 3 ? (float)o[r][0][3] : 0.f};
           }
-          return;
-        }
+        } else {
 #pragma unroll
         for (int r = 0; r < RB; ++r) {
           if (!okr[r]) continue;
@@ -1191,6 +1218,7 @@
             if (co < a.bits_max) dst[co] = co < a.head_bits[hh] ? (float)o[r][0][j] : 0.f;
           }
         }
+        }
       } else {
         Real o[RB][CHP / 16][4];
         if constexpr (P::WLDS) {
@@ -1203,22 +1231,23 @@
         }
         if constexpr (LT::kLean) {
           static_assert(CHP == 16 && LT::kA2 == 8, "lean ChEst store");
-          char* plane = reinterpret_cast<char*>(a.h_ref + ((size_t)b * U + u) * F * kT * LT::kA2);
+          char* plane = prm->h_ref + (size_t)((unsigned)bu * prm->href_bu);
+          unsigned go = 16u * (unsigned)g;
+          asm volatile("" : "+v"(go));
 #pragma unroll
           for (int r = 0; r < RB; ++r) {
             if (okr[r] && g < 2)
-              *reinterpret_cast<floatx4*>(plane + (unsigned)((p0r + r) * kT + t) * (unsigned)(LT::kA2 * 4) +
-                                          16u * (unsigned)g) =
+              *reinterpret_cast<floatx4*>(plane + ((unsigned)((p0r + r) * kT + t) * (unsigned)(LT::kA2 * 4) + go)) =
                   floatx4{(float)o[r][0][0], (float)o[r][0][1], (float)o[r][0][2], (float)o[r][0][3]};
           }
-          return;
-        }
+        } else {
         const int A2 = 2 * a.A;
 #pragma unroll
         for (int r = 0; r < RB; ++r) {
           if (!okr[r]) continue;
           const int f = f_start + p0r + r;
           store_f32<CHP / 16>(a.h_ref + ((((size_t)b * U + u) * F + f) * kT + t) * A2, o[r], g, A2);
+        }
         }
       }
     };
diff --git a/neural_rx_amd/csrc/nrx_geom.h b/neural_rx_amd/csrc/nrx_geom.h
--- a/neural_rx_amd/csrc/nrx_geom.h
+++ b/neural_rx_amd/csrc/nrx_geom.h
@@ -74,4 +74,72 @@
 #define NRX_COL_LEAN 1
 #endif
 
+struct ColLaunch {
+  unsigned rsrc[4];
+  unsigned s_in0, a0, pe0;
+  unsigned st_bu;
+  unsigned a_bu;
+  int a_u;
+  int F, U, B, order_rev;
+  int wi_full, wi_per;
+  int head_bits;
+  int M;
+  const char* s_in;
+  char* s_out;
+  char* a_out;
+  char* llr;
+  char* h_ref;
+  unsigned llr_bu, href_bu;
+  const float* active;
+  const char* y;
+  const char* h_hat;
+  const char* pe;
+  char* pe16;
+  const float* mcs_mask;
+  unsigned y_b, pe_u;
+  int nq, pad_;
+  SepW<_Float16, float> w[3];
+  DenseW<_Float16, float> tail[4];
+};
+
+inline ColLaunch col_launch_block(const FwdArgs<_Float16, float, _Float16>& a, int inline_combine, int order_rev) {
+  ColLaunch c{};
+  const uintptr_t base = reinterpret_cast<uintptr_t>(a.ws_base);
+  c.rsrc[0] = (unsigned)base;
+  c.rsrc[1] = (unsigned)(base >> 32) & 0xffffu;
+  c.rsrc[2] = a.ws_bytes;
+  c.rsrc[3] = 0x00020000u;
+  auto rel = [&](const void* p) { return (unsigned)(reinterpret_cast<const char*>(p) - a.ws_base); };
+  const unsigned plane = (unsigned)a.F * kT * kDS * 2u;
+  c.st_bu = plane;
+  c.s_in0 = rel(a.s_in);
+  c.pe0 = rel(a.pe16);
+  if (!inline_combine) c.a0 = rel(a.a), c.a_bu = plane, c.a_u = 0;
+  else if (a.U == 2) c.a0 = rel(a.a) + plane, c.a_bu = plane, c.a_u = -2 * (int)plane;
+  else c.a0 = kGzOob, c.a_bu = 0, c.a_u = 0;
+  c.F = a.F, c.U = a.U, c.B = a.B, c.order_rev = order_rev;
+  const int per_xcd = (a.B / 8) * a.U;
+  c.wi_full = 8 * per_xcd, c.wi_per = per_xcd;
+  if (per_xcd == 0 && (a.B * a.U) % 8 == 0) c.wi_full = -1, c.wi_per = a.B * a.U / 8;
+  c.head_bits = a.head_bits[0];
+  c.M = a.M;
+  c.s_in = reinterpret_cast<const char*>(a.s_in);
+  c.s_out = reinterpret_cast<char*>(a.s_out);
+  c.a_out = reinterpret_cast<char*>(a.a_out);
+  c.llr = reinterpret_cast<char*>(a.llr);
+  c.h_ref = reinterpret_cast<char*>(a.h_ref);
+  c.llr_bu = (unsigned)a.F * kT * ColLean<true>::kBits * 4u;
+  c.href_bu = (unsigned)a.F * kT * ColLean<true>::kA2 * 4u;
+  c.active = a.active;
+  c.y = reinterpret_cast<const char*>(a.y);
+  c.h_hat = reinterpret_cast<const char*>(a.h_hat);
+  c.pe = reinterpret_cast<const char*>(a.pe);
+  c.pe16 = reinterpret_cast<char*>(a.pe16);
+  c.mcs_mask = a.masking ? nullptr : a.mcs_mask;
+  c.y_b = (unsigned)a.F * kT * ColLean<true>::kA2 * 4u;
+  c.pe_u = (unsigned)a.F * kT * 2u * 4u;
+  c.nq = a.F * kT * ColLean<true>::kA2 / 4;
+  return c;
 }
+
+}
diff --git a/neural_rx_amd/csrc/nrx_internal.h b/neural_rx_amd/csrc/nrx_internal.h
--- a/neural_rx_amd/csrc/nrx_internal.h
+++ b/neural_rx_amd/csrc/nrx_internal.h
@@ -102,6 +102,16 @@
   S* pe16;
 };
 
+template <class A>
+inline void stage_planes(A& a, int s) {
+  const int i = s - a.num_init;
+  if (i < 0 || i % 2 != 0) return;
+  auto* si = a.s_in;
+  a.s_in = a.s_out, a.s_out = si;
+  auto* ai = a.a;
+  a.a = a.a_out, a.a_out = ai;
+}
+
 struct FusedCtl {
   void* sync;
   int spin_limit;
diff --git a/neural_rx_amd/csrc/nrx_k_col.hip b/neural_rx_amd/csrc/nrx_k_col.hip
--- a/neural_rx_amd/csrc/nrx_k_col.hip
+++ b/neural_rx_amd/csrc/nrx_k_col.hip
@@ -7,24 +7,23 @@
 #include "nrx_col.inc"
 
 #ifdef NRX_STAMPS
-static void col_stamp_select(hipStream_t st) {
+static int col_stamp_select(hipStream_t st) {
   static int launch_no = 0;
   static const int sel = getenv("NRX_STAMP_COL") ? atoi(getenv("NRX_STAMP_COL")) : -1;
   const int on = launch_no++ == sel;
   (void)hipMemcpyToSymbolAsync(HIP_SYMBOL(g_nrx_stamp_on), &on, sizeof(int), 0, hipMemcpyHostToDevice, st);
+  return on;
 }
 #else
-static void col_stamp_select(hipStream_t) {}
+static int col_stamp_select(hipStream_t) { return 0; }
 #endif
 
 hipError_t launch_init_col(const BlockParams<P16>& bp, const StagePlan& sp, hipStream_t st) {
   const int items = sp.items, grid = sp.grid;
-  col_stamp_select(st);
+  const int stamp = col_stamp_select(st);
   const bool agg = sp.tail == TAIL_AGG;
-  if (sp.variant != COL_GENERIC) {
-    if (!sp.one || !agg) return hipErrorInvalidValue;
-    k_init_col<TAIL_AGG, ColLean<true>><<<grid, 512, sp.lds, st>>>(bp, items);
-  } else if (sp.one) {
+  if (sp.variant != COL_GENERIC) return launch_init_col_lean(bp, sp, stamp, st);
+  if (sp.one) {
     if (agg) k_init_col<TAIL_AGG><<<grid, 512, sp.lds, st>>>(bp, items);
     else k_init_col<TAIL_NONE><<<grid, 512, sp.lds, st>>>(bp, items);
   } else {
@@ -37,13 +36,9 @@
 hipError_t launch_update_col(const BlockParams<P16>& bp, const StagePlan& sp, hipStream_t st) {
   const int items = sp.items, grid = sp.grid, L = sp.lds;
   const bool ch32 = sp.chp == 32, one = sp.one;
-  col_stamp_select(st);
-  if (sp.variant != COL_GENERIC) {
-    if (!one || ch32) return hipErrorInvalidValue;
-    if (sp.tail != TAIL_READOUT_WB) k_update_col<16, TAIL_AGG, ColLean<true>><<<grid, 512, L, st>>>(bp, items);
-    else if (sp.variant == COL_LEAN) k_update_col<16, TAIL_READOUT_WB, ColLean<true>><<<grid, 512, L, st>>>(bp, items);
-    else k_update_col<16, TAIL_READOUT_WB, ColLean<false>><<<grid, 512, L, st>>>(bp, items);
-  } else if (sp.tail == TAIL_READOUT_WB) {
+  const int stamp = col_stamp_select(st);
+  if (sp.variant != COL_GENERIC) return launch_update_col_lean(bp, sp, stamp, st);
+  if (sp.tail == TAIL_READOUT_WB) {
     if (ch32) {
       if (one) k_update_col<32, TAIL_READOUT_WB><<<grid, 512, L, st>>>(bp, items);
       else k_update_col_multi<32, TAIL_READOUT_WB><<<grid, 512, L, st>>>(bp, items);
@@ -106,10 +101,7 @@
   set((const void*)k_update_col_multi<16, TAIL_READOUT_WB>);
   set((const void*)k_update_col_multi<32, TAIL_READOUT_WB>);
   set((const void*)k_fwd_col<16>);
-  set((const void*)k_init_col<TAIL_AGG, ColLean<true>>);
-  set((const void*)k_update_col<16, TAIL_AGG, ColLean<true>>);
-  set((const void*)k_update_col<16, TAIL_READOUT_WB, ColLean<true>>);
-  set((const void*)k_update_col<16, TAIL_READOUT_WB, ColLean<false>>);
+  if (const hipError_t r = setup_col_lean(); r != hipSuccess) e = r;
   return e;
 }
 
@@ -117,6 +109,8 @@
 
 #ifdef NRX_STAMPS
 extern "C" int nrx_debug_col_stamps(void* out, int n) {
-  return (int)hipMemcpyFromSymbol(out, HIP_SYMBOL(nrx::g_nrx_rr_stamps), (size_t)n * 64 * 8, 0, hipMemcpyDeviceToHost);
+  const hipError_t e =
+      hipMemcpyFromSymbol(out, HIP_SYMBOL(nrx::g_nrx_rr_stamps), (size_t)n * 64 * 8, 0, hipMemcpyDeviceToHost);
+  return e != hipSuccess ? (int)e : (int)nrx::col_lean_stamps(static_cast<unsigned long long*>(out), n);
 }
 #endif
diff --git a/neural_rx_amd/csrc/nrx_k_col_lean.hip b/neural_rx_amd/csrc/nrx_k_col_lean.hip
--- /dev/null
+++ b/neural_rx_amd/csrc/nrx_k_col_lean.hip
@@ -0,0 +1,74 @@
+#include "nrx_device.inc"
+#include "nrx_launch.inc"
+
+namespace nrx {
+
+#include "nrx_rr.inc"
+#include "nrx_col.inc"
+
+static ColLaunch lean_block(const BlockParams<P16>& bp, const StagePlan& sp) {
+  ColLaunch cl = col_launch_block(bp.a, bp.inline_combine, sp.order_rev);
+  for (int l = 0; l < 3; ++l) cl.w[l] = bp.w[l];
+  if (sp.tail == TAIL_READOUT_WB) {
+    cl.tail[0] = bp.llr[0][0], cl.tail[1] = bp.llr[0][1], cl.tail[2] = bp.chest[0], cl.tail[3] = bp.chest[1];
+  } else {
+    cl.tail[0] = bp.agg[0], cl.tail[1] = bp.agg[1];
+  }
+  return cl;
+}
+
+#ifdef NRX_STAMPS
+static void lean_stamp_select(int on, hipStream_t st) {
+  (void)hipMemcpyToSymbolAsync(HIP_SYMBOL(g_nrx_stamp_on), &on, sizeof(int), 0, hipMemcpyHostToDevice, st);
+}
+#else
+static void lean_stamp_select(int, hipStream_t) {}
+#endif
+
+hipError_t launch_init_col_lean(const BlockParams<P16>& bp, const StagePlan& sp, int stamp, hipStream_t st) {
+  if (sp.variant == COL_GENERIC || !sp.one || sp.tail != TAIL_AGG) return hipErrorInvalidValue;
+  lean_stamp_select(stamp, st);
+  k_init_col_lean<ColLean<true>><<<sp.grid, 512, sp.lds, st>>>(lean_block(bp, sp));
+  return hipGetLastError();
+}
+
+hipError_t launch_update_col_lean(const BlockParams<P16>& bp, const StagePlan& sp, int stamp, hipStream_t st) {
+  if (sp.variant == COL_GENERIC || !sp.one || sp.chp == 32) return hipErrorInvalidValue;
+  lean_stamp_select(stamp, st);
+  const ColLaunch cl = lean_block(bp, sp);
+  const int grid = sp.grid, L = sp.lds;
+  if (sp.tail != TAIL_READOUT_WB) k_update_col_lean<TAIL_AGG, ColLean<true>><<<grid, 512, L, st>>>(cl);
+  else if (sp.variant == COL_LEAN) k_update_col_lean<TAIL_READOUT_WB, ColLean<true>><<<grid, 512, L, st>>>(cl);
+  else k_update_col_lean<TAIL_READOUT_WB, ColLean<false>><<<grid, 512, L, st>>>(cl);
+  return hipGetLastError();
+}
+
+hipError_t setup_col_lean() {
+  hipError_t e = hipSuccess;
+  auto set = [&](const void* f) {
+    const hipError_t r = hipFuncSetAttribute(f, hipFuncAttributeMaxDynamicSharedMemorySize, kColLds);
+    if (r != hipSuccess) e = r;
+  };
+  set((const void*)k_init_col_lean<ColLean<true>>);
+  set((const void*)k_update_col_lean<TAIL_AGG, ColLean<true>>);
+  set((const void*)k_update_col_lean<TAIL_READOUT_WB, ColLean<true>>);
+  set((const void*)k_update_col_lean<TAIL_READOUT_WB, ColLean<false>>);
+  return e;
+}
+
+hipError_t col_lean_stamps(unsigned long long* out, int n) {
+#ifdef NRX_STAMPS
+  unsigned long long* tmp = static_cast<unsigned long long*>(malloc((size_t)n * 64 * 8));
+  if (!tmp) return hipErrorOutOfMemory;
+  const hipError_t e = hipMemcpyFromSymbol(tmp, HIP_SYMBOL(g_nrx_rr_stamps), (size_t)n * 64 * 8, 0, hipMemcpyDeviceToHost);
+  for (size_t i = 0; e == hipSuccess && i < (size_t)n * 64; ++i)
+    if (tmp[i]) out[i] = tmp[i];
+  free(tmp);
+  return e;
+#else
+  (void)out, (void)n;
+  return hipSuccess;
+#endif
+}
+
+}
diff --git a/neural_rx_amd/csrc/nrx_launch.inc b/neural_rx_amd/csrc/nrx_launch.inc
--- a/neural_rx_amd/csrc/nrx_launch.inc
+++ b/neural_rx_amd/csrc/nrx_launch.inc
@@ -20,6 +20,10 @@
 hipError_t launch_fwd_col(const Args16& args, const Model16& W, const FwdPlan& pl, const FusedCtl& fc, hipStream_t st,
                           Prof* prof);
 hipError_t setup_col();
+hipError_t launch_init_col_lean(const BlockParams<P16>& bp, const StagePlan& sp, int stamp, hipStream_t st);
+hipError_t launch_update_col_lean(const BlockParams<P16>& bp, const StagePlan& sp, int stamp, hipStream_t st);
+hipError_t setup_col_lean();
+hipError_t col_lean_stamps(unsigned long long* out, int n);
 
 template <class P>
 static void plan_stage(BlockParams<P>& bp, const FwdArgs<typename P::WT, typename P::BT, typename P::S>& args,
@@ -27,10 +31,7 @@
   const int i = s - args.num_init;
   const bool last = i == num_it - 1;
   bp.a = args;
-  if (i >= 0 && i % 2 == 0) {
-    std::swap(bp.a.s_in, bp.a.s_out);
-    std::swap(bp.a.a, bp.a.a_out);
-  }
+  stage_planes(bp.a, s);
   for (int l = 0; l < 3; ++l) bp.w[l] = i < 0 ? W.init[s][l] : W.upd[i][l];
   bp.m = i < 0 ? s : 0;
   bp.tail = i < 0 ? (s == args.num_init - 1 ? TAIL_AGG : TAIL_NONE) : (last ? ro_tail : TAIL_AGG);
diff --git a/neural_rx_amd/csrc/nrx_rr.inc b/neural_rx_amd/csrc/nrx_rr.inc
--- a/neural_rx_amd/csrc/nrx_rr.inc
+++ b/neural_rx_amd/csrc/nrx_rr.inc
@@ -199,6 +199,18 @@
     c1.store(WB + kHW1C, reinterpret_cast<float*>(WB + kHB1 + kHID * 4));
     l2.store(WB + kHW2, reinterpret_cast<float*>(WB + kHB2), nb2);
     c2.store(WB + kHW2 + nb2 * 256, reinterpret_cast<float*>(WB + kHB2 + 16 * 4), 2 * prm.a.A);
+  }
+  __device__ __forceinline__ void load(const DenseW<_Float16, float> (&hw)[4]) {
+    l1.load(hw[0]);
+    l2.load(hw[1]);
+    c1.load(hw[2]);
+    c2.load(hw[3]);
+  }
+  __device__ __forceinline__ void store(char* WB, int nb2, int a2) const {
+    l1.store(WB, reinterpret_cast<float*>(WB + kHB1));
+    c1.store(WB + kHW1C, reinterpret_cast<float*>(WB + kHB1 + kHID * 4));
+    l2.store(WB + kHW2, reinterpret_cast<float*>(WB + kHB2), nb2);
+    c2.store(WB + kHW2 + nb2 * 256, reinterpret_cast<float*>(WB + kHB2 + 16 * 4), a2);
   }
 };
 
```

New measurement: 1.287 million slots/s (median of 6 runs). No clear change (+0.7%).
